# qiyueyao/Kubernetes-verification

Measured on AMD Instinct MI355X. Metric: pod-pairs/sec for reachability build + all-checks latency, 100k pods, 1/2/4/8 GPU, higher is better.
Workload: dtype u64

## Files before the change

kubernetes-verification_amd/csrc/kano_engine.hpp:

```cpp
#pragma once
#include <hip/hip_runtime.h>
#include <hip/hip_ext.h>

#include <algorithm>
#include <cmath>
#include <functional>
#include <cerrno>
#include <cstdint>
#include <cstdlib>
#include <cstring>
#include <string>
#include <vector>
#include <array>
#include <chrono>
#include <ctime>
#include <cstdio>
#include <dlfcn.h>
#include <link.h>
#include <thread>

#include "kano_hip.h"
#include "kano_internal.hpp"
#include "kano_prims.hpp"

using namespace kano;

namespace {
constexpr int MAX_CWW = 8192;
constexpr int MAX_CWW_KNOB = 16384;
constexpr int XCD_WRITE = 3;
constexpr long long XCD_MIN_BYTES = 1ll << 30;
constexpr int HT_ROWS = 128;
constexpr int ROWS_CH = 24;
constexpr int LD_ALIGN = 16;
constexpr int MFMA_KMIN = 8;

}

struct DBuf {
  void* p = nullptr;
  size_t bytes = 0;
};

struct ClassSet {
  std::vector<int32_t> keys;
  int KS = 0;
  int packed = 0;
  int tbits = 0;
  i64 U = 0;
  i64 m0 = 0, m1 = 0;
  DBuf keys_d, table, smin, slot_of, flag, cid, cls, rep, mcnt, mcur, moff, mem, cval;
};

struct RowsInputs {
  DBuf wioff, wicls, soffc, slist, aloff, alist, alcoff, alc, rmoff, rmem, cmoff, cmem, ccls,
      hflag, hlist, Mc;
};

struct SideMatch {
  i64 nterms = 0;
  int NM = 0;
  bool dense = false;
  DBuf toff, tslot, tval, pmask, moff, mslot;
  DBuf table, pslot, gcnt, goff, gcur, gmem, pstart, plen, bits, bcnt, boff;
  i64 T = 0;
};

enum {
  SZ_UR = 0, SZ_UA, SZ_NNZ_SEL, SZ_NNZ_ALC, SZ_NNZ_ALW, SZ_NFLAGS, SZ_WI, SZ_HEAVY, SZ_MAXSEL,
  SZ_LIGHT, SZ_HSEL, SZ_NL, SZ_PAIRS, SZ_IDX0, SZ_IDX1, SZ_IDX2, SZ_IDX3, SZ_ERR, SZ_SLOTS = 18,
  SZ_SIGNAL = SZ_SLOTS
};

constexpr size_t ROW_STAGE_BYTES = 256 * 1024;

struct kano_ctx {
  int device = 0;
  hipStream_t stream = nullptr;
  bool own_stream = false;
  std::string err;

  i64 n = 0, W = 0, ldM = 0, P = 0, PB = 0;
  int ncols = 0;
  std::vector<int32_t> colbits;
  i64 r0 = 0, r1 = -1;
  bool have_pods = false, have_pols = false, built = false;
  bool lists_mode = false;
  bool cols_valid = false;
  bool rows_dirty = false;
  bool rows_deferred = false;
  bool defer_alloc = false;
  bool rows_timed = false;
  bool alist_valid = false;
  bool cols_deferred = false;
  int32_t cross_G = 0;
  i64 groups_n = -1;
  int32_t groups_G = 0;
  int stage_timing = 0;
  int cls_packed = 1;
  int rows_wide = 1;
  DBuf rw_items, rw_segs, rw_ticket;
  DBuf slist_tmp;
  int sort_ww = 768;
  i64 rows_w_grid = 0;
  int rows_early_heavy = 2;
  int assign_ipt = 0;
  int async_rows = 1;
  int shadow_count_mode = 0;
  int path_dens = 8;
  int path_tm = 2;
  int path_tn = 2;
  int heavy_gemm = -1;
  double xo_mfma = 4500e12, xo_or = 8500e9;
  i64 heavy_gemm_min = 512;
  int time_or = 0;
  int heavy_expand_lds = 2;
  int dx_on = 1;
  DBuf dx_sc, dx_sa;
  DBuf mct;
  bool shg_prefilled = false;
  i64 dx_ldY = 0, dx_PBo = 0;
  bool dense_sel = false;
  int ac_lds = 1;
  int mlists_side_ok = 1;
  bool mlists_side = false;
  bool rin_marked = false;
  i64 sel_early_cap = -1;
  int path_lds = 1;
  int rows_ch = ROWS_CH;
  int rows_cww = MAX_CWW_KNOB;
  int shadow_r = 0;
  int shg_sub_lds = 1;
  int rows_cu_off = 20;
  int xcd_split = 1;
  i64 xcd_min_bytes = XCD_MIN_BYTES;
  int xcd_write = XCD_WRITE;
  int xcd_eng0 = -1;
  bool xcd_tried = false, eng_on_xcd = false, xcd_last_ok = false;
  int side_mode = 0;
  int xcd_side = -1;
  hipStream_t stream_x = nullptr, stream2_x = nullptr, stream3x = nullptr;
  hipStream_t stream2_u = nullptr;
  hipEvent_t ev_sw = nullptr, ev_sw2 = nullptr;
  i64 rows_cu_bytes = 8ll << 30;
  int num_cus = 0, rows_cus = 0;

  ClassSet rc, cc;
  SideMatch sm, am;
  i64 UAW = 0, ldC = 0;
  i64 nnz_sel = 0, nnz_alc = 0, nnz_alw = 0, heavy_count = 0, wi_total = 0, nflags = 0;
  i64 heavy_sel = 0;
  i64 light_cost = 0;
  bool rows_use_alist = false;
  int max_sel = 0;
  int heavy_path = 0;
  int heavy_kernel = 0;
  int rows_kernel = 0;

  DBuf pv;
  DBuf scnt, cost, soffc, scur, slist, ecls, wicls, maxs, wicnt, wioff, hflag, hoff, hlist, sq, pfoff;
  DBuf ACT, AC, nca, acnt, alcoff, alc, aloff, alist;
  DBuf M, Mc, color, colnand, col_and, col_or_c, col_nand_c;
  DBuf scan_tmp;
  i64 scan_cap = 0;
  int scan_parity = 0;
  DBuf scan_tmp2;
  i64 scan_cap2 = 0;
  int scan_parity2 = 0;
  hipEvent_t ev_pre = nullptr, ev_pre_done = nullptr, ev_pre_ac = nullptr;
  bool pre_forked = false, pre_side_pending = false, pre_ac_pending = false;
  bool tail_compacted = false;
  hipEvent_t ev_pairs = nullptr;
  DBuf gid, gids, cgroup, R, multi, A1, A2, own, cross, gmin, gmax, ckey, corder, kcnt, koff;
  DBuf flags, T, loff, L, tp, poff, out, tcnt, toff;
  DBuf scratch_words, ident;
  DBuf xw, xg;
  i64 xg_emul = -1;
  DBuf pT, pR[2], pD[2], pA, pB, pcnt;
  DBuf xv, asel, aalw, iterm, idead, irows;
  i64 inc_A = 0, inc_acap = 0, inc_xcols = 0;
  std::vector<uint8_t> dead;
  bool user_edited = false;
  i64 shadow_total = -1;
  DBuf conflict_out;
  i64 conflict_total = -1;
  bool vs_count_only = false;
  bool shg_ran = false;
  DBuf shg_h, shg_tkey, shg_trep, shg_slot, shg_isrep, shg_gidx, shg_gid, shg_reps, shg_sub,
      shg_err;
  DBuf sizes;
  DBuf icnt, ioff, sysrow, idxd;
  u64* ghost = nullptr;
  void* row_stage = nullptr;
  u64* gmirror = nullptr;
  u64* gmirror_dev = nullptr;
  DBuf sig_ctr;
  u64 sig_seq = 0;
  u64 sig_armed = 0;
  u64 sig_wait = 0;
  double ht[20] = {};
  double ht_wait_cur = 0.0;
  int ht_wait = 0;
  std::chrono::steady_clock::time_point ht_last{};

  hipEvent_t ev[10] = {};
  hipStream_t stream2 = nullptr;
  hipEvent_t ev_fork2 = nullptr, ev_join2 = nullptr;
  bool fork_pending = false;
  std::function<int(bool)> fork_hook;
  hipStream_t stream3 = nullptr;
  hipStream_t stream3m = nullptr;
  bool stream3m_tried = false;
  hipStream_t rows_last = nullptr;
  RowsInputs rin_alt;
  int rows_set = 0;
  bool rows_overlap = false;
  hipEvent_t rows_after = nullptr;
  hipEvent_t rows_in = nullptr;
  hipEvent_t ev_rin = nullptr;
  hipEvent_t ev_rin_e = nullptr;
  hipEvent_t ev_rows_end[2] = {};
  hipEvent_t rows_end_ev[2] = {};
  bool rows_end_rec[2] = {false, false};
  hipEvent_t ev_fork = nullptr;
  hipEvent_t ev_sizes = nullptr;
  bool async_pending = false;
  int pipeline = 0;
  bool primed = false;
  bool priming = false;
  bool consume_prime = false;
  bool prime_pre_marked = false;
  bool prime_alist_valid = false;
  u64 prime_sig = 0;
  u64* bell = nullptr;
  u64* bell_dev = nullptr;
  u64 bell_seq = 0;
  u64 gate_ticks = 0;
  u64 wall_khz = 100000;
  DBuf gate_wait;
  u64 gate_seq0 = 0;
  u64 gate_forced = 0;
  DBuf sizes_alt;
  hipEvent_t ev_tail = nullptr;
  hipEvent_t ev_rt[2][2] = {};
  bool rows_time_pending[2] = {false, false};
  hipEvent_t ev_m0 = nullptr, ev_m1 = nullptr;
  bool mfma_time_pending = false;
  double mfma_ops_last = 0.0, mfma_ops_sum = 0.0, mfma_ms_sum = 0.0;
  i64 mfma_n = 0;
  float rows_ms_last = 0.f;
  double rows_ms_sum = 0.0, rows_ms_min = 0.0, rows_ms_max = 0.0;
  i64 rows_ms_n = 0;
  bool vs_open = false, vs_shadow = false, vs_cross_want = false, vs_cross_on = false;
  bool vs_have_sys = false, vs_sys_on = false;
  bool vs_rows = false;
  i64 vs_nb = 0, vs_rl = 0;
};

#define KCHK(expr)                                                                 \
  do {                                                                             \
    hipError_t e_ = (expr);                                                        \
    if (e_ != hipSuccess) {                                                        \
      ctx->err = std::string(#expr) + " -> " + hipGetErrorString(e_);             \
      return -EIO;                                                                 \
    }                                                                              \
  } while (0)

#define KLAUNCH()                                                                  \
  do {                                                                             \
    hipError_t e_ = hipGetLastError();                                             \
    if (e_ != hipSuccess) {                                                        \
      ctx->err = std::string("kernel launch at line ") + std::to_string(__LINE__) + \
                 " -> " + hipGetErrorString(e_);                                   \
      return -EIO;                                                                 \
    }                                                                              \
  } while (0)

#define KTRY(expr)       \
  do {                   \
    int rc_ = (expr);    \
    if (rc_) return rc_; \
  } while (0)

namespace kano_eng {

int fail(kano_ctx* ctx, int code, const std::string& msg);
int settle(kano_ctx* ctx);
int dalloc(kano_ctx* ctx, DBuf& b, size_t bytes);
void dfree(DBuf& b);
int sync(kano_ctx* ctx);
int ensure_built(kano_ctx* ctx);
int ensure_matrix(kano_ctx* ctx);
i64 rows_local(const kano_ctx* ctx);

template <typename T>
T* P_(DBuf& b) {
  return reinterpret_cast<T*>(b.p);
}

inline unsigned nblk(i64 n, i64 per = TPB) { return (unsigned)((n + per - 1) / per); }

}
```

kubernetes-verification_amd/csrc/kano_hip.hip:

```cpp
#include "kano_engine.hpp"
#include "kano_kernels.hpp"

namespace kano_eng {

int fail(kano_ctx* ctx, int code, const std::string& msg) {
  ctx->err = msg;
  return code;
}

int settle(kano_ctx* ctx);

int dalloc(kano_ctx* ctx, DBuf& b, size_t bytes) {
  if (bytes == 0) bytes = 16;
  if (b.p && b.bytes >= bytes) return 0;
  if (b.p) {
    KTRY(settle(ctx));
    KCHK(hipFree(b.p));
    b.p = nullptr;
    b.bytes = 0;
  }
  const hipError_t e = hipMalloc(&b.p, bytes);
  if (e != hipSuccess) {
    b.p = nullptr;
    return fail(ctx, -ENOMEM, "hipMalloc(" + std::to_string(bytes) + " bytes) -> " +
                                  hipGetErrorString(e));
  }
  b.bytes = bytes;
  return 0;
}

void dfree(DBuf& b) {
  if (b.p) (void)hipFree(b.p);
  b.p = nullptr;
  b.bytes = 0;
}


template <typename... KArgs, typename... Args>
void launch_marked(void (*kernel)(KArgs...), dim3 grid, dim3 block, size_t lds, hipStream_t st,
                   hipEvent_t ev, Args... args) {
  hipExtLaunchKernelGGL(kernel, grid, block, (std::uint32_t)lds, st, nullptr, ev, 0, args...);
}

inline i64 scan_tiles(i64 n, int items = SCAN_ITEMS) {
  return (n + (i64)TPB * items - 1) / ((i64)TPB * items);
}

int scan_reserve(kano_ctx* ctx, i64 slots, bool side = false) {
  i64& cap = side ? ctx->scan_cap2 : ctx->scan_cap;
  if (slots <= cap) return 0;
  slots = std::max<i64>(slots, 2 * cap);
  const size_t bytes = sizeof(u64) * 2 * (size_t)slots;
  DBuf& tmp = side ? ctx->scan_tmp2 : ctx->scan_tmp;
  KTRY(dalloc(ctx, tmp, bytes));
  KCHK(hipMemsetAsync(tmp.p, 0, bytes, side ? ctx->stream2 : ctx->stream));
  cap = slots;
  (side ? ctx->scan_parity2 : ctx->scan_parity) = 0;
  return 0;
}

struct ScanBatch {
  ScanJobs jobs{};
  kano_ctx* ctx;
  bool side = false;
  explicit ScanBatch(kano_ctx* c, bool on_side = false) : ctx(c), side(on_side) {
    jobs.count = 0;
    jobs.npub = 0;
  }
  void publish(int slot) {
    if (!ctx->gmirror_dev || jobs.npub == MAX_PUBLISH) return;
    jobs.pub_src[jobs.npub] = P_<u64>(ctx->sizes) + slot;
    jobs.pub_dst[jobs.npub] = ctx->gmirror_dev + slot;
    ++jobs.npub;
  }
  template <typename Tin, typename Tout>
  int add(const Tin* in, i64 n, Tout* out, int total_slot = -1) {
    static_assert(sizeof(Tin) == 4 || sizeof(Tin) == 8, "int32 / int64 scans");
    static_assert(sizeof(Tout) == 4 || sizeof(Tout) == 8, "int32 / int64 scans");
    if (jobs.count == MAX_SCAN_JOBS) KTRY(run());
    ScanJob& j = jobs.j[jobs.count++];
    j.in = in;
    j.out = out;
    j.total = total_slot >= 0 ? P_<u64>(ctx->sizes) + total_slot : nullptr;
    j.total_host = total_slot >= 0 && ctx->gmirror_dev ? ctx->gmirror_dev + total_slot : nullptr;
    j.n = n;
    j.st = 0;
    j.in64 = sizeof(Tin) == 8;
    j.out64 = sizeof(Tout) == 8;
    j.gen = 0;
    j.gcnt = nullptr;
    return 0;
  }
  int add_rep_flags(ClassSet& cs, int pbits, i64 n, int total_slot) {
    KTRY(add(static_cast<const int32_t*>(nullptr), n, P_<int32_t>(cs.cid), total_slot));
    ScanJob& j = jobs.j[jobs.count - 1];
    j.gen = 1;
    j.gsmin = P_<int32_t>(cs.smin);
    j.gtab = P_<u64>(cs.table);
    j.gpb = pbits;
    j.gslot = P_<int32_t>(cs.slot_of);
    j.gm0 = cs.m0;
    return 0;
  }
  int add_class_lengths(const int32_t* cls, const i64* loff, i64 m0, i64 n, i64* out,
                        int total_slot) {
    KTRY(add(static_cast<const int32_t*>(nullptr), n, out, total_slot));
    ScanJob& j = jobs.j[jobs.count - 1];
    j.gen = 2;
    j.gslot = cls;
    j.gloff = loff;
    j.gm0 = m0;
    return 0;
  }
  int add_class_counts(const int32_t* cls, const i64* cnt, i64 m0, i64 n, i64* out,
                       int total_slot) {
    KTRY(add(static_cast<const int32_t*>(nullptr), n, out, total_slot));
    ScanJob& j = jobs.j[jobs.count - 1];
    j.gen = 3;
    j.gslot = cls;
    j.gcnt = cnt;
    j.gm0 = m0;
    return 0;
  }
  template <int NJ, int IT>
  void launch_n(dim3 g, u64* cur, u64* nxt, hipEvent_t mark) {
    ScanJobsN<NJ> a;
    for (int q = 0; q < NJ; ++q) a.j[q] = jobs.j[q];
    a.count = jobs.count;
    a.npub = jobs.npub;
    for (int q = 0; q < MAX_PUBLISH; ++q) {
      a.pub_src[q] = jobs.pub_src[q];
      a.pub_dst[q] = jobs.pub_dst[q];
    }
    a.sig_host = jobs.sig_host;
    a.sig_val = jobs.sig_val;
    a.sig_ctr = jobs.sig_ctr;
    a.sig_n = jobs.sig_n;
    launch_marked(k_scan_lb<NJ, IT>, g, dim3(TPB), 0, side ? ctx->stream2 : ctx->stream, mark, a,
                  cur, nxt, side ? ctx->scan_cap2 : ctx->scan_cap);
  }
  template <int IT>
  void launch_it(dim3 g, u64* cur, u64* nxt, hipEvent_t mark) {
    switch (jobs.count) {
      case 1: launch_n<1, IT>(g, cur, nxt, mark); break;
      case 2: launch_n<2, IT>(g, cur, nxt, mark); break;
      case 3: launch_n<3, IT>(g, cur, nxt, mark); break;
      case 4: launch_n<4, IT>(g, cur, nxt, mark); break;
      case 5: launch_n<5, IT>(g, cur, nxt, mark); break;
      case 6: launch_n<6, IT>(g, cur, nxt, mark); break;
      case 7: launch_n<7, IT>(g, cur, nxt, mark); break;
      default: launch_n<MAX_SCAN_JOBS, IT>(g, cur, nxt, mark); break;
    }
  }
  int run(hipEvent_t mark = nullptr) {
    if (jobs.count == 0) return 0;
    const int items = SCAN_ITEMS;
    i64 slots = 0, maxt = 1;
    for (int q = 0; q < jobs.count; ++q) {
      jobs.j[q].st = slots;
      slots += 1 + scan_tiles(jobs.j[q].n, items);
      maxt = std::max<i64>(maxt, scan_tiles(jobs.j[q].n, items));
    }
    KTRY(scan_reserve(ctx, slots, side));
    int writers = jobs.npub > 0 ? 1 : 0;
    for (int q = 0; q < jobs.count; ++q) writers += jobs.j[q].total_host ? 1 : 0;
    jobs.sig_host = nullptr;
    if (side) writers = 0;
    if (writers > 0 && ctx->sig_ctr.p) {
      jobs.sig_host = ctx->gmirror_dev + SZ_SIGNAL;
      jobs.sig_val = ++ctx->sig_seq;
      jobs.sig_ctr = reinterpret_cast<uint32_t*>(ctx->sig_ctr.p);
      jobs.sig_n = writers;
      ctx->sig_armed = jobs.sig_val;
    } else if (writers > 0) {
      ctx->sig_armed = 0;
    }
    u64* st = P_<u64>(side ? ctx->scan_tmp2 : ctx->scan_tmp);
    const i64 cap = side ? ctx->scan_cap2 : ctx->scan_cap;
    int& parity = side ? ctx->scan_parity2 : ctx->scan_parity;
    u64* cur = st + (parity ? cap : 0);
    u64* nxt = st + (parity ? 0 : cap);
    const dim3 g((unsigned)maxt, (unsigned)jobs.count);
    if (items == 32) launch_it<32>(g, cur, nxt, mark);
    else if (items == 16) launch_it<16>(g, cur, nxt, mark);
    else if (items == 4) launch_it<4>(g, cur, nxt, mark);
    else launch_it<SCAN_ITEMS>(g, cur, nxt, mark);
    KLAUNCH();
    parity ^= 1;
    jobs.count = 0;
    jobs.npub = 0;
    return 0;
  }
};

template <typename Tin, typename Tout>
int scan_excl(kano_ctx* ctx, const Tin* in, i64 n, Tout* out) {
  ScanBatch sb(ctx);
  KTRY(sb.add(in, n, out));
  return sb.run();
}

struct FillBatch {
  FillJobs jobs{};
  kano_ctx* ctx;
  hipStream_t st = nullptr;
  explicit FillBatch(kano_ctx* c, hipStream_t s = nullptr) : ctx(c), st(s) { jobs.count = 0; }
  int add(DBuf& b, size_t bytes, uint32_t value);
  int add_raw(void* p, size_t bytes, uint32_t value) {
    if (bytes == 0) return 0;
    if (jobs.count == MAX_FILLS) KTRY(run());
    jobs.j[jobs.count++] = FillJob{static_cast<uint32_t*>(p), (i64)(bytes / 4), value};
    return 0;
  }
  int run();
  FillJobs take() {
    FillJobs j = jobs;
    jobs.count = 0;
    return j;
  }
};

unsigned fill_ride_blocks(const FillJobs& fj) {
  if (fj.count == 0) return 0;
  i64 most = 0;
  for (int q = 0; q < fj.count; ++q) most = std::max(most, fj.j[q].words);
  return (unsigned)std::max<i64>(1, std::min<i64>(FILL_RIDE_BLOCKS, (most + TPB - 1) / TPB));
}

int FillBatch::add(DBuf& b, size_t bytes, uint32_t value) {
  if (bytes == 0) return 0;
  if (bytes % 4 != 0 || bytes > b.bytes) return fail(ctx, -EINVAL, "internal: bad fill job");
  if (jobs.count == MAX_FILLS) KTRY(run());
  jobs.j[jobs.count++] = FillJob{reinterpret_cast<uint32_t*>(b.p), (i64)(bytes / 4), value};
  return 0;
}

int FillBatch::run() {
  if (jobs.count == 0) return 0;
  i64 most = 0;
  for (int q = 0; q < jobs.count; ++q) most = std::max(most, jobs.j[q].words);
  const unsigned grid = (unsigned)std::max<i64>(1, std::min<i64>(2048, (most + TPB - 1) / TPB));
  hipLaunchKernelGGL(k_fill_many, dim3(grid), dim3(TPB), 0, st ? st : ctx->stream, jobs);
  KLAUNCH();
  jobs.count = 0;
  return 0;
}

void swap_rows_ptrs(kano_ctx* ctx) {
  RowsInputs& a = ctx->rin_alt;
  std::swap(ctx->wioff, a.wioff);
  std::swap(ctx->wicls, a.wicls);
  std::swap(ctx->soffc, a.soffc);
  std::swap(ctx->slist, a.slist);
  std::swap(ctx->aloff, a.aloff);
  std::swap(ctx->alist, a.alist);
  std::swap(ctx->alcoff, a.alcoff);
  std::swap(ctx->alc, a.alc);
  std::swap(ctx->rc.moff, a.rmoff);
  std::swap(ctx->rc.mem, a.rmem);
  std::swap(ctx->cc.moff, a.cmoff);
  std::swap(ctx->cc.mem, a.cmem);
  std::swap(ctx->cc.cls, a.ccls);
  std::swap(ctx->hflag, a.hflag);
  std::swap(ctx->hlist, a.hlist);
  std::swap(ctx->Mc, a.Mc);
  ctx->rows_set ^= 1;
}

void ring_bell(kano_ctx* ctx) {
  if (ctx->bell) __atomic_store_n(ctx->bell, ctx->bell_seq, __ATOMIC_SEQ_CST);
}

int unprime(kano_ctx* ctx) {
  if (!ctx->primed || ctx->priming) return 0;
  ctx->primed = false;
  ring_bell(ctx);
  ctx->gate_forced = ctx->bell_seq;
  KCHK(hipStreamSynchronize(ctx->stream));
  KCHK(hipStreamSynchronize(ctx->stream2));
  std::swap(ctx->sizes, ctx->sizes_alt);
  swap_rows_ptrs(ctx);
  ctx->alist_valid = ctx->prime_alist_valid;
  return 0;
}

int sync(kano_ctx* ctx) {
  KTRY(unprime(ctx));
  KCHK(hipStreamSynchronize(ctx->stream));
  return 0;
}

int settle(kano_ctx* ctx) {
  KTRY(unprime(ctx));
  if (!ctx->async_pending) return 0;
  ctx->async_pending = false;
  KCHK(hipSetDevice(ctx->device));
  KCHK(hipStreamSynchronize(ctx->stream3));
  if (ctx->stream3m) KCHK(hipStreamSynchronize(ctx->stream3m));
  if (ctx->stream3x) KCHK(hipStreamSynchronize(ctx->stream3x));
  return sync(ctx);
}

int resolve_rows_slot(kano_ctx* ctx, int k, bool block) {
  if (!ctx->rows_time_pending[k]) return 0;
  if (!block) {
    const hipError_t q = hipEventQuery(ctx->ev_rt[k][1]);
    if (q == hipErrorNotReady) return 0;
    KCHK(q);
  }
  ctx->rows_time_pending[k] = false;
  KCHK(hipEventSynchronize(ctx->ev_rt[k][1]));
  float ms = 0.f;
  KCHK(hipEventElapsedTime(&ms, ctx->ev_rt[k][0], ctx->ev_rt[k][1]));
  ctx->rows_ms_last = ms;
  if (ctx->rows_ms_n == 0 || ms < ctx->rows_ms_min) ctx->rows_ms_min = ms;
  if (ctx->rows_ms_n == 0 || ms > ctx->rows_ms_max) ctx->rows_ms_max = ms;
  ctx->rows_ms_sum += ms;
  ctx->rows_ms_n += 1;
  return 0;
}

int resolve_rows_time(kano_ctx* ctx, bool block = true) {
  for (int k = 0; k < 2; ++k) KTRY(resolve_rows_slot(ctx, k, block));
  return 0;
}

int swap_rows_inputs(kano_ctx* ctx) {
  swap_rows_ptrs(ctx);
  ctx->alist_valid = false;
  if (ctx->rows_end_rec[ctx->rows_set]) {
    const hipError_t q = hipEventQuery(ctx->rows_end_ev[ctx->rows_set]);
    if (q == hipErrorNotReady)
      KCHK(hipStreamWaitEvent(ctx->stream, ctx->rows_end_ev[ctx->rows_set], 0));
    else
      KCHK(q);
  }
  return 0;
}


int resolve_mfma_time(kano_ctx* ctx) {
  if (!ctx->mfma_time_pending) return 0;
  ctx->mfma_time_pending = false;
  KCHK(hipEventSynchronize(ctx->ev_m1));
  float ms = 0.f;
  KCHK(hipEventElapsedTime(&ms, ctx->ev_m0, ctx->ev_m1));
  ctx->mfma_ms_sum += ms;
  ctx->mfma_ops_sum += ctx->mfma_ops_last;
  ctx->mfma_n += 1;
  return 0;
}

int read_slots(kano_ctx* ctx, int first, int count, i64* out) {
  KCHK(hipMemcpyAsync(ctx->ghost, P_<u64>(ctx->sizes) + first, sizeof(u64) * count,
                      hipMemcpyDeviceToHost, ctx->stream));
  KTRY(sync(ctx));
  for (int k = 0; k < count; ++k) out[k] = (i64)ctx->ghost[k];
  return 0;
}

void* pinned_dev(void* host) {
  if (!host || (reinterpret_cast<uintptr_t>(host) & 15)) return nullptr;
  hipPointerAttribute_t at{};
  void* dptr = nullptr;
  if (hipPointerGetAttributes(&at, host) == hipSuccess && at.type == hipMemoryTypeHost &&
      at.devicePointer)
    dptr = at.devicePointer;
  (void)hipGetLastError();
  return dptr;
}

int copy_out(kano_ctx* ctx, void* host, const void* dev, size_t bytes, hipStream_t st) {
  if (bytes == 0) return 0;
  hipPointerAttribute_t at{};
  void* dptr = nullptr;
  if (hipPointerGetAttributes(&at, host) == hipSuccess && at.type == hipMemoryTypeHost &&
      at.devicePointer)
    dptr = at.devicePointer;
  (void)hipGetLastError();
  if (!dptr || (reinterpret_cast<uintptr_t>(dptr) & 15) || (reinterpret_cast<uintptr_t>(dev) & 15)) {
    KCHK(hipMemcpyAsync(host, dev, bytes, hipMemcpyDeviceToHost, st));
    return 0;
  }
  const i64 n16 = (i64)(bytes / 16);
  const int ntail = (int)((bytes % 16) / 4);
  const unsigned grid = (unsigned)std::max<i64>(1, std::min<i64>(1024, nblk(std::max<i64>(1, n16))));
  hipLaunchKernelGGL(k_copy_out, dim3(grid), dim3(TPB), 0, st, static_cast<const uint4*>(dev),
                     static_cast<uint4*>(dptr), n16,
                     reinterpret_cast<const uint32_t*>(static_cast<const char*>(dev) + n16 * 16),
                     reinterpret_cast<uint32_t*>(static_cast<char*>(dptr) + n16 * 16), ntail);
  KLAUNCH();
  return 0;
}

int mirror_begin(kano_ctx* ctx) {
  if (ctx->sig_armed) {
    ctx->sig_wait = ctx->sig_armed;
    ctx->sig_armed = 0;
    return 0;
  }
  ctx->sig_wait = 0;
  KCHK(hipEventRecord(ctx->ev_sizes, ctx->stream));
  return 0;
}

int wait_signal(kano_ctx* ctx, u64 val) {
  volatile u64* sig = ctx->gmirror + SZ_SIGNAL;
  using clk = std::chrono::steady_clock;
  const auto t0 = clk::now();
  for (uint32_t spin = 1; *sig < val; ++spin) {
    __builtin_ia32_pause();
    if ((spin & 0xfff) != 0) continue;
    if (clk::now() - t0 > std::chrono::seconds(1)) {
      KCHK(hipStreamSynchronize(ctx->stream));
      if (*sig < val)
        return fail(ctx, -EIO, "internal: host signal not raised (wait " +
                                   std::to_string(ctx->ht_wait) + ": want " + std::to_string(val) +
                                   ", have " + std::to_string((u64)*sig) + ")");
      break;
    }
  }
  return 0;
}

int mirror_wait(kano_ctx* ctx, int first, int count, i64* out) {
  const auto t0 = std::chrono::steady_clock::now();
  if (ctx->sig_wait) {
    const u64 v = ctx->sig_wait;
    ctx->sig_wait = 0;
    KTRY(wait_signal(ctx, v));
  } else {
    KCHK(hipEventSynchronize(ctx->ev_sizes));
  }
  const double w =
      std::chrono::duration<double, std::micro>(std::chrono::steady_clock::now() - t0).count();
  ctx->ht_wait_cur += w;
  const int k = 9 + std::min(ctx->ht_wait++, 2);
  ctx->ht[k] = std::max(ctx->ht[k], w);
  for (int q = 0; q < count; ++q) out[q] = (i64)((volatile u64*)ctx->gmirror)[first + q];
  return 0;
}

int stage_mark(kano_ctx* ctx, int k, hipStream_t st) {
  if (ctx->stage_timing) KCHK(hipEventRecord(ctx->ev[k], st));
  return 0;
}

i64 rows_local(const kano_ctx* ctx) { return ctx->r1 - ctx->r0; }

i64 table_size(i64 n) {
  i64 T = 64;
  while (T < 2 * n) T <<= 1;
  return T;
}

int cls_pod_bits(const kano_ctx* ctx, const ClassSet& cs) {
  if (!cs.packed) return 0;
  int pb = 1;
  while (pb < 31 && ((i64)1 << pb) < ctx->n) ++pb;
  return cs.tbits + pb <= 63 ? pb : 0;
}

int classify_alloc1(kano_ctx* ctx, ClassSet& cs, FillBatch& fb) {
  const i64 n = ctx->n, T = table_size(n);
  KTRY(dalloc(ctx, cs.table, sizeof(u64) * T));
  KTRY(dalloc(ctx, cs.smin, sizeof(int32_t) * T));
  KTRY(dalloc(ctx, cs.slot_of, sizeof(int32_t) * std::max<i64>(1, n)));
  KTRY(dalloc(ctx, cs.flag, sizeof(int32_t) * std::max<i64>(1, n)));
  KTRY(dalloc(ctx, cs.cid, sizeof(int32_t) * (n + 1)));
  KTRY(dalloc(ctx, cs.cls, sizeof(int32_t) * std::max<i64>(1, n)));
  KTRY(fb.add(cs.table, (cs.packed ? sizeof(u64) : sizeof(int32_t)) * T, 0xffffffffu));
  if (!cls_pod_bits(ctx, cs)) KTRY(fb.add(cs.smin, sizeof(int32_t) * T, 0x7fffffffu));
  const i64 m = std::max<i64>(1, cs.m1 - cs.m0);
  KTRY(dalloc(ctx, cs.rep, sizeof(int32_t) * m));
  KTRY(dalloc(ctx, cs.mcnt, sizeof(int32_t) * m));
  KTRY(dalloc(ctx, cs.mcur, sizeof(int32_t) * m));
  KTRY(dalloc(ctx, cs.moff, sizeof(int32_t) * (m + 1)));
  KTRY(dalloc(ctx, cs.mem, sizeof(int32_t) * m));
  return 0;
}

ClsSide cls_side(kano_ctx* ctx, ClassSet& cs) {
  ClsSide a{};
  a.keys = P_<int32_t>(cs.keys_d);
  a.KS = cs.KS;
  a.packed = cs.packed;
  a.pbits = cls_pod_bits(ctx, cs);
  a.tmask = (uint32_t)(table_size(ctx->n) - 1);
  a.table = P_<int32_t>(cs.table);
  a.slot_of = P_<int32_t>(cs.slot_of);
  a.smin = P_<int32_t>(cs.smin);
  a.flag = P_<int32_t>(cs.flag);
  a.cid = P_<int32_t>(cs.cid);
  a.cls = P_<int32_t>(cs.cls);
  a.rep = P_<int32_t>(cs.rep);
  a.mcnt = P_<int32_t>(cs.mcnt);
  a.mcur = P_<int32_t>(cs.mcur);
  a.moff = P_<int32_t>(cs.moff);
  a.mem = P_<int32_t>(cs.mem);
  a.cval = P_<int32_t>(cs.cval);
  a.m0 = cs.m0;
  a.m1 = cs.m1;
  a.U = cs.U;
  return a;
}

int classify_phase1(kano_ctx* ctx) {
  const i64 n = ctx->n;
  ClsPair pr{{cls_side(ctx, ctx->rc), cls_side(ctx, ctx->cc)}};
  const i64 nr = ctx->rc.m1 - ctx->rc.m0, na = ctx->cc.m1 - ctx->cc.m0;
  const i64 most = std::max(nr, na);
  if (most > 0) {
    hipLaunchKernelGGL(k_cls_insert, dim3(nblk(most), 2), dim3(TPB), 0, ctx->stream,
                       P_<int32_t>(ctx->pv), n, pr);
    KLAUNCH();
  }
  ScanBatch sb(ctx);
  KTRY(sb.add_rep_flags(ctx->rc, cls_pod_bits(ctx, ctx->rc), nr, SZ_UR));
  KTRY(sb.add_rep_flags(ctx->cc, cls_pod_bits(ctx, ctx->cc), na, SZ_UA));
  return sb.run();
}

int classify_alloc2(kano_ctx* ctx, ClassSet& cs) {
  return dalloc(ctx, cs.cval, sizeof(int32_t) * std::max<i64>(1, (i64)cs.KS * cs.U));
}

int classify_phase2a(kano_ctx* ctx) {
  ClsPair pr{{cls_side(ctx, ctx->rc), cls_side(ctx, ctx->cc)}};
  const i64 mr = ctx->rc.m1 - ctx->rc.m0, ma = ctx->cc.m1 - ctx->cc.m0;
  const i64 rl = std::max(mr, ma);
  hipStream_t side = ctx->mlists_side ? ctx->stream2 : nullptr;
  if (rl > 0) {
    const i64 prevU = std::max(ctx->rc.U, ctx->cc.U);
    const int ipt = ctx->assign_ipt > 0 ? ctx->assign_ipt
                                        : (prevU > 0 && prevU <= 1024 ? ASSIGN_IPT : 1);
    launch_marked(k_cls_assign_count, dim3(nblk(rl, (i64)TPB * ipt), 2), dim3(TPB), 0,
                  ctx->stream, side ? ctx->ev_pre : nullptr, pr, ipt);
    KLAUNCH();
  } else if (side) {
    KCHK(hipEventRecord(ctx->ev_pre, ctx->stream));
  }
  if (side) KCHK(hipStreamWaitEvent(side, ctx->ev_pre, 0));
  ScanBatch sb(ctx, side != nullptr);
  KTRY(sb.add(P_<int32_t>(ctx->rc.mcnt), mr, P_<int32_t>(ctx->rc.moff)));
  KTRY(sb.add(P_<int32_t>(ctx->cc.mcnt), ma, P_<int32_t>(ctx->cc.moff)));
  KTRY(sb.run());
  if (rl > 0) {
    hipLaunchKernelGGL(k_cls_mfill, dim3(nblk(rl), 2), dim3(TPB), 0, side ? side : ctx->stream, pr,
                       (const int32_t*)nullptr, 0, (int32_t*)nullptr, (int32_t*)nullptr,
                       reinterpret_cast<int32_t*>(P_<u64>(ctx->sizes) + SZ_ERR));
    KLAUNCH();
  }
  return 0;
}

int classify_phase2b(kano_ctx* ctx, FillJobs fj) {
  ClsPair pr{{cls_side(ctx, ctx->rc), cls_side(ctx, ctx->cc)}};
  const i64 U = std::max(ctx->rc.U, ctx->cc.U);
  if (U > 0) {
    const unsigned nbv = nblk(U), nbf = fill_ride_blocks(fj);
    hipLaunchKernelGGL(k_cls_vals, dim3(nbv + nbf, 2), dim3(TPB), 0, ctx->stream,
                       P_<int32_t>(ctx->pv), ctx->n, pr, fj, nbv);
    KLAUNCH();
  } else if (fj.count > 0) {
    hipLaunchKernelGGL(k_fill_many, dim3(fill_ride_blocks(fj)), dim3(TPB), 0, ctx->stream, fj);
    KLAUNCH();
  }
  return 0;
}

int match_alloc(kano_ctx* ctx, SideMatch& sx, ClassSet& cs, FillBatch& fb) {
  const i64 P = ctx->P, U = cs.U;
  KTRY(dalloc(ctx, sx.pstart, sizeof(i64) * std::max<i64>(1, P)));
  KTRY(dalloc(ctx, sx.plen, sizeof(int32_t) * std::max<i64>(1, P)));
  if (P == 0) return 0;
  if (U == 0) {
    KTRY(fb.add(sx.pstart, sizeof(i64) * P, 0u));
    KTRY(fb.add(sx.plen, sizeof(int32_t) * P, 0u));
    return 0;
  }
  if (sx.dense) return 0;
  const int NM = sx.NM;
  sx.T = table_size(U);
  const i64 NT = std::max<i64>(1, (i64)NM * sx.T);
  KTRY(dalloc(ctx, sx.table, sizeof(int32_t) * NT));
  KTRY(dalloc(ctx, sx.pslot, sizeof(int32_t) * std::max<i64>(1, (i64)NM * U)));
  KTRY(dalloc(ctx, sx.gcnt, sizeof(int32_t) * NT));
  KTRY(dalloc(ctx, sx.gcur, sizeof(int32_t) * std::max<i64>(1, (i64)NM * U)));
  KTRY(dalloc(ctx, sx.goff, sizeof(int32_t) * (NT + 1)));
  KTRY(dalloc(ctx, sx.gmem, sizeof(int32_t) * ((i64)NM * U + U)));
  if (NM > 0) {
    KTRY(fb.add(sx.table, sizeof(int32_t) * NT, 0xffffffffu));
    KTRY(fb.add(sx.gcnt, sizeof(int32_t) * NT, 0u));
  }
  return 0;
}

JoinSide join_side(kano_ctx* ctx, SideMatch& sx, ClassSet& cs) {
  JoinSide a{};
  a.cval = P_<int32_t>(cs.cval);
  a.U = cs.U;
  a.moff = P_<int32_t>(sx.moff);
  a.mslot = P_<int32_t>(sx.mslot);
  a.table = P_<int32_t>(sx.table);
  a.T = sx.T;
  a.pslot = P_<int32_t>(sx.pslot);
  a.gcnt = P_<int32_t>(sx.gcnt);
  a.goff = P_<int32_t>(sx.goff);
  a.gcur = P_<int32_t>(sx.gcur);
  a.gmem = P_<int32_t>(sx.gmem);
  a.toff = P_<i64>(sx.toff);
  a.tval = P_<int32_t>(sx.tval);
  a.pmask = P_<int32_t>(sx.pmask);
  a.pstart = P_<i64>(sx.pstart);
  a.plen = P_<int32_t>(sx.plen);
  a.NM = sx.NM;
  a.live = (ctx->P > 0 && cs.U > 0 && !sx.dense) ? 1 : 0;
  a.ctab = P_<u64>(cs.table);
  a.ctmask = (uint32_t)(table_size(ctx->n) - 1);
  a.csmin = P_<int32_t>(cs.smin);
  a.cpb = cls_pod_bits(ctx, cs);
  a.ccid = P_<int32_t>(cs.cid);
  a.cm0 = cs.m0;
  a.kbits = P_<int32_t>(cs.keys_d) + cs.KS;
  a.KS = cs.KS;
  return a;
}

int match_dense(kano_ctx* ctx, SideMatch& sx, ClassSet& cs);

int match_both(kano_ctx* ctx) {
  JoinPair pr{{join_side(ctx, ctx->am, ctx->cc), join_side(ctx, ctx->sm, ctx->rc)}};
  const JoinSide &a0 = pr.s[0], &a1 = pr.s[1];
  const i64 maxU = std::max(a0.live ? a0.U : 0, a1.live ? a1.U : 0);
  const unsigned rows_i = (a0.live ? a0.NM : 0) + (a1.live ? a1.NM : 0);
  const unsigned rows_f = (a0.live ? a0.NM + 1 : 0) + (a1.live ? a1.NM + 1 : 0);
  if (rows_i > 0) {
    hipLaunchKernelGGL(k_join_insert, dim3(nblk(maxU), rows_i), dim3(TPB), 0, ctx->stream, pr);
    KLAUNCH();
    ScanBatch sb(ctx);
    for (int q = 0; q < 2; ++q) {
      SideMatch& sx = q ? ctx->sm : ctx->am;
      if (pr.s[q].live && sx.NM > 0)
        KTRY(sb.add(P_<int32_t>(sx.gcnt), (i64)sx.NM * sx.T, P_<int32_t>(sx.goff)));
    }
    KTRY(sb.run());
  }
  if (rows_f > 0) {
    const unsigned nbf = nblk(maxU), nbm = nblk(ctx->P);
    hipLaunchKernelGGL(k_join_fill_match, dim3(std::max(nbf, nbm), rows_f + 2), dim3(TPB), 0,
                       ctx->stream, ctx->P, pr, (int)rows_f, nbf, nbm);
    KLAUNCH();
  }
  if (ctx->P > 0 && ctx->cc.U > 0 && ctx->am.dense) KTRY(match_dense(ctx, ctx->am, ctx->cc));
  if (ctx->P > 0 && ctx->rc.U > 0 && ctx->sm.dense) KTRY(match_dense(ctx, ctx->sm, ctx->rc));
  return 0;
}

int match_dense(kano_ctx* ctx, SideMatch& sx, ClassSet& cs) {
  const i64 P = ctx->P, U = cs.U;
  const i64 UW = (U + 63) / 64, ld = std::max<i64>(2, (UW + 1) & ~(i64)1);
  KTRY(dalloc(ctx, sx.bits, sizeof(u64) * P * ld));
  KTRY(dalloc(ctx, sx.boff, sizeof(i64) * (P + 1)));
  hipLaunchKernelGGL(k_class_eval, dim3(nblk(U), (unsigned)ctx->PB), dim3(TPB), 0, ctx->stream,
                     P_<int32_t>(cs.cval), U, P, P_<i64>(sx.toff), P_<int32_t>(sx.tslot),
                     P_<int32_t>(sx.tval), (u64*)nullptr, P_<u64>(sx.bits), ld);
  KLAUNCH();
  hipLaunchKernelGGL(k_popc_rows, dim3((unsigned)P), dim3(TPB), 0, ctx->stream, P_<u64>(sx.bits),
                     ld, UW, P_<int32_t>(sx.plen));
  KLAUNCH();
  KTRY((scan_excl<int32_t, i64>(ctx, P_<int32_t>(sx.plen), P, P_<i64>(sx.boff))));
  i64 nnz = 0;
  KCHK(hipMemcpyAsync(&nnz, P_<i64>(sx.boff) + P, 8, hipMemcpyDeviceToHost, ctx->stream));
  KTRY(sync(ctx));
  KTRY(dalloc(ctx, sx.gmem, sizeof(int32_t) * std::max<i64>(1, nnz)));
  hipLaunchKernelGGL(k_bits_to_lists, dim3((unsigned)P), dim3(TPB), 0, ctx->stream,
                     P_<u64>(sx.bits), ld, UW, P_<i64>(sx.boff), P_<int32_t>(sx.gmem));
  KLAUNCH();
  hipLaunchKernelGGL(k_offsets_to_start, dim3(nblk(P)), dim3(TPB), 0, ctx->stream,
                     P_<i64>(sx.boff), P, P_<i64>(sx.pstart));
  KLAUNCH();
  return 0;
}

int sel_spb(const kano_ctx* ctx) {
  return ctx->P >= 8 * std::max<i64>(1, ctx->rc.U) ? TPB : WPB;
}

int front_fills(kano_ctx* ctx, FillBatch& fb) {
  KTRY(dalloc(ctx, ctx->sizes, sizeof(u64) * SZ_SLOTS));
  KTRY(fb.add(ctx->sizes, sizeof(u64) * SZ_SLOTS, 0u));
  KTRY(classify_alloc1(ctx, ctx->rc, fb));
  KTRY(classify_alloc1(ctx, ctx->cc, fb));
  return 0;
}

int select_engine_streams(kano_ctx* ctx);

int front_a(kano_ctx* ctx) {
  KTRY(select_engine_streams(ctx));
  ctx->rc.m0 = ctx->r0;
  ctx->rc.m1 = ctx->r1;
  ctx->cc.m0 = 0;
  ctx->cc.m1 = ctx->n;
  {
    FillBatch fb(ctx);
    KTRY(front_fills(ctx, fb));
    KTRY(fb.run());
  }
  KTRY(classify_phase1(ctx));
  KTRY(mirror_begin(ctx));
  ctx->mlists_side = ctx->stream2 != nullptr && ctx->mlists_side_ok;
  if (!ctx->mlists_side && ctx->stream2) {
    KTRY(classify_phase2a(ctx));
    KCHK(hipEventRecord(ctx->ev_pre, ctx->stream));
    return 0;
  }
  return classify_phase2a(ctx);
}

int do_front(kano_ctx* ctx, int path, bool primed = false) {
  if (primed) {
    ctx->primed = false;
    ring_bell(ctx);
    ctx->rc.m0 = ctx->r0;
    ctx->rc.m1 = ctx->r1;
    ctx->cc.m0 = 0;
    ctx->cc.m1 = ctx->n;
    ctx->sig_wait = ctx->prime_sig;
  } else {
    KTRY(front_a(ctx));
  }
  ctx->pre_forked = ctx->stream2 != nullptr;
  i64 u[2] = {0, 0};
  KTRY(mirror_wait(ctx, SZ_UR, 2, u));
  KTRY(resolve_rows_time(ctx, false));
  ctx->rc.U = u[0];
  ctx->cc.U = u[1];
  KTRY(stage_mark(ctx, 1, ctx->stream));

  const i64 P = ctx->P, Ur = ctx->rc.U, Ua = ctx->cc.U;
  ctx->UAW = (Ua + 63) / 64;
  ctx->ldC = std::max<i64>(2, (ctx->UAW + 1) & ~(i64)1);
  FillJobs carried{};
  {
    FillBatch fb(ctx);
    KTRY(classify_alloc2(ctx, ctx->rc));
    KTRY(classify_alloc2(ctx, ctx->cc));
    KTRY(match_alloc(ctx, ctx->am, ctx->cc, fb));
    KTRY(match_alloc(ctx, ctx->sm, ctx->rc, fb));
    KTRY(dalloc(ctx, ctx->nca, sizeof(int32_t) * std::max<i64>(1, P)));
    KTRY(dalloc(ctx, ctx->acnt, sizeof(int32_t) * std::max<i64>(1, P)));
    KTRY(dalloc(ctx, ctx->alcoff, sizeof(i64) * (P + 1)));
    KTRY(dalloc(ctx, ctx->aloff, sizeof(i64) * (P + 1)));
    KTRY(dalloc(ctx, ctx->scnt, sizeof(int32_t) * std::max<i64>(1, Ur)));
    KTRY(dalloc(ctx, ctx->cost, sizeof(u64) * std::max<i64>(1, Ur)));
    KTRY(dalloc(ctx, ctx->wicnt, sizeof(int32_t) * std::max<i64>(1, Ur)));
    KTRY(dalloc(ctx, ctx->hflag, sizeof(int32_t) * std::max<i64>(1, Ur)));
    KTRY(dalloc(ctx, ctx->sq, sizeof(i64) * std::max<i64>(1, Ur)));
    KTRY(dalloc(ctx, ctx->soffc, sizeof(i64) * (Ur + 1)));
    KTRY(dalloc(ctx, ctx->wioff, sizeof(int32_t) * (Ur + 1)));
    KTRY(dalloc(ctx, ctx->hoff, sizeof(int32_t) * (Ur + 1)));
    KTRY(dalloc(ctx, ctx->pfoff, sizeof(i64) * (Ur + 1)));
    KTRY(dalloc(ctx, ctx->scur, sizeof(int32_t) * std::max<i64>(1, Ur)));
    KTRY(fb.add(ctx->scnt, sizeof(int32_t) * Ur, 0u));
    KTRY(fb.add(ctx->cost, sizeof(u64) * Ur, 0u));
    KTRY(fb.add(ctx->scur, sizeof(int32_t) * Ur, 0u));
    carried = fb.take();
  }
  KTRY(classify_phase2b(ctx, carried));
  KTRY(match_both(ctx));
  KTRY(stage_mark(ctx, 2, ctx->stream));
  ctx->dense_sel = ctx->dx_on && Ur > 0 && Ur <= DX_MAX &&
                   (ctx->dx_on == 2 || ctx->nnz_sel >= 32 * Ur);
  if (P > 0 && ctx->dense_sel) {
    const i64 ldU = (Ur + 63) / 64;
    ctx->dx_ldY = (Ur + 255) / 256 * 256;
    ctx->dx_PBo = (ctx->PB + GK_KC - 1) / GK_KC * GK_KC;
    KTRY(dalloc(ctx, ctx->dx_sc, sizeof(u64) * (size_t)(P * ldU)));
    KTRY(dalloc(ctx, ctx->dx_sa, sizeof(u64) * (size_t)(ctx->dx_PBo * ctx->dx_ldY)));
    hipLaunchKernelGGL(k_selrows_dx, dim3(nblk(P, WPB)), dim3(TPB), sizeof(u64) * WPB * ldU,
                       ctx->stream, P, P_<i64>(ctx->am.pstart), P_<int32_t>(ctx->am.plen),
                       P_<int32_t>(ctx->am.gmem), P_<int32_t>(ctx->cc.mcnt), P_<int32_t>(ctx->nca),
                       P_<int32_t>(ctx->acnt), P_<i64>(ctx->sm.pstart), P_<int32_t>(ctx->sm.plen),
                       P_<int32_t>(ctx->sm.gmem), ldU, P_<u64>(ctx->dx_sc));
    KLAUNCH();
    const i64 tiles = ctx->dx_PBo * (ctx->dx_ldY / 64);
    hipLaunchKernelGGL(k_ptrans, dim3(nblk(tiles, WPB)), dim3(TPB), 0, ctx->stream,
                       P_<u64>(ctx->dx_sc), ldU, P, P_<u64>(ctx->dx_sa), ctx->dx_ldY, ctx->dx_PBo,
                       (const int32_t*)nullptr);
    KLAUNCH();
    hipLaunchKernelGGL(k_cls_counts_dx, dim3((unsigned)Ur), dim3(TPB), 0, ctx->stream,
                       P_<u64>(ctx->dx_sa), ctx->dx_ldY, ctx->PB, Ur, P_<int32_t>(ctx->acnt),
                       P_<int32_t>(ctx->scnt), P_<unsigned long long>(ctx->cost));
    KLAUNCH();
  } else if (P > 0) {
    const bool sel = Ur > 0;
    hipLaunchKernelGGL(k_pol_counts, dim3(nblk(P, sel_spb(ctx))), dim3(TPB), 0, ctx->stream, P,
                       P_<i64>(ctx->am.pstart), P_<int32_t>(ctx->am.plen),
                       P_<int32_t>(ctx->am.gmem), P_<int32_t>(ctx->cc.mcnt), P_<int32_t>(ctx->nca),
                       P_<int32_t>(ctx->acnt), P_<i64>(ctx->sm.pstart), P_<int32_t>(ctx->sm.plen),
                       sel ? P_<int32_t>(ctx->sm.gmem) : (const int32_t*)nullptr,
                       P_<int32_t>(ctx->scnt), P_<unsigned long long>(ctx->cost), sel_spb(ctx));
    KLAUNCH();
  }
  if (Ur > 0) {
    ClassPlan a;
    a.U = Ur;
    a.scnt = P_<int32_t>(ctx->scnt);
    a.cost = P_<unsigned long long>(ctx->cost);
    a.mcnt = P_<int32_t>(ctx->rc.mcnt);
    a.W = ctx->W;
    a.ch = ctx->rows_ch;
    a.force = path == KANO_PATH_MFMA ? 2 : 0;
    a.wicnt = P_<int32_t>(ctx->wicnt);
    a.hflag = P_<int32_t>(ctx->hflag);
    a.sq = P_<i64>(ctx->sq);
    a.maxs = reinterpret_cast<int32_t*>(P_<u64>(ctx->sizes) + SZ_MAXSEL);
    a.light = P_<unsigned long long>(ctx->sizes) + SZ_LIGHT;
    a.hsel = P_<unsigned long long>(ctx->sizes) + SZ_HSEL;
    hipLaunchKernelGGL(k_class_plan, dim3(nblk(Ur)), dim3(TPB), 0, ctx->stream, a);
    KLAUNCH();
  }
  ScanBatch sb(ctx);
  KTRY(sb.add(P_<int32_t>(ctx->nca), P, P_<i64>(ctx->alcoff), SZ_NNZ_ALC));
  KTRY(sb.add(P_<int32_t>(ctx->acnt), P, P_<i64>(ctx->aloff), SZ_NNZ_ALW));
  KTRY(sb.add(P_<int32_t>(ctx->scnt), Ur, P_<i64>(ctx->soffc), SZ_NNZ_SEL));
  KTRY(sb.add(P_<int32_t>(ctx->wicnt), Ur, P_<int32_t>(ctx->wioff), SZ_WI));
  KTRY(sb.add(P_<int32_t>(ctx->hflag), Ur, P_<int32_t>(ctx->hoff), SZ_HEAVY));
  KTRY(sb.add(P_<i64>(ctx->sq), Ur, P_<i64>(ctx->pfoff), SZ_NFLAGS));
  sb.publish(SZ_MAXSEL);
  sb.publish(SZ_LIGHT);
  sb.publish(SZ_HSEL);
  KTRY(sb.run());
  return 0;
}

int read_sizes(kano_ctx* ctx) {
  i64 v[SZ_HSEL - SZ_NNZ_SEL + 1];
  KTRY(mirror_wait(ctx, SZ_NNZ_SEL, SZ_HSEL - SZ_NNZ_SEL + 1, v));
  ctx->nnz_sel = v[SZ_NNZ_SEL - SZ_NNZ_SEL];
  ctx->nnz_alc = v[SZ_NNZ_ALC - SZ_NNZ_SEL];
  ctx->nnz_alw = v[SZ_NNZ_ALW - SZ_NNZ_SEL];
  ctx->nflags = v[SZ_NFLAGS - SZ_NNZ_SEL];
  ctx->wi_total = v[SZ_WI - SZ_NNZ_SEL];
  ctx->heavy_count = v[SZ_HEAVY - SZ_NNZ_SEL];
  ctx->max_sel = (int)(v[SZ_MAXSEL - SZ_NNZ_SEL] & 0xffffffff);
  ctx->light_cost = v[SZ_LIGHT - SZ_NNZ_SEL];
  ctx->heavy_sel = v[SZ_HSEL - SZ_NNZ_SEL];
  return 0;
}

int mc_cols(kano_ctx* ctx) {
  const i64 U = ctx->rc.U;
  if (rows_local(ctx) > 0 && U > 0) {
    hipLaunchKernelGGL(k_mc_cols, dim3(nblk(ctx->UAW, 64), nblk(U, 128)), dim3(TPB), 0,
                       ctx->stream, P_<u64>(ctx->Mc), ctx->ldC, ctx->UAW, ctx->cc.U, U,
                       P_<int32_t>(ctx->rc.mcnt), P_<u64>(ctx->col_or_c), P_<u64>(ctx->col_nand_c));
    KLAUNCH();
  }
  return 0;
}

PolPodsArgs pol_pods_args(kano_ctx* ctx) {
  return PolPodsArgs{ctx->P, P_<i64>(ctx->alcoff), P_<int32_t>(ctx->alc),
                     P_<int32_t>(ctx->cc.moff), P_<int32_t>(ctx->cc.mem), P_<i64>(ctx->aloff),
                     P_<int32_t>(ctx->alist)};
}

int build_alist(kano_ctx* ctx, hipStream_t st = nullptr, bool launch = true) {
  const i64 P = ctx->P;
  KTRY(dalloc(ctx, ctx->alist, sizeof(int32_t) * std::max<i64>(1, ctx->nnz_alw)));
  if (launch && P > 0 && ctx->cc.U > 0) {
    hipLaunchKernelGGL(k_pol_pods, dim3(nblk(P, WPB)), dim3(TPB), 0, st ? st : ctx->stream,
                       pol_pods_args(ctx));
    KLAUNCH();
  }
  ctx->alist_valid = true;
  return 0;
}

bool ac_whole_rows(const kano_ctx* ctx) {
  return ctx->ac_lds && ctx->P > 0 && ctx->cc.U > 0 &&
         sizeof(u64) * (size_t)ctx->ldC * WPB <= 32 * 1024;
}

using PreLaunch = std::function<int(FillBatch&)>;
using PreRun = std::function<int(hipStream_t)>;
int do_back_pre(kano_ctx* ctx, const PreLaunch& pre_fill, const PreRun& pre_run) {
  const i64 U = ctx->rc.U, P = ctx->P, ldMc = ctx->ldC;
  const bool side = ctx->pre_forked;
  ctx->pre_forked = false;
  hipStream_t ss = side ? ctx->stream2 : nullptr;
  if (side) KCHK(hipStreamWaitEvent(ss, ctx->ev_pre, 0));
  KTRY(dalloc(ctx, ctx->AC, sizeof(u64) * std::max<i64>(1, P * ctx->ldC)));
  KTRY(dalloc(ctx, ctx->Mc, sizeof(u64) * std::max<i64>(1, U * ldMc)));
  KTRY(dalloc(ctx, ctx->col_or_c, sizeof(u64) * ldMc));
  KTRY(dalloc(ctx, ctx->col_nand_c, sizeof(u64) * ldMc));
  const bool ac_fill = !ac_whole_rows(ctx);
  if (side && ac_fill) {
    FillBatch fa(ctx, ss);
    KTRY(fa.add(ctx->AC, sizeof(u64) * P * ctx->ldC, 0u));
    KTRY(fa.run());
    KCHK(hipEventRecord(ctx->ev_pre_ac, ss));
    ctx->pre_ac_pending = true;
  }
  {
    FillBatch fb(ctx, ss);
    if (!side && ac_fill) KTRY(fb.add(ctx->AC, sizeof(u64) * P * ctx->ldC, 0u));
    KTRY(fb.add(ctx->Mc, sizeof(u64) * U * ldMc, 0u));
    KTRY(fb.add(ctx->col_or_c, sizeof(u64) * ldMc, 0u));
    KTRY(fb.add(ctx->col_nand_c, sizeof(u64) * ldMc, 0u));
    if (pre_fill) KTRY(pre_fill(fb));
    KTRY(fb.run());
  }
  if (pre_run) KTRY(pre_run(ss));
  if (side) {
    KCHK(hipEventRecord(ctx->ev_pre_done, ss));
    ctx->pre_side_pending = true;
  }
  return 0;
}

int join_event(kano_ctx* ctx, hipEvent_t e) {
  const hipError_t q = hipEventQuery(e);
  if (q == hipSuccess) return 0;
  if (q != hipErrorNotReady) KCHK(q);
// ... 783 lines not shown
  KLAUNCH();
  const i64 budget_rows = std::max<i64>(1, (2ll << 30) / (8 * ldM));
  const unsigned ycols = std::max<unsigned>(1, nblk(W, TPB * 4));
  for (int32_t g0 = 0; g0 < G; g0 += (int32_t)budget_rows) {
    const int32_t g1 = (int32_t)std::min<i64>(G, (i64)g0 + budget_rows);
    const i64 ng = g1 - g0;
    KTRY(dalloc(ctx, ctx->R, sizeof(u64) * ng * ldM));
    KCHK(hipMemsetAsync(ctx->R.p, 0, sizeof(u64) * ng * ldM, ctx->stream));
    hipLaunchKernelGGL(k_cross_accum, dim3((unsigned)nclass, ycols), dim3(TPB), 0, ctx->stream,
                       P_<int32_t>(ctx->cgroup), moff, mem, P_<u64>(ctx->M), ldM, ctx->r0, W, g0,
                       g1, P_<u64>(ctx->R), P_<u64>(ctx->multi));
    KLAUNCH();
    hipLaunchKernelGGL(k_cross_groups, dim3((unsigned)ng, ycols), dim3(TPB), 0, ctx->stream,
                       P_<u64>(ctx->R), ldM, W, P_<u64>(ctx->A1), P_<u64>(ctx->A2));
    KLAUNCH();
    hipLaunchKernelGGL(k_cross_own, dim3(nblk(n)), dim3(TPB), 0, ctx->stream,
                       gdev, n, P_<u64>(ctx->R), ldM, g0, g1, P_<u64>(ctx->own));
    KLAUNCH();
  }
  hipLaunchKernelGGL(k_cross_final, dim3(nblk(W)), dim3(TPB), 0, ctx->stream, P_<u64>(ctx->multi),
                     P_<u64>(ctx->A1), P_<u64>(ctx->A2), P_<u64>(ctx->own), W, n,
                     P_<u64>(ctx->cross));
  KLAUNCH();
  return 0;
}

}

using namespace kano_eng;

extern "C" {

int kano_create_lean(int device, kano_ctx** out) {
  g_create_lean = true;
  const int rc = kano_create(device, out);
  g_create_lean = false;
  return rc;
}

int kano_create(int device, kano_ctx** out) {
  if (!out) return -EINVAL;
  *out = nullptr;
  int ndev = 0;
  if (hipGetDeviceCount(&ndev) != hipSuccess || ndev == 0) return -ENODEV;
  if (device < 0 || device >= ndev) return -EINVAL;
  const bool trace = getenv("KANO_CREATE_TRACE") != nullptr;
  auto tc0 = std::chrono::steady_clock::now();
  auto mark = [&](const char* what) {
    if (!trace) return;
    const auto t = std::chrono::steady_clock::now();
    std::fprintf(stderr, "kano_create %s %.3f ms\n", what,
                 std::chrono::duration<double, std::milli>(t - tc0).count());
    tc0 = t;
  };
  if (hipSetDevice(device) != hipSuccess) return -EIO;
  mark("set_device");
  kano_ctx* ctx = new kano_ctx();
  ctx->device = device;
  (void)hipDeviceGetAttribute(&ctx->num_cus, hipDeviceAttributeMultiprocessorCount, device);
  if (const char* t = getenv("KANO_TUNE")) {
    std::string spec(t);
    size_t pos = 0;
    while (pos < spec.size()) {
      size_t end = spec.find(',', pos);
      if (end == std::string::npos) end = spec.size();
      const std::string kv = spec.substr(pos, end - pos);
      const size_t eq = kv.find('=');
      if (eq != std::string::npos) {
        const std::string k = kv.substr(0, eq);
        const int v = atoi(kv.c_str() + eq + 1);
        if (k == "timing") ctx->stage_timing = v;
        if (k == "packed") ctx->cls_packed = v;
        if (k == "rw" && v >= 0 && v <= 2) ctx->rows_wide = v;
        if (k == "rwg" && v >= 0) ctx->rows_w_grid = v;
        if (k == "rheavy" && v >= 0 && v <= 2) ctx->rows_early_heavy = v;
        if (k == "aipt" && v >= 0 && v <= ASSIGN_IPT) ctx->assign_ipt = v;
        if (k == "sww" && v >= 1 && v <= SORT_LDS_WW) ctx->sort_ww = v;
        if (k == "cww" && v >= 16 && v <= MAX_CWW_KNOB && v % 16 == 0) ctx->rows_cww = v;
        if (k == "rch" && v >= 1 && v <= 1024) ctx->rows_ch = v;
        if (k == "async") ctx->async_rows = v;
        if (k == "shcount" && v >= 0 && v <= 2) ctx->shadow_count_mode = v;
        if (k == "pathdens" && v >= 0 && v <= 101) ctx->path_dens = v;
        if (k == "pathtm" && (v == 1 || v == 2 || v == 4)) ctx->path_tm = v;
        if (k == "pathlds") ctx->path_lds = v;
        if (k == "pathtn" && (v == 2 || v == 4)) ctx->path_tn = v;
        if (k == "shgsub") ctx->shg_sub_lds = v;
        if (k == "shr" && (v == 1 || v == 2 || v == 4 || v == 8)) ctx->shadow_r = v;
        if (k == "rcu" && v >= 0 && v <= 28 && (v < 4 || v % 4 == 0)) ctx->rows_cu_off = v;
        if (k == "rcubytes" && v >= 0) ctx->rows_cu_bytes = (i64)v << 30;
        if (k == "xcd") ctx->xcd_split = v;
        if (k == "xcdmin" && v >= 0) ctx->xcd_min_bytes = (i64)v << 10;
        if (k == "xcdw" && v >= 1 && v <= 7) ctx->xcd_write = v;
        if (k == "xcde" && v >= 0 && v <= 7) ctx->xcd_eng0 = v;
        if (k == "xcdside" && v >= -1 && v <= 1) ctx->xcd_side = v;
        if (k == "hgemm" && (v == -1 || v == 0 || v == 22 || v == 42 || v == 44))
          ctx->heavy_gemm = v;
        if (k == "hgemmmin" && v > 0) ctx->heavy_gemm_min = v;
        if (k == "hortime") ctx->time_or = v;
        if (k == "hexplds" && v >= 2 && v <= 4) ctx->heavy_expand_lds = v;
        if (k == "dx") ctx->dx_on = v;
        if (k == "aclds") ctx->ac_lds = v;
        if (k == "mlside") ctx->mlists_side_ok = v;
        if (k == "xomfma" && v > 0) ctx->xo_mfma = (double)v * 1e12;
        if (k == "xoor" && v > 0) ctx->xo_or = (double)v * 1e9;
      }
      pos = end + 1;
    }
  }
  int prio_lo = 0, prio_hi = 0;
  (void)hipDeviceGetStreamPriorityRange(&prio_lo, &prio_hi);
  (void)prio_lo;

  const int prio_main = prio_hi;
  if (hipStreamCreateWithPriority(&ctx->stream, hipStreamNonBlocking, prio_main) != hipSuccess) {
    delete ctx;
    return -EIO;
  }
  ctx->own_stream = true;
  mark("stream");
  for (auto& e : ctx->ev) (void)hipEventCreate(&e);
  mark("stage_events");
  {
    const int lds44 = (int)(sizeof(u64) * 2 * GK_KC * (256 + 256));
    (void)hipFuncSetAttribute(reinterpret_cast<const void*>(&k_heavy_gemm_f4<4, 4, gemm_kc(4, 4)>),
                              hipFuncAttributeMaxDynamicSharedMemorySize, lds44);
    (void)hipFuncSetAttribute(reinterpret_cast<const void*>(&k_heavy_gemm_f4<4, 2, gemm_kc(4, 2)>),
                              hipFuncAttributeMaxDynamicSharedMemorySize, lds44);
    (void)hipFuncSetAttribute(reinterpret_cast<const void*>(&k_heavy_gemm_f4<2, 2, gemm_kc(2, 2)>),
                              hipFuncAttributeMaxDynamicSharedMemorySize, lds44);
    (void)hipFuncSetAttribute(reinterpret_cast<const void*>(&k_rows<1024>),
                              hipFuncAttributeMaxDynamicSharedMemorySize,
                              (int)sizeof(u64) * MAX_CWW_KNOB);
    (void)hipFuncSetAttribute(reinterpret_cast<const void*>(&k_rows_w<1024>),
                              hipFuncAttributeMaxDynamicSharedMemorySize,
                              (int)sizeof(u64) * MAX_CWW_KNOB);
  }
  mark("func_attributes");
  if (hipStreamCreateWithFlags(&ctx->stream3, hipStreamNonBlocking) != hipSuccess) {
    ctx->stream3 = nullptr;
    kano_destroy(ctx);
    return -EIO;
  }
  if (!g_create_lean) KTRY(ensure_masked_stream(ctx));
  mark("write_streams");
  if (hipStreamCreateWithPriority(&ctx->stream2, hipStreamNonBlocking, prio_main) != hipSuccess ||
      hipEventCreateWithFlags(&ctx->ev_fork, hipEventDisableTiming) != hipSuccess ||
      hipEventCreateWithFlags(&ctx->ev_sizes, hipEventDisableTiming) != hipSuccess ||
      hipEventCreateWithFlags(&ctx->ev_tail, hipEventDisableTiming) != hipSuccess ||
      hipEventCreateWithFlags(&ctx->ev_rin, hipEventDisableTiming) != hipSuccess ||
      hipEventCreateWithFlags(&ctx->ev_rin_e, hipEventDisableTiming) != hipSuccess ||
      hipEventCreateWithFlags(&ctx->ev_fork2, hipEventDisableTiming) != hipSuccess ||
      hipEventCreateWithFlags(&ctx->ev_join2, hipEventDisableTiming) != hipSuccess ||
      hipEventCreateWithFlags(&ctx->ev_pre, hipEventDisableTiming) != hipSuccess ||
      hipEventCreateWithFlags(&ctx->ev_pre_done, hipEventDisableTiming) != hipSuccess ||
      hipEventCreateWithFlags(&ctx->ev_pre_ac, hipEventDisableTiming) != hipSuccess ||
      hipEventCreateWithFlags(&ctx->ev_sw, hipEventDisableTiming) != hipSuccess ||
      hipEventCreateWithFlags(&ctx->ev_sw2, hipEventDisableTiming) != hipSuccess ||
      hipEventCreateWithFlags(&ctx->ev_pairs, hipEventDisableTiming) != hipSuccess ||
      hipEventCreate(&ctx->ev_m0) != hipSuccess || hipEventCreate(&ctx->ev_m1) != hipSuccess ||
      hipEventCreateWithFlags(&ctx->ev_rows_end[0], hipEventDisableTiming) != hipSuccess ||
      hipEventCreateWithFlags(&ctx->ev_rows_end[1], hipEventDisableTiming) != hipSuccess ||
      hipEventCreate(&ctx->ev_rt[0][0]) != hipSuccess || hipEventCreate(&ctx->ev_rt[0][1]) != hipSuccess ||
      hipEventCreate(&ctx->ev_rt[1][0]) != hipSuccess || hipEventCreate(&ctx->ev_rt[1][1]) != hipSuccess) {
    kano_destroy(ctx);
    return -EIO;
  }
  mark("stream2_events");
  if (hipHostMalloc(reinterpret_cast<void**>(&ctx->ghost), sizeof(u64) * SZ_SLOTS,
                    hipHostMallocDefault) != hipSuccess) {
    kano_destroy(ctx);
    return -ENOMEM;
  }
  if (hipHostMalloc(reinterpret_cast<void**>(&ctx->gmirror), sizeof(u64) * (SZ_SIGNAL + 1),
                    hipHostMallocCoherent | hipHostMallocMapped) != hipSuccess ||
      hipHostGetDevicePointer(reinterpret_cast<void**>(&ctx->gmirror_dev), ctx->gmirror, 0) !=
          hipSuccess) {
    kano_destroy(ctx);
    return -ENOMEM;
  }
  for (int k = 0; k <= SZ_SIGNAL; ++k) ctx->gmirror[k] = 0;
  if (hipHostMalloc(reinterpret_cast<void**>(&ctx->bell), 64,
                    hipHostMallocCoherent | hipHostMallocMapped) != hipSuccess ||
      hipHostGetDevicePointer(reinterpret_cast<void**>(&ctx->bell_dev), ctx->bell, 0) !=
          hipSuccess) {
    kano_destroy(ctx);
    return -ENOMEM;
  }
  ctx->bell[0] = 0;
  {
    int khz = 0;
    if (hipDeviceGetAttribute(&khz, hipDeviceAttributeWallClockRate, device) != hipSuccess ||
        khz <= 0)
      khz = 100000;
    ctx->gate_ticks = (u64)khz * 200;
    ctx->wall_khz = (u64)khz;
  }
  if (hipHostMalloc(&ctx->row_stage, ROW_STAGE_BYTES, hipHostMallocDefault) != hipSuccess)
    ctx->row_stage = nullptr;
  if (dalloc(ctx, ctx->sig_ctr, sizeof(uint32_t) * 4) != 0 ||
      hipMemset(ctx->sig_ctr.p, 0, sizeof(uint32_t) * 4) != hipSuccess) {
    kano_destroy(ctx);
    return -ENOMEM;
  }
  mark("pinned_and_device_buffers");
  *out = ctx;
  return 0;
}

void kano_destroy(kano_ctx* ctx) {
  if (!ctx) return;
  (void)hipSetDevice(ctx->device);
  ring_bell(ctx);
  if (ctx->stream) (void)hipStreamSynchronize(ctx->stream);
  if (ctx->stream2) (void)hipStreamSynchronize(ctx->stream2);
  if (ctx->stream3) (void)hipStreamSynchronize(ctx->stream3);
  if (ctx->stream3m) (void)hipStreamSynchronize(ctx->stream3m);
  for (hipStream_t t : {ctx->stream_x, ctx->stream2_x, ctx->stream3x, ctx->stream2_u})
    if (t) (void)hipStreamSynchronize(t);
  if (ctx->ghost) (void)hipHostFree(ctx->ghost);
  if (ctx->gmirror) (void)hipHostFree(ctx->gmirror);
  if (ctx->row_stage) (void)hipHostFree(ctx->row_stage);
  if (ctx->bell) (void)hipHostFree(ctx->bell);
  dfree(ctx->sizes_alt);
  dfree(ctx->gate_wait);
  for (ClassSet* cs : {&ctx->rc, &ctx->cc}) {
    DBuf* b[] = {&cs->keys_d, &cs->table, &cs->smin, &cs->slot_of, &cs->flag, &cs->cid, &cs->cls,
                 &cs->rep,    &cs->mcnt,  &cs->mcur, &cs->moff,    &cs->mem,  &cs->cval};
    for (DBuf* x : b) dfree(*x);
  }
  for (SideMatch* sx : {&ctx->sm, &ctx->am}) {
    DBuf* b[] = {&sx->toff,  &sx->tslot, &sx->tval, &sx->pmask,  &sx->moff, &sx->mslot,
                 &sx->table, &sx->pslot, &sx->gcnt, &sx->goff,   &sx->gcur, &sx->gmem,
                 &sx->pstart, &sx->plen, &sx->bits, &sx->bcnt,   &sx->boff};
    for (DBuf* x : b) dfree(*x);
  }
  DBuf* bufs[] = {&ctx->pv,     &ctx->scnt,    &ctx->cost,    &ctx->soffc,     &ctx->scur,
                  &ctx->slist,  &ctx->maxs,    &ctx->wicnt,   &ctx->wioff,     &ctx->hflag,
                  &ctx->hoff,   &ctx->hlist,   &ctx->sq,      &ctx->pfoff,     &ctx->ACT,
                  &ctx->AC,     &ctx->nca,     &ctx->acnt,    &ctx->alcoff,    &ctx->alc,
                  &ctx->aloff,  &ctx->alist,   &ctx->M,       &ctx->Mc,        &ctx->color,
                  &ctx->colnand, &ctx->col_and, &ctx->col_or_c, &ctx->col_nand_c, &ctx->scan_tmp, &ctx->scan_tmp2,
                  &ctx->shg_h,  &ctx->shg_tkey, &ctx->shg_trep, &ctx->shg_slot, &ctx->shg_isrep,
                  &ctx->shg_gidx, &ctx->shg_gid, &ctx->shg_reps, &ctx->shg_sub, &ctx->shg_err, &ctx->sig_ctr,
                  &ctx->gid,    &ctx->cgroup,  &ctx->R,       &ctx->multi,     &ctx->A1,
                  &ctx->A2,     &ctx->own,     &ctx->cross,   &ctx->gmin,      &ctx->gmax,
                  &ctx->flags,  &ctx->T,       &ctx->loff,    &ctx->L,         &ctx->tp,
                  &ctx->poff,   &ctx->out,     &ctx->conflict_out, &ctx->scratch_words, &ctx->ident, &ctx->ecls,
                  &ctx->tcnt,   &ctx->toff,    &ctx->sizes,   &ctx->icnt,      &ctx->ioff,
                  &ctx->sysrow, &ctx->wicls,   &ctx->idxd,
                  &ctx->ckey,   &ctx->corder,  &ctx->kcnt,    &ctx->koff,
                  &ctx->gids,
                  &ctx->pT,     &ctx->pR[0],   &ctx->pR[1],   &ctx->pD[0],     &ctx->pD[1],
                  &ctx->pA,     &ctx->pB,      &ctx->pcnt,
                  &ctx->xv,     &ctx->asel,    &ctx->aalw,    &ctx->iterm,     &ctx->idead,
                  &ctx->irows,  &ctx->xw,      &ctx->xg,
                  &ctx->rw_items, &ctx->rw_segs, &ctx->rw_ticket, &ctx->slist_tmp,
                  &ctx->dx_sc, &ctx->dx_sa, &ctx->mct};
  for (DBuf* b : bufs) dfree(*b);
  RowsInputs& ra = ctx->rin_alt;
  for (DBuf* b : {&ra.wioff, &ra.wicls, &ra.soffc, &ra.slist, &ra.aloff, &ra.alist, &ra.alcoff,
                  &ra.alc, &ra.rmoff, &ra.rmem, &ra.cmoff, &ra.cmem, &ra.ccls, &ra.hflag,
                  &ra.hlist, &ra.Mc})
    dfree(*b);
  for (auto& e : ctx->ev)
    if (e) (void)hipEventDestroy(e);
  if (ctx->own_stream && ctx->stream) (void)hipStreamDestroy(ctx->stream);
  if (ctx->stream2) (void)hipStreamDestroy(ctx->stream2);
  if (ctx->stream3) (void)hipStreamDestroy(ctx->stream3);
  if (ctx->stream3m) (void)hipStreamDestroy(ctx->stream3m);
  for (hipStream_t t : {ctx->stream_x, ctx->stream2_x, ctx->stream3x, ctx->stream2_u})
    if (t) (void)hipStreamDestroy(t);
  for (hipEvent_t e : {ctx->ev_sw, ctx->ev_sw2})
    if (e) (void)hipEventDestroy(e);
  for (hipEvent_t e : {ctx->ev_fork, ctx->ev_tail, ctx->ev_rin, ctx->ev_rin_e, ctx->ev_sizes,
                       ctx->ev_fork2, ctx->ev_join2, ctx->ev_pre, ctx->ev_pre_done, ctx->ev_pre_ac, ctx->ev_pairs, ctx->ev_m0, ctx->ev_m1, ctx->ev_rows_end[0],
                       ctx->ev_rows_end[1], ctx->ev_rt[0][0], ctx->ev_rt[0][1], ctx->ev_rt[1][0],
                       ctx->ev_rt[1][1]})
    if (e) (void)hipEventDestroy(e);
  delete ctx;
}

const char* kano_last_error(const kano_ctx* ctx) { return ctx ? ctx->err.c_str() : "null context"; }

int kano_set_stream(kano_ctx* ctx, void* s) {
  if (!ctx) return -EINVAL;
  KCHK(hipSetDevice(ctx->device));
  KTRY(settle(ctx));
  KTRY(leave_xcd_streams(ctx));
  KCHK(hipStreamSynchronize(ctx->stream2));
  KCHK(hipStreamSynchronize(ctx->stream3));
  if (ctx->stream3m) KCHK(hipStreamSynchronize(ctx->stream3m));
  if (ctx->stream3x) KCHK(hipStreamSynchronize(ctx->stream3x));
  if (ctx->own_stream && ctx->stream) {
    (void)hipStreamSynchronize(ctx->stream);
    (void)hipStreamDestroy(ctx->stream);
    ctx->stream = nullptr;
    ctx->own_stream = false;
  }
  if (s) {
    ctx->stream = (hipStream_t)s;
  } else {
    KCHK(hipStreamCreateWithFlags(&ctx->stream, hipStreamNonBlocking));
    ctx->own_stream = true;
  }
  return 0;
}

int kano_set_pods(kano_ctx* ctx, int64_t n, int32_t ncols, const int32_t* pod_val) {
  if (!ctx) return -EINVAL;
  if (n < 0 || ncols < 0 || n >= (int64_t)INT32_MAX / 2 || (n * ncols > 0 && !pod_val))
    return fail(ctx, -EINVAL, "kano_set_pods: bad arguments");
  KCHK(hipSetDevice(ctx->device));
  KTRY(settle(ctx));
  ctx->n = n;
  ctx->W = (n + 63) / 64;
  ctx->ldM = std::max<i64>(LD_ALIGN, (ctx->W + LD_ALIGN - 1) / LD_ALIGN * LD_ALIGN);
  ctx->ncols = ncols;
  ctx->colbits.assign(ncols, 1);
  for (int32_t c = 0; c < ncols; ++c) {
    int32_t mx = 0, mn = 0;
    const int32_t* col = pod_val + (i64)c * n;
    for (i64 i = 0; i < n; ++i) {
      mx = std::max(mx, col[i] + 3);
      mn = std::min(mn, col[i] + 3);
    }
    int b = 1;
    while (b < 31 && (1 << b) <= mx) ++b;
    ctx->colbits[c] = mn < 0 ? 64 : b;
  }
  KTRY(dalloc(ctx, ctx->pv, sizeof(int32_t) * std::max<i64>(1, n * ncols)));
  if (n * ncols > 0)
    KCHK(hipMemcpyAsync(ctx->pv.p, pod_val, sizeof(int32_t) * n * ncols, hipMemcpyHostToDevice,
                        ctx->stream));
  ctx->r0 = 0;
  ctx->r1 = n;
  ctx->have_pods = true;
  ctx->have_pols = false;
  ctx->built = false;
  return sync(ctx);
}

int kano_set_expressions(kano_ctx* ctx, int32_t E, const int32_t* col, const int32_t* op,
                         const int64_t* off, const int32_t* vals) {
  if (!ctx) return -EINVAL;
  if (!ctx->have_pods) return fail(ctx, -EINVAL, "kano_set_expressions before kano_set_pods");
  if (E < 0 || (E > 0 && (!col || !op || !off))) return fail(ctx, -EINVAL, "kano_set_expressions");
  if (E == 0) return 0;
  KCHK(hipSetDevice(ctx->device));
  KTRY(settle(ctx));
  const i64 n = ctx->n, nc = ctx->ncols;
  for (int32_t e = 0; e < E; ++e) {
    if (col[e] >= nc || op[e] < 0 || op[e] > 3 || off[e + 1] < off[e])
      return fail(ctx, -EINVAL, "kano_set_expressions: bad requirement");
    for (i64 k = off[e] + 1; k < off[e + 1]; ++k)
      if (vals[k - 1] >= vals[k]) return fail(ctx, -EINVAL, "kano_set_expressions: unsorted set");
  }
  DBuf grown;
  KTRY(dalloc(ctx, grown, sizeof(int32_t) * std::max<i64>(1, n * (nc + E))));
  if (n * nc > 0)
    KCHK(hipMemcpyAsync(grown.p, ctx->pv.p, sizeof(int32_t) * n * nc, hipMemcpyDeviceToDevice,
                        ctx->stream));
  const i64 nv = off[E];
  std::vector<uint8_t> h(sizeof(int32_t) * 2 * E + sizeof(i64) * (E + 1) +
                         sizeof(int32_t) * std::max<i64>(1, nv) + 16);
  std::memcpy(h.data(), off, sizeof(i64) * (E + 1));
  int32_t* hb = reinterpret_cast<int32_t*>(h.data() + sizeof(i64) * (E + 1));
  std::memcpy(hb, col, sizeof(int32_t) * E);
  std::memcpy(hb + E, op, sizeof(int32_t) * E);
  if (nv) std::memcpy(hb + 2 * E, vals, sizeof(int32_t) * nv);
  DBuf args;
  KTRY(dalloc(ctx, args, h.size()));
  KCHK(hipMemcpyAsync(args.p, h.data(), h.size(), hipMemcpyHostToDevice, ctx->stream));
  if (n > 0) {
    const i64* d_off = P_<i64>(args);
    const int32_t* d_b = reinterpret_cast<const int32_t*>(d_off + E + 1);
    hipLaunchKernelGGL(k_expr_cols, dim3(nblk(n), (unsigned)E), dim3(TPB), 0, ctx->stream,
                       P_<int32_t>(grown), n, d_b, d_b + E, d_off, d_b + 2 * E,
                       P_<int32_t>(grown) + n * nc);
    KLAUNCH();
  }
  KTRY(sync(ctx));
  dfree(args);
  dfree(ctx->pv);
  ctx->pv = grown;
  ctx->ncols = (int32_t)(nc + E);
  ctx->colbits.resize((size_t)ctx->ncols, 3);
  ctx->have_pols = false;
  ctx->built = false;
  return 0;
}

static constexpr int MAX_MASKS = 64;

static int prepare_side(kano_ctx* ctx, i64 P, const int64_t* off, const int32_t* col,
                        const int32_t* val, ClassSet& cs, SideMatch& sx) {
  const i64 nt = off[P];
  std::vector<int32_t> slot(ctx->ncols, -1);
  for (i64 t = 0; t < nt; ++t) {
    if (col[t] < 0 || col[t] >= ctx->ncols) return fail(ctx, -EINVAL, "term column out of range");
    slot[col[t]] = 0;
  }
  cs.keys.clear();
  for (int32_t c = 0; c < ctx->ncols; ++c)
    if (slot[c] == 0) {
      slot[c] = (int32_t)cs.keys.size();
      cs.keys.push_back(c);
    }
  cs.KS = (int)cs.keys.size();
  std::vector<int32_t> kd(cs.keys);
  int tb = 0;
  for (int32_t c : cs.keys) {
    kd.push_back(ctx->colbits[c]);
    tb += ctx->colbits[c];
  }
  cs.packed = (tb <= 63 && ctx->cls_packed) ? 1 : 0;
  cs.tbits = tb;
  KTRY(dalloc(ctx, cs.keys_d, sizeof(int32_t) * std::max<size_t>(1, kd.size())));
  if (cs.KS > 0)
    KCHK(hipMemcpy(cs.keys_d.p, kd.data(), sizeof(int32_t) * kd.size(), hipMemcpyHostToDevice));
  std::vector<i64> toff(P + 1, 0);
  std::vector<int32_t> tslot, tval, pmask(std::max<i64>(1, P), -1), moff(1, 0), mslot;
  std::vector<std::vector<int32_t>> masks;
  std::vector<std::pair<int32_t, int32_t>> terms;
  tslot.reserve(nt);
  tval.reserve(nt);
  for (i64 p = 0; p < P; ++p) {
    terms.clear();
    for (i64 t = off[p]; t < off[p + 1]; ++t) terms.emplace_back(slot[col[t]], val[t]);
// ... 832 lines not shown
    a.slist = P_<int32_t>(ctx->slist);
    a.mcnt = P_<int32_t>(ctx->rc.mcnt);
    a.pfoff = P_<i64>(ctx->pfoff);
    a.nca = P_<int32_t>(ctx->nca);
    a.alcoff = P_<i64>(ctx->alcoff);
    a.alc = P_<int32_t>(ctx->alc);
    a.AC = P_<u64>(ctx->AC);
    a.ldC = ctx->ldC;
    a.flags = count_only ? nullptr : P_<uint8_t>(ctx->flags);
    a.T = P_<i64>(ctx->T);
    const int R = ctx->shadow_r > 0 ? ctx->shadow_r : (sp.nf >= (i64)1 << 24 ? 8 : 1);
    const i64 grid = (sp.nf + (i64)TPB * R - 1) / ((i64)TPB * R);
    i64* tc = count_only ? (i64*)nullptr : P_<i64>(ctx->tcnt);
    const i64 UA = ctx->cc.U;
#define KANO_CFT(RR)                                                                       \
  hipLaunchKernelGGL((k_conflict_test<1024, RR>), dim3((unsigned)grid), dim3(TPB), 0,      \
                     ctx->stream, a, sp.nf, tc, UA)
    if (R == 8) KANO_CFT(8);
    else if (R == 4) KANO_CFT(4);
    else if (R == 2) KANO_CFT(2);
    else KANO_CFT(1);
#undef KANO_CFT
    KLAUNCH();
  }
  {
    ScanBatch sb(ctx);
    if (!count_only) KTRY(sb.add(P_<i64>(ctx->tcnt), sp.nt, P_<i64>(ctx->toff)));
    KTRY(sb.add(P_<i64>(ctx->T), sp.U, P_<i64>(ctx->loff), SZ_NL));
    KTRY(sb.run());
  }
  {
    ScanBatch sb(ctx);
    KTRY(shadow_stage_b(ctx, sp, sb));
    KTRY(sb.run());
  }
  i64 tot[2] = {0, 0};
  KTRY(read_slots(ctx, SZ_NL, 2, tot));
  *nl = tot[0];
  *total = tot[1];
  return 0;
}

int conflict_compact(kano_ctx* ctx, i64 nl) {
  const i64 U = ctx->rc.U, nf = ctx->nflags;
  const i64 nt = (nf + SH_TILE - 1) / SH_TILE;
  KTRY(dalloc(ctx, ctx->L, sizeof(int2) * std::max<i64>(1, nl)));
  if (nt > 0 && nl > 0) {
    hipLaunchKernelGGL(k_shadow_compact, dim3((unsigned)nt), dim3(TPB), 0, ctx->stream,
                       P_<i64>(ctx->soffc), U, P_<int32_t>(ctx->slist), P_<i64>(ctx->pfoff),
                       P_<uint8_t>(ctx->flags), nf, P_<i64>(ctx->toff), P_<int2>(ctx->L), nl);
    KLAUNCH();
  }
  return 0;
}
}

extern "C" {

int kano_conflict_pairs(kano_ctx* ctx, int mode, int64_t* count, int64_t* class_pairs) {
  KTRY(ensure_built(ctx));
  if (mode != 0 && mode != 1) return fail(ctx, -EINVAL, "kano_conflict_pairs: unknown mode");
  ctx->conflict_total = -1;
  i64 nl = 0, total = 0;
  KTRY(conflict_front(ctx, mode == 1, &nl, &total));
  if (mode == 0) {
    const i64 rl = rows_local(ctx);
    KTRY(dalloc(ctx, ctx->conflict_out, sizeof(int2) * std::max<i64>(1, total)));
    KTRY(conflict_compact(ctx, nl));
    if (rl > 0 && total > 0) {
      hipLaunchKernelGGL(k_shadow_emit, dim3(nblk(rl)), dim3(TPB), 0, ctx->stream,
                         P_<int32_t>(ctx->rc.cls), ctx->r0, ctx->r1, P_<i64>(ctx->loff),
                         P_<int2>(ctx->L), P_<i64>(ctx->poff), P_<int2>(ctx->conflict_out), total,
                         (const i64*)nullptr, nl);
      KLAUNCH();
    }
    ctx->conflict_total = total;
  }
  if (count) *count = total;
  if (class_pairs) *class_pairs = nl;
  return 0;
}

int kano_conflict_fetch(kano_ctx* ctx, int32_t* pairs) {
  KTRY(ensure_built(ctx));
  if (ctx->conflict_total < 0)
    return fail(ctx, -EINVAL, "kano_conflict_fetch before kano_conflict_pairs (mode 0)");
  if (ctx->conflict_total > 0) {
    if (!pairs) return fail(ctx, -EINVAL, "kano_conflict_fetch: NULL buffer");
    KCHK(hipMemcpyAsync(pairs, ctx->conflict_out.p, sizeof(int2) * ctx->conflict_total,
                        hipMemcpyDeviceToHost, ctx->stream));
  }
  return sync(ctx);
}

int kano_conflict_lists(kano_ctx* ctx, int64_t n_lists, int64_t nbits, int64_t P,
                        const int64_t* soff, const int32_t* slist, const uint64_t* allow_rows,
                        int mode, int64_t* count) {
  if (ctx && mode != 0 && mode != 1)
    return fail(ctx, -EINVAL, "kano_conflict_lists: unknown mode");
  KTRY(lists_setup(ctx, "kano_conflict_lists", n_lists, nbits, P, soff, slist, allow_rows));
  return kano_conflict_pairs(ctx, mode, count, nullptr);
}

int kano_conflict_classes(kano_ctx* ctx, int64_t* off, int32_t* pairs, int32_t* members) {
  KTRY(ensure_built(ctx));
  i64 nl = 0, total = 0;
  KTRY(conflict_front(ctx, false, &nl, &total));
  KTRY(conflict_compact(ctx, nl));
  const i64 U = ctx->rc.U;
  if (off)
    KCHK(hipMemcpyAsync(off, ctx->loff.p, sizeof(i64) * (U + 1), hipMemcpyDeviceToHost,
                        ctx->stream));
  if (pairs && nl > 0)
    KCHK(hipMemcpyAsync(pairs, ctx->L.p, sizeof(int2) * nl, hipMemcpyDeviceToHost, ctx->stream));
  if (members && U > 0)
    KCHK(hipMemcpyAsync(members, ctx->rc.mcnt.p, sizeof(int32_t) * U, hipMemcpyDeviceToHost,
                        ctx->stream));
  return sync(ctx);
}

}

namespace {
typedef int (*RcclAllGather)(const void*, void*, size_t, int, void*, hipStream_t);
constexpr int RCCL_UINT64 = 5;
int rccl_find_loaded(struct dl_phdr_info* info, size_t, void* out) {
  const char* name = info->dlpi_name;
  if (name && std::strstr(name, "librccl")) {
    *static_cast<std::string*>(out) = name;
    return 1;
  }
  return 0;
}
RcclAllGather rccl_all_gather() {
  static RcclAllGather fn = [] {
    std::string path;
    dl_iterate_phdr(rccl_find_loaded, &path);
    void* f = nullptr;
    if (!path.empty()) {
      if (void* h = dlopen(path.c_str(), RTLD_NOW | RTLD_NOLOAD)) f = dlsym(h, "ncclAllGather");
    }
    if (!f) f = dlsym(RTLD_DEFAULT, "ncclAllGather");
    if (!f) {
      void* h = dlopen("librccl.so", RTLD_NOW | RTLD_GLOBAL);
      if (!h) h = dlopen("librccl.so.1", RTLD_NOW | RTLD_GLOBAL);
      if (h) f = dlsym(h, "ncclAllGather");
    }
    return reinterpret_cast<RcclAllGather>(f);
  }();
  return fn;
}

int verify_front(kano_ctx* ctx, int path, const int32_t* gid, int32_t ngroups, int64_t sys_row,
                 bool want_shadow, u64* words_dev, bool count_only = false) {
  ctx->vs_count_only = want_shadow && count_only;
  ctx->consume_prime = ctx->primed;
  if (ctx->async_pending && !ctx->primed) KTRY(swap_rows_inputs(ctx));
  const bool stored = !gid && ngroups == KANO_STORED_GROUPS;
  const bool want_cross = gid || stored;
  CrossPlan cp;
  ShadowPlan sp;
  auto pre_fill = [&](FillBatch& fb) -> int {
    return want_cross ? cross_prepare(ctx, gid, ngroups, cp, fb) : 0;
  };
  auto pre_run = [&](hipStream_t st) -> int {
    if (!want_cross || !cp.on) return 0;
    ScanBatch sb(ctx, st != nullptr);
    KTRY(cross_stage_a(ctx, cp, sb, st));
    KTRY(sb.run());
    return cross_stage_b1(ctx, cp, st);
  };
  auto extra = [&](FillBatch& fb) -> int {
    return want_shadow ? shadow_prepare(ctx, sp, fb) : 0;
  };
  ctx->vs_open = false;
  ctx->fork_pending = false;
  ctx->tail_compacted = false;
  bool fork_marked = false;
  const bool side_sh = want_shadow && !count_only;
  if (want_shadow) {
    ctx->fork_hook = [&](bool marked) -> int {
      if (!marked) KCHK(hipEventRecord(ctx->ev_fork2, ctx->stream));
      KCHK(hipStreamWaitEvent(ctx->stream2, ctx->ev_fork2, 0));
      KTRY(shadow_test_launch(ctx, sp, ctx->stream2));
      fork_marked = true;
      return 0;
    };
  }
  const int brc = build_impl(ctx, path, false, want_cross, extra, pre_fill, pre_run);
  ctx->fork_hook = nullptr;
  KTRY(brc);
  const i64 n = ctx->n, W = ctx->W;
  const bool have_sys = sys_row >= ctx->r0 && sys_row < ctx->r1;
  const bool cross_on = want_cross && cp.on;
  if (cross_on) KTRY(cross_stage_b2(ctx, cp));
  const bool side_run = fork_marked && side_sh;
  if (!side_run && fork_marked) {
    KCHK(hipEventRecord(ctx->ev_join2, ctx->stream2));
    ctx->fork_pending = true;
  }
  if (want_shadow && !side_run) {
    ScanBatch sb(ctx);
    if (ctx->fork_pending) {
      KCHK(hipStreamWaitEvent(ctx->stream, ctx->ev_join2, 0));
      ctx->fork_pending = false;
      KTRY(shadow_stage_a_scans(ctx, sp, sb));
    } else {
      KTRY(shadow_stage_a(ctx, sp, sb));
    }
    KTRY(sb.run());
  }
  if (ctx->cols_deferred) {
    ctx->cols_deferred = false;
    KTRY(mc_cols(ctx));
  }
  const i64 nb = std::max<i64>(1, nblk(W * 64));
  KTRY(dalloc(ctx, ctx->col_and, sizeof(u64) * std::max<i64>(1, W)));
  KTRY(dalloc(ctx, ctx->sysrow, sizeof(u64) * std::max<i64>(1, W)));
  KTRY(dalloc(ctx, ctx->icnt, sizeof(i64) * 4 * nb));
  KTRY(dalloc(ctx, ctx->ioff, sizeof(i64) * 4 * (nb + 1)));
  KTRY(dalloc(ctx, ctx->idxd, sizeof(int32_t) * std::max<i64>(1, 4 * n) + 16));
  const bool sys_on = have_sys && W > 0;
  if (n > 0 && W > 0) {
    FinishArgs fa{};
    fa.cla = P_<int32_t>(ctx->cc.cls);
    fa.n = n;
    fa.W = W;
    fa.nb = nb;
    fa.col_or_c = P_<u64>(ctx->col_or_c);
    fa.col_nand_c = P_<u64>(ctx->col_nand_c);
    fa.color = P_<u64>(ctx->color);
    fa.colnand = P_<u64>(ctx->colnand);
    fa.col_and = P_<u64>(ctx->col_and);
    fa.ldC = ctx->ldC;
    if (cross_on) {
      fa.gid = cp.gdev;
      fa.G = cp.G;
      fa.R = P_<u64>(ctx->R);
      fa.multi = P_<u64>(ctx->multi);
      fa.A1 = P_<u64>(ctx->A1);
      fa.A2 = P_<u64>(ctx->A2);
      fa.cross = P_<u64>(ctx->cross);
      fa.err = reinterpret_cast<int32_t*>(P_<u64>(ctx->sizes) + SZ_ERR);
    }
    if (sys_on) {
      fa.Mc = P_<u64>(ctx->Mc);
      fa.clr = P_<int32_t>(ctx->rc.cls);
      fa.sys_row = sys_row;
      fa.sysrow = P_<u64>(ctx->sysrow);
    }
    fa.icnt = P_<i64>(ctx->icnt);
    fa.words = words_dev;
    if (want_shadow && sp.rl > 0 && !side_run) {
      fa.rcls = P_<int32_t>(ctx->rc.cls);
      fa.loff = P_<i64>(ctx->loff);
      fa.tp = P_<i64>(ctx->tp);
      fa.r0 = ctx->r0;
      fa.r1 = ctx->r1;
    }
    hipLaunchKernelGGL(k_verify_cols, dim3((unsigned)nb), dim3(TPB), 0, ctx->stream, fa);
    KLAUNCH();
  } else {
    KCHK(hipMemsetAsync(ctx->icnt.p, 0, sizeof(i64) * 4 * nb, ctx->stream));
  }
  if (side_run) {
    hipStream_t s2 = ctx->stream2;
    {
      ScanBatch sbs(ctx, true);
      KTRY(shadow_stage_a_scans(ctx, sp, sbs));
      KTRY(sbs.add_class_counts(P_<int32_t>(ctx->rc.cls), P_<i64>(ctx->T), ctx->r0, sp.rl,
                                P_<i64>(ctx->poff), SZ_PAIRS));
      KTRY(sbs.run(sp.nt > 0 ? nullptr : ctx->ev_pairs));
    }
    KTRY(dalloc(ctx, ctx->L, sizeof(int2) * std::max<i64>(1, sp.nf)));
    if (sp.nt > 0) {
      launch_marked(k_shadow_compact, dim3((unsigned)sp.nt), dim3(TPB), 0, s2, ctx->ev_pairs,
                    P_<i64>(ctx->soffc), ctx->rc.U, P_<int32_t>(ctx->slist),
                    P_<i64>(ctx->pfoff), P_<uint8_t>(ctx->flags), sp.nf, P_<i64>(ctx->toff),
                    P_<int2>(ctx->L), sp.nf);
      KLAUNCH();
    }
    ctx->tail_compacted = true;
  }
  ctx->vs_open = true;
  ctx->vs_shadow = want_shadow;
  ctx->vs_cross_want = want_cross;
  ctx->vs_cross_on = cross_on;
  ctx->vs_have_sys = have_sys;
  ctx->vs_sys_on = sys_on;
  ctx->vs_rows = true;
  ctx->vs_nb = nb;
  ctx->vs_rl = sp.rl;
  return 0;
}

int spin_event(kano_ctx* ctx, hipEvent_t e) {
  using clk = std::chrono::steady_clock;
  const auto t0 = clk::now();
  for (uint32_t spin = 1;; ++spin) {
    const hipError_t q = hipEventQuery(e);
    if (q == hipSuccess) return 0;
    if (q != hipErrorNotReady) KCHK(q);
    __builtin_ia32_pause();
    if ((spin & 0xff) == 0 && clk::now() - t0 > std::chrono::seconds(1)) {
      KCHK(hipEventSynchronize(e));
      return 0;
    }
  }
}

int prime_next(kano_ctx* ctx) {
  if (ctx->primed || !ctx->bell || ctx->stage_timing) return 0;
  KTRY(dalloc(ctx, ctx->sizes_alt, sizeof(u64) * SZ_SLOTS));
  ctx->prime_alist_valid = ctx->alist_valid;
  KTRY(swap_rows_inputs(ctx));
  std::swap(ctx->sizes, ctx->sizes_alt);
  ctx->primed = true;
  ctx->priming = true;
  const u64 armed = ctx->sig_armed, waiting = ctx->sig_wait;
  if (!ctx->gate_wait.p) {
    KTRY(dalloc(ctx, ctx->gate_wait, sizeof(u64) * GATE_RING));
    KCHK(hipMemsetAsync(ctx->gate_wait.p, 0, sizeof(u64) * GATE_RING, ctx->stream));
  }
  hipLaunchKernelGGL(k_gate, dim3(1), dim3(64), 0, ctx->stream, (const u64*)ctx->bell_dev,
                     ++ctx->bell_seq, ctx->gate_ticks, P_<u64>(ctx->gate_wait));
  int rc = hipGetLastError() == hipSuccess ? 0 : fail(ctx, -EIO, "k_gate launch failed");
  if (!rc) {
    ctx->sig_armed = 0;
    rc = front_a(ctx);
  }
  ctx->priming = false;
  if (rc) {
    (void)unprime(ctx);
    return rc;
  }
  ctx->prime_sig = ctx->sig_wait;
  ctx->sig_armed = armed;
  ctx->sig_wait = waiting;
  return 0;
}

int verify_back_direct(kano_ctx* ctx, int32_t* idx, void* idx_h, int64_t* counts,
                       int32_t* shadow_pairs, void* pairs_h, int64_t shadow_cap,
                       int64_t* shadow_count, bool async, bool compacted = false) {
  using clk = std::chrono::steady_clock;
  auto tmark = clk::now();
  auto part = [&](int k) {
    const auto t = clk::now();
    ctx->ht[k] = std::max(ctx->ht[k], std::chrono::duration<double, std::micro>(t - tmark).count());
    tmark = t;
  };
  const i64 n = ctx->n, rl = ctx->vs_rl;
  const bool want_shadow = ctx->vs_shadow;
  const bool pairs_mode = want_shadow && shadow_cap >= 0;
  hipStream_t st = ctx->stream;
  const i64 nf = ctx->nflags, nt = (nf + SH_TILE - 1) / SH_TILE;
  i64 out_cap = 0;
  const bool pairs_job = pairs_mode && pairs_h && rl > 0;
  const u64* tots = P_<u64>(ctx->sizes) + SZ_IDX0;
  if (pairs_mode) {
    KTRY(dalloc(ctx, ctx->L, sizeof(int2) * std::max<i64>(1, nf)));
    KTRY(dalloc(ctx, ctx->out, sizeof(int2) * 1024));
    out_cap = (i64)(ctx->out.bytes / sizeof(int2));
    if (compacted) KCHK(hipStreamWaitEvent(st, ctx->ev_pairs, 0));
    if (nt > 0 && !compacted) {
      hipLaunchKernelGGL(k_shadow_compact, dim3((unsigned)nt), dim3(TPB), 0, st,
                         P_<i64>(ctx->soffc), ctx->rc.U, P_<int32_t>(ctx->slist),
                         P_<i64>(ctx->pfoff), P_<uint8_t>(ctx->flags), nf, P_<i64>(ctx->toff),
                         P_<int2>(ctx->L), nf);
      KLAUNCH();
    }
    if (rl > 0) {
      hipLaunchKernelGGL(k_shadow_emit, dim3(nblk(rl)), dim3(TPB), 0, st,
                         P_<int32_t>(ctx->rc.cls), ctx->r0, ctx->r1, P_<i64>(ctx->loff),
                         P_<int2>(ctx->L), P_<i64>(ctx->poff), P_<int2>(ctx->out), out_cap,
                         nt > 0 ? P_<i64>(ctx->toff) + nt : (const i64*)nullptr, nf);
      KLAUNCH();
    }
  }
  CopySegs cj{};
  int njobs = 0;
  cj.j[njobs++] = CopySeg{static_cast<const char*>(ctx->idxd.p), static_cast<char*>(idx_h),
                          tots, 4, nullptr, 0, 4, 4 * n};
  if (pairs_job) {
    cj.j[njobs++] = CopySeg{static_cast<const char*>(ctx->out.p), static_cast<char*>(pairs_h),
                            reinterpret_cast<const u64*>(P_<i64>(ctx->poff) + rl), 1, nullptr, 0,
                            8, std::min<i64>(shadow_cap, out_cap)};
  }
  if (njobs > 0) {
    hipExtLaunchKernelGGL(k_copy_segs, dim3(256, njobs), dim3(TPB), 0, st, nullptr, ctx->ev_tail,
                          0, cj);
    KLAUNCH();
  }
  if (ctx->vs_rows) {
    ctx->rows_overlap = async;
    ctx->rows_in = ctx->rin_marked ? ctx->ev_rin_e : ctx->ev_tail;
    ctx->rin_marked = false;
    const int rc = launch_rows(ctx);
    ctx->rows_overlap = false;
    ctx->rows_in = nullptr;
    KTRY(rc);
  }
  if (async && ctx->pipeline) KTRY(prime_next(ctx));
  part(12);
  const auto tw0 = clk::now();
  KTRY(spin_event(ctx, ctx->ev_tail));
  ctx->ht[18] += std::chrono::duration<double, std::micro>(clk::now() - tw0).count();
  part(14);
  ctx->sig_wait = 0;
  constexpr int NS = SZ_ERR - SZ_NL + 1;
  i64 v[NS];
  for (int q = 0; q < NS; ++q) v[q] = (i64)((volatile u64*)ctx->gmirror)[SZ_NL + q];
  if (ctx->vs_cross_on && (v[SZ_ERR - SZ_NL] & 0xffffffff)) {
    (void)settle(ctx);
    (void)sync(ctx);
    return fail(ctx, -EINVAL, "kano_verify: a group id lies outside [0, ngroups)");
  }
  for (int r = 0; r < 4; ++r) counts[r] = v[SZ_IDX0 - SZ_NL + r];
  if (!ctx->vs_have_sys) counts[3] = -1;
  if (want_shadow) {
    const i64 total = v[SZ_PAIRS - SZ_NL];
    *shadow_count = total;
    ctx->shadow_total = pairs_mode ? total : -1;
    if (pairs_mode && total > out_cap) {
      KTRY(unprime(ctx));
      KTRY(dalloc(ctx, ctx->out, sizeof(int2) * (total + total / 4)));
      if (rl > 0) {
        hipLaunchKernelGGL(k_shadow_emit, dim3(nblk(rl)), dim3(TPB), 0, st,
                           P_<int32_t>(ctx->rc.cls), ctx->r0, ctx->r1, P_<i64>(ctx->loff),
                           P_<int2>(ctx->L), P_<i64>(ctx->poff), P_<int2>(ctx->out), total,
                           (const i64*)nullptr, nf);
        KLAUNCH();
      }
      if (shadow_pairs && total <= shadow_cap)
        KTRY(copy_out(ctx, shadow_pairs, ctx->out.p, sizeof(int2) * total, st));
      KCHK(hipEventRecord(ctx->ev_tail, st));
      KCHK(hipEventSynchronize(ctx->ev_tail));
    }
  }
  part(15);
  if (async) {
    ctx->async_pending = true;
    return 0;
  }
  KTRY(sync(ctx));
  return 0;
}

int verify_back(kano_ctx* ctx, const u64* gathered, int32_t nranks, int32_t* idx, int64_t* counts,
                int32_t* shadow_pairs, int64_t shadow_cap, int64_t* shadow_count,
                bool may_async = false) {
  if (!ctx->vs_open) return fail(ctx, -EINVAL, "kano_verify_combine without kano_verify_shard");
  ctx->vs_open = false;
  const i64 n = ctx->n, W = ctx->W, nb = ctx->vs_nb;
  const bool want_shadow = ctx->vs_shadow;
  const bool cross_row = gathered ? ctx->vs_cross_want : ctx->vs_cross_on;
  const bool pairs_mode = want_shadow && shadow_cap >= 0;
  if (want_shadow && ctx->vs_count_only && shadow_cap >= 0) {
    (void)sync(ctx);
    return fail(ctx, -EINVAL, "kano_verify_combine: the shard ran policy_shadow count-only "
                              "(with_shadow = 2); pass shadow_cap < 0");
  }
  void* idx_h = n > 0 ? pinned_dev(idx) : nullptr;
  void* pairs_h = pairs_mode && shadow_pairs ? pinned_dev(shadow_pairs) : nullptr;
  const bool direct = n > 0 && W > 0 && idx_h && (!pairs_mode || !shadow_pairs || pairs_h);
  const bool side_sh = want_shadow && ctx->tail_compacted;
  const bool compacted = side_sh && direct && pairs_mode;
  if (side_sh && !compacted) KCHK(hipStreamWaitEvent(ctx->stream, ctx->ev_pairs, 0));
  ctx->tail_compacted = false;
  ScanBatch sb(ctx);
  if (want_shadow && !side_sh)
    KTRY(sb.add(P_<i64>(ctx->tp), ctx->vs_rl, P_<i64>(ctx->poff), SZ_PAIRS));
  if (gathered && n > 0 && W > 0) {
    if (cross_row) KTRY(dalloc(ctx, ctx->cross, sizeof(u64) * ctx->ldM));
    hipLaunchKernelGGL(k_combine_cols, dim3((unsigned)nb), dim3(TPB), 0, ctx->stream, gathered,
                       nranks, n, W, nb, P_<u64>(ctx->color), P_<u64>(ctx->colnand),
                       P_<u64>(ctx->col_and), cross_row ? P_<u64>(ctx->cross) : nullptr,
                       P_<i64>(ctx->icnt));
    KLAUNCH();
  }
  for (int r = 0; r < 4; ++r)
    KTRY(sb.add(P_<i64>(ctx->icnt) + r * nb, nb, P_<i64>(ctx->ioff) + r * (nb + 1),
                SZ_IDX0 + r));
  sb.publish(SZ_ERR);
  if (want_shadow && !compacted) sb.publish(SZ_NL);
  if (sb.jobs.count == 0) ctx->sig_armed = 0;
  KTRY(sb.run());
  IdxRows ir{};
  ir.W = W;
  ir.n = n;
  ir.nb = nb;
  ir.row[0] = P_<u64>(ctx->col_and);
  ir.row[1] = P_<u64>(ctx->color);
  ir.inv[1] = 1;
  ir.row[2] = cross_row ? P_<u64>(ctx->cross) : nullptr;
  ir.row[3] = ctx->vs_sys_on ? P_<u64>(ctx->sysrow) : nullptr;
  ir.inv[3] = 1;
  int32_t* idx_dev = P_<int32_t>(ctx->idxd);
  if (n > 0 && W > 0) {
    hipLaunchKernelGGL(k_idx_write, dim3((unsigned)nb, 4), dim3(TPB), 0, ctx->stream, ir,
                       P_<i64>(ctx->ioff), nb + 1, P_<u64>(ctx->sizes) + SZ_IDX0, idx_dev);
    KLAUNCH();
  }
  if (direct)
    return verify_back_direct(ctx, idx, idx_h, counts, shadow_pairs, pairs_h, shadow_cap,
                              shadow_count, may_async && ctx->async_rows, compacted);
  constexpr int NS = SZ_ERR - SZ_NL + 1;
  using clk = std::chrono::steady_clock;
  auto tmark = clk::now();
  auto part = [&](int k) {
    const auto t = clk::now();
    ctx->ht[k] = std::max(ctx->ht[k], std::chrono::duration<double, std::micro>(t - tmark).count());
    tmark = t;
  };
  const bool signalled = ctx->sig_armed != 0;
  KTRY(mirror_begin(ctx));
  hipEvent_t tail_ev = signalled ? nullptr : ctx->ev_sizes;
  const bool async = may_async && ctx->async_rows;
  if (!tail_ev) {
    KCHK(hipEventRecord(ctx->ev_sizes, ctx->stream));
    tail_ev = ctx->ev_sizes;
  }
  part(12);
  i64 v[NS];
  KTRY(mirror_wait(ctx, SZ_NL, NS, v));
  tmark = clk::now();
  if (ctx->vs_cross_on && (v[SZ_ERR - SZ_NL] & 0xffffffff)) {
    (void)sync(ctx);
    return fail(ctx, -EINVAL, "kano_verify: a group id lies outside [0, ngroups)");
  }
  i64 nidx = 0;
  for (int r = 0; r < 4; ++r) {
    counts[r] = v[SZ_IDX0 - SZ_NL + r];
    nidx += counts[r];
  }
  if (!ctx->vs_have_sys) counts[3] = -1;
  hipStream_t cs = ctx->stream2;
  KCHK(hipStreamWaitEvent(cs, tail_ev, 0));
  i64 total = 0;
  if (want_shadow) {
    total = v[SZ_PAIRS - SZ_NL];
    if (shadow_cap >= 0) {
      KTRY(shadow_back(ctx, v[0], total, cs));
      part(13);
      ctx->shadow_total = total;
    } else {
      ctx->shadow_total = -1;
    }
    *shadow_count = total;
  }
  tmark = clk::now();
  if (nidx > 0) {
    KTRY(copy_out(ctx, idx, idx_dev, sizeof(int32_t) * nidx, cs));
  }
  part(15);
  if (want_shadow && shadow_pairs && total > 0 && total <= shadow_cap)
    KTRY(copy_out(ctx, shadow_pairs, ctx->out.p, sizeof(int2) * total, cs));
  part(16);
  KCHK(hipEventRecord(ctx->ev_tail, cs));
  if (ctx->vs_rows) {
    ctx->rows_overlap = async;
    ctx->rows_after = ctx->ev_tail;
    const int rc = launch_rows(ctx);
    ctx->rows_overlap = false;
    ctx->rows_after = nullptr;
    KTRY(rc);
  }
  KCHK(hipEventRecord(ctx->ev_fork, cs));
  KCHK(hipStreamWaitEvent(ctx->stream, ctx->ev_fork, 0));
  part(17);
  if (async) {
    KCHK(hipEventSynchronize(ctx->ev_tail));
    part(14);
    ctx->async_pending = true;
    return 0;
  }
  KTRY(sync(ctx));
  part(14);
  return 0;
}
void host_time_record(kano_ctx* ctx, std::chrono::steady_clock::time_point t0,
                      std::chrono::steady_clock::time_point t1,
                      std::chrono::steady_clock::time_point t2) {
  auto us = [](std::chrono::steady_clock::duration d) {
    return std::chrono::duration<double, std::micro>(d).count();
  };
  double* h = ctx->ht;
  if (h[0] > 0) h[4] += us(t0 - ctx->ht_last);
  h[0] += 1;
  h[1] += us(t1 - t0);
  h[2] += us(t2 - t1);
  h[3] += ctx->ht_wait_cur;
  h[5] = std::max(h[5], us(t1 - t0));
  h[6] = std::max(h[6], us(t2 - t1));
  h[7] = std::max(h[7], ctx->ht_wait_cur);
  h[8] = std::max(h[8], us(t2 - t0));
  ctx->ht_last = t2;
}
}

extern "C" {

int kano_verify(kano_ctx* ctx, int path, const int32_t* gid, int32_t ngroups, int64_t sys_row,
                int32_t* idx, int64_t* counts, int32_t* shadow_pairs, int64_t shadow_cap,
                int64_t* shadow_count) {
  if (!ctx) return -EINVAL;
  if (!counts || (!idx && ctx->n > 0))
    return fail(ctx, -EINVAL, "kano_verify: idx / counts must not be NULL");
  ring_bell(ctx);
  using clk = std::chrono::steady_clock;
  const auto t0 = clk::now();
  ctx->ht_wait = 0;
  ctx->ht_wait_cur = 0.0;
  KTRY(verify_front(ctx, path, gid, ngroups, sys_row, shadow_count != nullptr, nullptr,
                    shadow_cap < 0));
  const auto t1 = clk::now();
  const int rc =
      verify_back(ctx, nullptr, 0, idx, counts, shadow_pairs, shadow_cap, shadow_count, true);
  host_time_record(ctx, t0, t1, clk::now());
  return rc;
}

int kano_set_pipeline(kano_ctx* ctx, int on) {
  if (!ctx) return -EINVAL;
  if (!on) KTRY(unprime(ctx));
  ctx->pipeline = on ? 1 : 0;
  return 0;
}

int kano_settle(kano_ctx* ctx) {
  if (!ctx) return -EINVAL;
  KCHK(hipSetDevice(ctx->device));
  return settle(ctx);
}

int kano_gate_timing(kano_ctx* ctx, int reset, int64_t* gates, double* mean_us,
                     double* max_us) {
  if (!ctx) return -EINVAL;
  KCHK(hipSetDevice(ctx->device));
  KTRY(settle(ctx));
  const u64 last = ctx->bell_seq - (ctx->gate_forced == ctx->bell_seq ? 1 : 0);
  const u64 n = last > ctx->gate_seq0 ? std::min<u64>(last - ctx->gate_seq0, GATE_RING) : 0;
  double sum = 0.0, mx = 0.0;
  if (n > 0 && ctx->gate_wait.p) {
    u64 ring[GATE_RING];
    KCHK(hipMemcpy(ring, ctx->gate_wait.p, sizeof(ring), hipMemcpyDeviceToHost));
    for (u64 q = 0; q < n; ++q) {
      const double us = (double)ring[(last - q) % GATE_RING] * 1e3 / (double)ctx->wall_khz;
      sum += us;
      mx = std::max(mx, us);
    }
  }
  if (gates) *gates = (int64_t)n;
  if (mean_us) *mean_us = n ? sum / (double)n : 0.0;
  if (max_us) *max_us = mx;
  if (reset) ctx->gate_seq0 = ctx->bell_seq;
  return 0;
}

int kano_host_times(kano_ctx* ctx, double* out, int reset) {
  if (!ctx || !out) return -EINVAL;
  for (int k = 0; k < 20; ++k) out[k] = ctx->ht[k];
  if (reset)
    for (double& v : ctx->ht) v = 0.0;
  return 0;
}

int kano_verify_shard(kano_ctx* ctx, int path, const int32_t* gid, int32_t ngroups,
                      int64_t sys_row, int with_shadow, uint64_t* words_dev) {
  if (!ctx) return -EINVAL;
  if (!words_dev) return fail(ctx, -EINVAL, "kano_verify_shard: words_dev is NULL");
  return verify_front(ctx, path, gid, ngroups, sys_row, with_shadow != 0,
                      reinterpret_cast<u64*>(words_dev), with_shadow == 2);
}

int kano_verify_combine(kano_ctx* ctx, const uint64_t* gathered_dev, int32_t nranks,
                        int32_t* idx, int64_t* counts, int32_t* shadow_pairs, int64_t shadow_cap,
                        int64_t* shadow_count) {
  if (!ctx) return -EINVAL;
  if (!counts || (!idx && ctx->n > 0) || !gathered_dev || nranks < 1)
    return fail(ctx, -EINVAL, "kano_verify_combine: bad arguments");
  if (ctx->vs_open && ctx->vs_shadow && !shadow_count)
    return fail(ctx, -EINVAL, "kano_verify_combine: shadow_count is NULL but the shard ran policy_shadow");
  return verify_back(ctx, reinterpret_cast<const u64*>(gathered_dev), nranks, idx, counts,
                     shadow_pairs, shadow_cap, shadow_count, true);
}

int kano_verify_gather(kano_ctx* ctx, int path, const int32_t* gid, int32_t ngroups,
                       int64_t sys_row, int with_shadow, void* comm, int32_t nranks,
                       int32_t* idx, int64_t* counts, int32_t* shadow_pairs, int64_t shadow_cap,
                       int64_t* shadow_count) {
  if (!ctx) return -EINVAL;
  if (nranks < 1) return fail(ctx, -EINVAL, "kano_verify_gather: bad communicator");
  if (!counts || (!idx && ctx->n > 0))
    return fail(ctx, -EINVAL, "kano_verify_gather: idx / counts must not be NULL");
  if (with_shadow && !shadow_count)
    return fail(ctx, -EINVAL, "kano_verify_gather: shadow_count is NULL but with_shadow is set");
  ring_bell(ctx);
  const RcclAllGather ag = comm ? rccl_all_gather() : nullptr;
  if (comm && !ag)
    return fail(ctx, -ENOSYS, "kano_verify_gather: no RCCL in the process (ncclAllGather)");
  const i64 nw = 3 * ctx->W;
  KTRY(dalloc(ctx, ctx->xw, sizeof(u64) * std::max<i64>(1, nw)));
  const void* xg_before = ctx->xg.p;
  KTRY(dalloc(ctx, ctx->xg, sizeof(u64) * std::max<i64>(1, nw * nranks)));
  if (!comm && (ctx->xg.p != xg_before || ctx->xg_emul != nw * nranks)) {
    KCHK(hipMemsetAsync(ctx->xg.p, 0, sizeof(u64) * std::max<i64>(1, nw * nranks), ctx->stream));
    ctx->xg_emul = nw * nranks;
  }
  using clk = std::chrono::steady_clock;
  const auto t0 = clk::now();
  ctx->ht_wait = 0;
  ctx->ht_wait_cur = 0.0;
  KTRY(verify_front(ctx, path, gid, ngroups, sys_row, with_shadow != 0, P_<u64>(ctx->xw),
                    with_shadow == 2));
  if (comm) ctx->xg_emul = -1;
  if (nw > 0 && comm) {
    const int rc = ag(ctx->xw.p, ctx->xg.p, (size_t)nw, RCCL_UINT64, comm, ctx->stream);
    if (rc != 0) {
      (void)sync(ctx);
      return fail(ctx, -EIO, "kano_verify_gather: ncclAllGather returned " + std::to_string(rc));
    }
  } else if (nw > 0) {
    KCHK(hipMemcpyAsync(ctx->xg.p, ctx->xw.p, sizeof(u64) * nw, hipMemcpyDeviceToDevice,
                        ctx->stream));
  }
  const auto t1 = clk::now();
  const int rc = verify_back(ctx, P_<u64>(ctx->xg), nranks, idx, counts, shadow_pairs,
                             shadow_cap, shadow_count, true);
  host_time_record(ctx, t0, t1, clk::now());
  return rc;
}

int kano_checks_shard(kano_ctx* ctx, const int32_t* gid, int32_t ngroups, int64_t sys_row,
                      uint64_t* words_dev) {
  KTRY(ensure_matrix(ctx));
  if (!words_dev) return fail(ctx, -EINVAL, "kano_checks_shard: words_dev is NULL");
  const i64 n = ctx->n, W = ctx->W;
  const bool stored = !gid && ngroups == KANO_STORED_GROUPS;
  const bool want_cross = gid || stored;
  if (!ctx->cols_valid) KTRY(recompute_cols(ctx));
  bool cross_on = false;
  if (want_cross) {
    KTRY(crosscheck_impl(ctx, stored ? nullptr : gid, stored ? 0 : ngroups));
    cross_on = n > 0 && rows_local(ctx) > 0 && W > 0;
  }
  const i64 nb = std::max<i64>(1, nblk(W * 64));
  KTRY(dalloc(ctx, ctx->col_and, sizeof(u64) * std::max<i64>(1, W)));
  KTRY(dalloc(ctx, ctx->sysrow, sizeof(u64) * std::max<i64>(1, W)));
  KTRY(dalloc(ctx, ctx->icnt, sizeof(i64) * 4 * nb));
  KTRY(dalloc(ctx, ctx->ioff, sizeof(i64) * 4 * (nb + 1)));
  KTRY(dalloc(ctx, ctx->idxd, sizeof(int32_t) * std::max<i64>(1, 4 * n) + 16));
  KTRY(dalloc(ctx, ctx->sizes, sizeof(u64) * SZ_SLOTS));
  if (W > 0) {
    KCHK(hipMemcpyAsync(words_dev, ctx->color.p, sizeof(u64) * W, hipMemcpyDeviceToDevice,
                        ctx->stream));
    if (cross_on)
      KCHK(hipMemcpyAsync(words_dev + W, ctx->cross.p, sizeof(u64) * W, hipMemcpyDeviceToDevice,
                          ctx->stream));
    else
      KCHK(hipMemsetAsync(words_dev + W, 0, sizeof(u64) * W, ctx->stream));
    KCHK(hipMemcpyAsync(words_dev + 2 * W, ctx->colnand.p, sizeof(u64) * W,
                        hipMemcpyDeviceToDevice, ctx->stream));
  }
  const bool have_sys = sys_row >= ctx->r0 && sys_row < ctx->r1;
  const bool sys_on = have_sys && W > 0;
  if (sys_on)
    KCHK(hipMemcpyAsync(ctx->sysrow.p, P_<u64>(ctx->M) + (sys_row - ctx->r0) * ctx->ldM,
                        sizeof(u64) * W, hipMemcpyDeviceToDevice, ctx->stream));
  hipLaunchKernelGGL(k_row_zero_counts, dim3((unsigned)nb), dim3(TPB), 0, ctx->stream,
                     sys_on ? P_<u64>(ctx->sysrow) : (const u64*)nullptr, n, W,
// ... 140 lines not shown
```

kubernetes-verification_amd/csrc/kano_kernels.hpp:

```cpp
#pragma once
#include "kano_prims.hpp"

namespace kano {

struct ClsSide {
  const int32_t* keys;
  int KS;
  int packed;
  int pbits;
  uint32_t tmask;
  int32_t* table;
  int32_t* slot_of;
  int32_t* smin;
  int32_t* flag;
  const int32_t* cid;
  int32_t* cls;
  int32_t* rep;
  int32_t* mcnt;
  int32_t* mcur;
  const int32_t* moff;
  int32_t* mem;
  int32_t* cval;
  i64 m0, m1, U;
};
struct ClsPair {
  ClsSide s[2];
};

constexpr int KEY_LDS_MAX = 8192;
constexpr int KEY_ITEMS = 8;
struct KeySort {
  i64 U;
  i64 nb;
  const int32_t* mcnt;
  const int32_t* gmin;
  const int32_t* gmax;
  int32_t G;
  int32_t* ckey;
  int32_t* hist;
  const int32_t* hoff;
  int32_t* order;
};

__device__ __forceinline__ void key_hist_block(const KeySort& k, i64 b) {
  extern __shared__ int32_t h[];
  const int nk = k.G + 1;
  for (int q = threadIdx.x; q < nk; q += TPB) h[q] = 0;
  __syncthreads();
  const i64 c0 = b * TPB * KEY_ITEMS;
  for (int q = 0; q < KEY_ITEMS; ++q) {
    const i64 c = c0 + (i64)q * TPB + threadIdx.x;
    if (c >= k.U) break;
    int32_t key = -1;
    if (k.mcnt[c] > 0 && k.gmin[c] <= k.gmax[c]) key = k.gmin[c] == k.gmax[c] ? k.gmin[c] : k.G;
    k.ckey[c] = key;
    if (key >= 0) atomicAdd(&h[key], 1);
  }
  __syncthreads();
  for (int q = threadIdx.x; q < nk; q += TPB) k.hist[(i64)q * k.nb + b] = h[q];
}

__device__ __forceinline__ void key_place_block(const KeySort& k, i64 b) {
  extern __shared__ int32_t h[];
  const int nk = k.G + 1;
  for (int q = threadIdx.x; q < nk; q += TPB) h[q] = k.hoff[(i64)q * k.nb + b];
  __syncthreads();
  const i64 c0 = b * TPB * KEY_ITEMS;
  for (int q = 0; q < KEY_ITEMS; ++q) {
    const i64 c = c0 + (i64)q * TPB + threadIdx.x;
    if (c >= k.U) break;
    const int32_t key = k.ckey[c];
    if (key >= 0) k.order[atomicAdd(&h[key], 1)] = (int32_t)c;
  }
}

constexpr int CLS_LDS = 512;

__device__ __forceinline__ int lds_class_slot(int32_t* lkey, int32_t c, bool insert) {
  uint32_t h = hfin(hmix(0x2545f491u, (uint32_t)c)) & (CLS_LDS - 1);
  for (int probe = 0; probe < CLS_LDS; ++probe) {
    int32_t cur = lkey[h];
    if (cur == -1 && insert) {
      cur = atomicCAS(&lkey[h], -1, c);
      if (cur == -1) return (int)h;
    }
    if (cur == c) return (int)h;
    if (cur == -1) return -1;
    h = (h + 1) & (CLS_LDS - 1);
  }
  return -1;
}


__device__ __forceinline__ uint32_t cls_packed_slot(const u64* tab, uint32_t tmask, u64 key) {
  uint32_t s = hfin(hmix(hmix(0x9747b28cu, (uint32_t)key), (uint32_t)(key >> 32))) & tmask;
  u64* t = const_cast<u64*>(tab);
  for (;;) {
    u64 cur = t[s];
    if (cur == ~0ull) {
      const u64 prev = atomicCAS(reinterpret_cast<unsigned long long*>(&t[s]), ~0ull,
                                 (unsigned long long)key);
      if (prev == ~0ull) break;
      cur = prev;
    }
    if (cur == key) break;
    s = (s + 1) & tmask;
  }
  return s;
}

__global__ __launch_bounds__(TPB) void k_cls_insert(const int32_t* __restrict__ pv, i64 n,
                                                    ClsPair pr) {
  const ClsSide a = blockIdx.y ? pr.s[1] : pr.s[0];
  const i64 i = a.m0 + (i64)blockIdx.x * TPB + threadIdx.x;
  const bool act = i < a.m1;
  if (act) a.mcnt[i - a.m0] = 0;
  if (a.packed) {
    __shared__ u64 lkey[CLS_LDS];
    __shared__ int32_t lmin[CLS_LDS], lslot[CLS_LDS];
    for (int t = threadIdx.x; t < CLS_LDS; t += TPB) {
      lkey[t] = ~0ull;
      lmin[t] = INT32_MAX;
    }
    __syncthreads();
    u64 key = 0;
    int t = -1;
    bool lead = false;
    if (act) {
      for (int k = 0; k < a.KS; ++k)
        key = (key << a.keys[a.KS + k]) | (u64)(uint32_t)(pv[(i64)a.keys[k] * n + i] + 3);
      uint32_t h = hfin(hmix(hmix(0x2545f491u, (uint32_t)key), (uint32_t)(key >> 32))) &
                   (CLS_LDS - 1);
      for (;;) {
        const u64 prev = atomicCAS(reinterpret_cast<unsigned long long*>(&lkey[h]), ~0ull,
                                   (unsigned long long)key);
        if (prev == ~0ull) { lead = true; break; }
        if (prev == key) break;
        h = (h + 1) & (CLS_LDS - 1);
      }
      t = (int)h;
      atomicMin(&lmin[t], (int32_t)i);
    }
    __syncthreads();
    if (lead && a.pbits) {
      unsigned long long* tb = reinterpret_cast<unsigned long long*>(a.table);
      const u64 mine = (key << a.pbits) | (u64)(uint32_t)lmin[t];
      uint32_t s = hfin(hmix(hmix(0x9747b28cu, (uint32_t)key), (uint32_t)(key >> 32))) & a.tmask;
      for (;;) {
        const u64 prev = atomicCAS(&tb[s], ~0ull, (unsigned long long)mine);
        if (prev == ~0ull) break;
        if ((prev >> a.pbits) == key) {
          if (prev > mine) atomicMin(&tb[s], (unsigned long long)mine);
          break;
        }
        s = (s + 1) & a.tmask;
      }
      lslot[t] = (int32_t)s;
    } else if (lead) {
      const uint32_t s = cls_packed_slot(reinterpret_cast<const u64*>(a.table), a.tmask, key);
      lslot[t] = (int32_t)s;
      if (lmin[t] < a.smin[s]) atomicMin(&a.smin[s], lmin[t]);
    }
    __syncthreads();
    if (act) a.slot_of[i] = lslot[t];
    return;
  }
  if (!act) return;
  uint32_t s;
  uint32_t h = 0x9747b28cu;
  for (int k = 0; k < a.KS; ++k) h = hmix(h, (uint32_t)pv[(i64)a.keys[k] * n + i]);
  s = hfin(h) & a.tmask;
  for (;;) {
    int32_t cur = a.table[s];
    if (cur < 0) {
      const int32_t prev = atomicCAS(&a.table[s], -1, (int32_t)i);
      if (prev < 0) break;
      cur = prev;
    }
    bool eq = true;
    for (int k = 0; k < a.KS; ++k) {
      const int32_t* col = pv + (i64)a.keys[k] * n;
      if (col[cur] != col[i]) { eq = false; break; }
    }
    if (eq) break;
    s = (s + 1) & a.tmask;
  }
  a.slot_of[i] = (int32_t)s;
  const int lane = threadIdx.x & 63;
  const u64 below = (1ull << lane) - 1ull;
  bool first = true;
  u64 pend = __ballot(true);
  for (int round = 0; round < 4 && pend; ++round) {
    const int leader = __ffsll((long long)pend) - 1;
    const uint32_t sl = __shfl(s, leader, 64);
    const u64 same = __ballot(s == sl);
    if (s == sl && (same & below)) first = false;
    pend &= ~same;
  }
  if (first && (int32_t)i < a.smin[s]) atomicMin(&a.smin[s], (int32_t)i);
}



constexpr int ASSIGN_IPT = 8;
__global__ __launch_bounds__(TPB) void k_cls_assign_count(ClsPair pr, int ipt) {
  const ClsSide a = blockIdx.y ? pr.s[1] : pr.s[0];
  __shared__ int32_t lkey[CLS_LDS], lcnt[CLS_LDS], lbase[CLS_LDS];
  for (int t = threadIdx.x; t < CLS_LDS; t += TPB) {
    lkey[t] = -1;
    lcnt[t] = 0;
  }
  __syncthreads();
  int32_t cs[ASSIGN_IPT], ts[ASSIGN_IPT], rs[ASSIGN_IPT];
  bool lead[ASSIGN_IPT];
  const i64 i0 = a.m0 + (i64)blockIdx.x * TPB * ipt + threadIdx.x;
#pragma unroll
  for (int k = 0; k < ASSIGN_IPT; ++k) {
    ts[k] = -2;
    lead[k] = false;
    const i64 i = i0 + (i64)k * TPB;
    if (k >= ipt || i >= a.m1) continue;
    const int32_t sl = a.slot_of[i];
    const int32_t rp = a.pbits ? (int32_t)(reinterpret_cast<const u64*>(a.table)[sl] &
                                           ((1ull << a.pbits) - 1ull))
                               : a.smin[sl];
    const int32_t c = a.cid[rp - a.m0];
    cs[k] = c;
    a.cls[i] = c;
    if (rp == (int32_t)i) a.rep[c] = (int32_t)i;
    uint32_t h = hfin(hmix(0x2545f491u, (uint32_t)c)) & (CLS_LDS - 1);
    int t = -1;
    for (int probe = 0; probe < CLS_LDS; ++probe) {
      const int32_t prev = atomicCAS(&lkey[h], -1, c);
      if (prev == -1) { lead[k] = true; t = (int)h; break; }
      if (prev == c) { t = (int)h; break; }
      h = (h + 1) & (CLS_LDS - 1);
    }
    ts[k] = t;
    if (t >= 0) rs[k] = atomicAdd(&lcnt[t], 1);
    else a.mcur[i - a.m0] = atomicAdd(&a.mcnt[c], 1);
  }
  __syncthreads();
#pragma unroll
  for (int k = 0; k < ASSIGN_IPT; ++k)
    if (lead[k]) lbase[ts[k]] = atomicAdd(&a.mcnt[cs[k]], lcnt[ts[k]]);
  __syncthreads();
#pragma unroll
  for (int k = 0; k < ASSIGN_IPT; ++k)
    if (ts[k] >= 0) a.mcur[i0 + (i64)k * TPB - a.m0] = lbase[ts[k]] + rs[k];
}


__global__ __launch_bounds__(TPB) void k_cls_mfill(ClsPair pr, const int32_t* __restrict__ gid,
                                                   int32_t G, int32_t* gmin, int32_t* gmax,
                                                   int32_t* err) {
  const ClsSide a = blockIdx.y ? pr.s[1] : pr.s[0];
  const i64 i = a.m0 + (i64)blockIdx.x * TPB + threadIdx.x;
  const bool act = i < a.m1;
  const int32_t c = act ? a.cls[i] : 0;
  if (act) a.mem[a.moff[c] + a.mcur[i - a.m0]] = (int32_t)i;
  if (blockIdx.y == 0 && gid) {
    __shared__ int32_t lk[CLS_LDS], lmn[CLS_LDS], lmx[CLS_LDS];
    for (int t = threadIdx.x; t < CLS_LDS; t += TPB) {
      lk[t] = -1;
      lmn[t] = INT32_MAX;
      lmx[t] = INT32_MIN;
    }
    __syncthreads();
    const int32_t g = act ? gid[i] : 0;
    if (act && (g < 0 || g >= G)) {
      atomicOr(err, 1);
    } else if (act) {
      const int t = lds_class_slot(lk, c, true);
      atomicMin(&lmn[t], g);
      atomicMax(&lmx[t], g);
    }
    __syncthreads();
    for (int t = threadIdx.x; t < CLS_LDS; t += TPB) {
      const int32_t k = lk[t];
      if (k < 0) continue;
      if (lmn[t] < gmin[k]) atomicMin(&gmin[k], lmn[t]);
      if (lmx[t] > gmax[k]) atomicMax(&gmax[k], lmx[t]);
    }
  }
}

__global__ __launch_bounds__(TPB) void k_cls_vals(const int32_t* __restrict__ pv, i64 n,
                                                  ClsPair pr, FillJobs fj, unsigned nbv) {
  if (blockIdx.x >= nbv) {
    if (blockIdx.y == 0) fill_item(fj, blockIdx.x - nbv, gridDim.x - nbv);
    return;
  }
  const ClsSide a = blockIdx.y ? pr.s[1] : pr.s[0];
  const i64 c = (i64)blockIdx.x * TPB + threadIdx.x;
  if (c < a.U) {
    const int32_t r = a.rep[c];
    for (int k = 0; k < a.KS; ++k) a.cval[(i64)k * a.U + c] = pv[(i64)a.keys[k] * n + r];
  }
}

__global__ __launch_bounds__(TPB) void k_expr_cols(const int32_t* __restrict__ pv, i64 n,
                                                   const int32_t* __restrict__ ecol,
                                                   const int32_t* __restrict__ eop,
                                                   const i64* __restrict__ eoff,
                                                   const int32_t* __restrict__ eval,
                                                   int32_t* __restrict__ out) {
  const i64 i = (i64)blockIdx.x * TPB + threadIdx.x;
  const i64 e = blockIdx.y;
  if (i >= n) return;
  const int32_t c = ecol[e];
  const int32_t v = c >= 0 ? pv[(i64)c * n + i] : -1;
  bool listed = false;
  if (v >= 0) {
    i64 lo = eoff[e], hi = eoff[e + 1];
    while (lo < hi) {
      const i64 mid = (lo + hi) >> 1;
      if (eval[mid] < v) lo = mid + 1; else hi = mid;
    }
    listed = lo < eoff[e + 1] && eval[lo] == v;
  }
  const int op = eop[e];
  const bool present = v != -1;
  const bool m = op == 0 ? listed : op == 1 ? !listed : op == 2 ? present : !present;
  out[e * n + i] = m ? 1 : 0;
}

__global__ __launch_bounds__(TPB) void k_class_eval(const int32_t* __restrict__ cval, i64 U, i64 P,
                                                    const i64* __restrict__ off,
                                                    const int32_t* __restrict__ slot,
                                                    const int32_t* __restrict__ val,
                                                    u64* __restrict__ outT,
                                                    u64* __restrict__ outP, i64 ldP) {
  const i64 c = (i64)blockIdx.x * TPB + threadIdx.x;
  const i64 pb = blockIdx.y;
  const i64 p0 = pb * 64;
  const int qn = (int)min((i64)64, P - p0);
  const bool live = c < U;
  const bool lane0 = (threadIdx.x & 63) == 0;
  const i64 cw = c >> 6;
  u64 word = 0;
  for (int q = 0; q < qn; ++q) {
    const i64 p = p0 + q;
    const i64 t0 = off[p], t1 = off[p + 1];
    bool ok = live;
    for (i64 t = t0; t < t1 && ok; ++t) ok = cval[(i64)slot[t] * U + c] == val[t];
    word |= (u64)ok << q;
    if (outP) {
      const u64 b = __ballot(ok);
      if (lane0 && cw * 64 < U) outP[p * ldP + cw] = b;
    }
  }
  if (live && outT) outT[pb * U + c] = word;
}

__global__ __launch_bounds__(TPB) void k_pol_count(const u64* __restrict__ AC, i64 ldC, i64 UW,
                                                   const int32_t* __restrict__ cmoff,
                                                   int32_t* __restrict__ nca,
                                                   int32_t* __restrict__ acnt) {
  __shared__ i64 sm[4];
  const i64 p = blockIdx.x;
  i64 nc = 0, np = 0;
  for (i64 w = threadIdx.x; w < UW; w += TPB) {
    u64 v = AC[p * ldC + w];
    nc += __popcll(v);
    if (cmoff) {
      while (v) {
        const i64 ca = w * 64 + __builtin_ctzll(v);
        np += cmoff[ca + 1] - cmoff[ca];
        v &= v - 1;
      }
    }
  }
  nc = block_sum(nc, sm);
  np = block_sum(np, sm);
  if (threadIdx.x == 0) {
    nca[p] = (int32_t)nc;
    acnt[p] = (int32_t)(cmoff ? np : nc);
  }
}

__global__ __launch_bounds__(TPB) void k_pol_classes(const u64* __restrict__ AC, i64 ldC, i64 UW,
                                                     const i64* __restrict__ alcoff,
                                                     int32_t* __restrict__ alc) {
  __shared__ int sm[4];
  const i64 p = blockIdx.x;
  i64 base = alcoff[p];
  for (i64 w0 = 0; w0 < UW; w0 += TPB) {
    const i64 w = w0 + threadIdx.x;
    u64 v = (w < UW) ? AC[p * ldC + w] : 0ull;
    int tot;
    i64 pos = base + block_excl_scan((int)__popcll(v), sm, tot);
    while (v) {
      alc[pos++] = (int32_t)(w * 64 + __builtin_ctzll(v));
      v &= v - 1;
    }
    base += tot;
  }
}

constexpr int WPB = TPB / 64;
__device__ __forceinline__ i64 wave_policy() {
  return (i64)blockIdx.x * WPB + (threadIdx.x >> 6);
}

struct PolPodsArgs {
  i64 P;
  const i64* alcoff;
  const int32_t* alc;
  const int32_t* cmoff;
  const int32_t* cmem;
  const i64* aloff;
  int32_t* alist;
};
__device__ __forceinline__ void pol_pods_item(const PolPodsArgs& a, i64 vb) {
  const i64 P = a.P;
  const i64* __restrict__ alcoff = a.alcoff;
  const int32_t* __restrict__ alc = a.alc;
  const int32_t* __restrict__ cmoff = a.cmoff;
  const int32_t* __restrict__ cmem = a.cmem;
  const i64* __restrict__ aloff = a.aloff;
  int32_t* __restrict__ alist = a.alist;
  __shared__ int32_t seg_m0[WPB][64];
  __shared__ int32_t seg_pre[WPB][65];
  const int wid = threadIdx.x >> 6, lane = threadIdx.x & 63;
  const i64 p = vb * WPB + wid;
  if (p >= P) return;
  i64 out = aloff[p];
  const i64 e1 = alcoff[p + 1];
  for (i64 e0 = alcoff[p]; e0 < e1; e0 += 64) {
    const int ns = (int)min((i64)64, e1 - e0);
    int32_t m0 = 0, len = 0;
    if (lane < ns) {
      const int32_t ca = alc[e0 + lane];
      m0 = cmoff[ca];
      len = cmoff[ca + 1] - m0;
    }
    int32_t tot;
    const int32_t pre = wave_excl_scan(len, tot);
    seg_m0[wid][lane] = m0;
    seg_pre[wid][lane] = pre;
    if (lane == 0) seg_pre[wid][ns] = tot;
    __builtin_amdgcn_wave_barrier();
    for (int32_t id = lane; id < tot; id += 64) {
      int lo = 0, hi = ns - 1;
      while (lo < hi) {
        const int mid = (lo + hi + 1) >> 1;
        if (seg_pre[wid][mid] <= id) lo = mid; else hi = mid - 1;
      }
      alist[out + id] = cmem[seg_m0[wid][lo] + (id - seg_pre[wid][lo])];
    }
    out += tot;
    __builtin_amdgcn_wave_barrier();
  }
}

__global__ __launch_bounds__(TPB) void k_pol_pods(PolPodsArgs a) { pol_pods_item(a, blockIdx.x); }

__device__ __forceinline__ uint32_t proj_hash(const int32_t* __restrict__ cval, i64 U, i64 c,
                                              const int32_t* __restrict__ slots, int ns) {
  uint32_t h = 0x2545f491u;
  for (int k = 0; k < ns; ++k) h = hmix(h, (uint32_t)cval[(i64)slots[k] * U + c]);
  return hfin(h);
}

struct JoinSide {
  const int32_t* cval;
  i64 U;
  const int32_t* moff;
  const int32_t* mslot;
  int32_t* table;
  i64 T;
  int32_t* pslot;
  int32_t* gcnt;
  const int32_t* goff;
  int32_t* gcur;
  int32_t* gmem;
  const i64* toff;
  const int32_t* tval;
  const int32_t* pmask;
  i64* pstart;
  int32_t* plen;
  int NM;
  int live;
  const u64* ctab;
  uint32_t ctmask;
  const int32_t* csmin;
  int cpb;
  const int32_t* ccid;
  i64 cm0;
  const int32_t* kbits;
  int KS;
};
struct JoinPair {
  JoinSide s[2];
};

__device__ __forceinline__ int join_row(const JoinPair& pr, int y, int extra, int* m) {
  const int r0 = pr.s[0].live ? pr.s[0].NM + extra : 0;
  if (y < r0) { *m = y; return 0; }
  *m = y - r0;
  return 1;
}

__global__ __launch_bounds__(TPB) void k_join_insert(JoinPair pr) {
  int m;
  const JoinSide a = join_row(pr, blockIdx.y, 0, &m) ? pr.s[1] : pr.s[0];
  const i64 c = (i64)blockIdx.x * TPB + threadIdx.x;
  const bool act = c < a.U;
  uint32_t s = 0;
  if (act) {
    const int32_t* sl = a.mslot + a.moff[m];
    const int ns = a.moff[m + 1] - a.moff[m];
    int32_t* tab = a.table + (i64)m * a.T;
    const uint32_t tm = (uint32_t)(a.T - 1);
    s = proj_hash(a.cval, a.U, c, sl, ns) & tm;
    for (;;) {
      int32_t cur = tab[s];
      if (cur < 0) {
        const int32_t prev = atomicCAS(&tab[s], -1, (int32_t)c);
        if (prev < 0) break;
        cur = prev;
      }
      bool eq = true;
      for (int k = 0; k < ns; ++k) {
        const int32_t* col = a.cval + (i64)sl[k] * a.U;
        if (col[cur] != col[c]) { eq = false; break; }
      }
      if (eq) break;
      s = (s + 1) & tm;
    }
    a.pslot[(i64)m * a.U + c] = (int32_t)s;
  }
  const int32_t r = wave_agg_inc(a.gcnt, act ? (i64)m * a.T + s : 0, act);
  if (act) a.gcur[(i64)m * a.U + c] = r;
}


__device__ __forceinline__ void join_fill_item(const JoinPair& pr, int y, i64 bx) {
  int m;
  const JoinSide a = join_row(pr, y, 1, &m) ? pr.s[1] : pr.s[0];
  const i64 c = bx * TPB + threadIdx.x;
  if (m == a.NM) {
    if (c < a.U) a.gmem[(i64)a.NM * a.U + c] = (int32_t)c;
    return;
  }
  if (c >= a.U) return;
  const i64 g = (i64)m * a.T + a.pslot[(i64)m * a.U + c];
  a.gmem[a.goff[g] + a.gcur[(i64)m * a.U + c]] = (int32_t)c;
}

__device__ __forceinline__ void join_match_item(i64 P, const JoinPair& pr, int side, i64 bx) {
  const JoinSide a = side ? pr.s[1] : pr.s[0];
  const i64 p = bx * TPB + threadIdx.x;
  if (!a.live || p >= P) return;
  const int m = a.pmask[p];
  i64 st = 0;
  int32_t len = 0;
  if (m == -3) {
    const i64 t0 = a.toff[p];
    bool possible = true;
    u64 key = 0;
    for (int k = 0; k < a.KS; ++k) {
      const int32_t v = a.tval[t0 + k];
      possible = possible && v >= 0;
      key = (key << a.kbits[k]) | (u64)(uint32_t)(v + 3);
    }
    if (possible && a.U > 0) {
      uint32_t s = hfin(hmix(hmix(0x9747b28cu, (uint32_t)key), (uint32_t)(key >> 32))) & a.ctmask;
      for (;;) {
        const u64 cur = a.ctab[s];
        if (cur == ~0ull) break;
        if ((a.cpb ? cur >> a.cpb : cur) == key) {
          const int32_t r = a.cpb ? (int32_t)(cur & ((1ull << a.cpb) - 1ull)) : a.csmin[s];
          st = (i64)a.NM * a.U + a.ccid[r - a.cm0];
          len = 1;
          break;
        }
        s = (s + 1) & a.ctmask;
      }
    }
  } else if (m == -2) {
    st = (i64)a.NM * a.U;
    len = (int32_t)a.U;
  } else if (m >= 0) {
    const i64 t0 = a.toff[p];
    const int32_t* sl = a.mslot + a.moff[m];
    const int ns = a.moff[m + 1] - a.moff[m];
    bool possible = true;
    uint32_t h = 0x2545f491u;
    for (int k = 0; k < ns; ++k) {
      const int32_t v = a.tval[t0 + k];
      possible = possible && v >= 0;
      h = hmix(h, (uint32_t)v);
    }
    if (possible && a.U > 0) {
      const int32_t* tab = a.table + (i64)m * a.T;
      const uint32_t tm = (uint32_t)(a.T - 1);
      uint32_t s = hfin(h) & tm;
      for (;;) {
        const int32_t cur = tab[s];
        if (cur < 0) break;
        bool eq = true;
        for (int k = 0; k < ns; ++k)
          if (a.cval[(i64)sl[k] * a.U + cur] != a.tval[t0 + k]) { eq = false; break; }
        if (eq) {
          const i64 g = (i64)m * a.T + s;
          st = a.goff[g];
          len = a.goff[g + 1] - a.goff[g];
          break;
        }
        s = (s + 1) & tm;
      }
    }
  }
  a.pstart[p] = st;
  a.plen[p] = len;
}

__global__ __launch_bounds__(TPB) void k_join_fill_match(i64 P, JoinPair pr, int rows_f,
                                                         unsigned nbf, unsigned nbm) {
  const int y = blockIdx.y;
  if (y < rows_f) {
    if (blockIdx.x < nbf) join_fill_item(pr, y, blockIdx.x);
  } else if (blockIdx.x < nbm) {
    join_match_item(P, pr, y - rows_f, blockIdx.x);
  }
}

__global__ __launch_bounds__(TPB) void k_bits_to_lists(const u64* __restrict__ bits, i64 ld,
                                                       i64 UW, const i64* __restrict__ off,
                                                       int32_t* __restrict__ lst) {
  __shared__ int sm[4];
  const i64 p = blockIdx.x;
  i64 base = off[p];
  for (i64 w0 = 0; w0 < UW; w0 += TPB) {
    const i64 w = w0 + threadIdx.x;
    u64 v = (w < UW) ? bits[p * ld + w] : 0ull;
    int tot;
    i64 pos = base + block_excl_scan((int)__popcll(v), sm, tot);
    while (v) {
      lst[pos++] = (int32_t)(w * 64 + __builtin_ctzll(v));
      v &= v - 1;
    }
    base += tot;
  }
}

__global__ __launch_bounds__(TPB) void k_popc_rows(const u64* __restrict__ bits, i64 ld, i64 UW,
                                                   int32_t* __restrict__ cnt) {
  __shared__ int sm[4];
  const i64 p = blockIdx.x;
  int s = 0;
  for (i64 w = threadIdx.x; w < UW; w += TPB) s += __popcll(bits[p * ld + w]);
  s = block_sum(s, sm);
  if (threadIdx.x == 0) cnt[p] = s;
}

__global__ __launch_bounds__(TPB) void k_offsets_to_start(const i64* __restrict__ off, i64 P,
                                                          i64* __restrict__ pstart) {
  const i64 p = (i64)blockIdx.x * TPB + threadIdx.x;
  if (p < P) pstart[p] = off[p];
}


__global__ __launch_bounds__(TPB) void k_sel_place(i64 P, const i64* __restrict__ pstart,
                                                   const int32_t* __restrict__ plen,
                                                   const int32_t* __restrict__ pcls,
                                                   const i64* __restrict__ soffc, int32_t* scur,
                                                   int32_t* __restrict__ slist,
                                                   int32_t* __restrict__ ecls, int spb,
                                                   FillJobs fj, unsigned nbs, i64 cap) {
  if (blockIdx.x >= nbs) {
    fill_item(fj, blockIdx.x - nbs, gridDim.x - nbs);
    return;
  }
  __shared__ int32_t lkey[CLS_LDS], lcnt[CLS_LDS], lbase[CLS_LDS];
  const bool comb = spb > WPB;
  if (comb) {
    for (int t = threadIdx.x; t < CLS_LDS; t += TPB) {
      lkey[t] = -1;
      lcnt[t] = 0;
    }
    __syncthreads();
  }
  const int lane = threadIdx.x & 63, wv = threadIdx.x >> 6;
  const bool lp = spb == TPB;
  const int q0 = lp ? threadIdx.x : wv, qs = lp ? TPB : TPB / 64;
  const int k0 = lp ? 0 : lane, ks = lp ? 1 : 64;
  for (int q = q0; q < spb; q += qs) {
    const i64 p = (i64)blockIdx.x * spb + q;
    if (p >= P) break;
    const int32_t* L = pcls + pstart[p];
    const int32_t len = plen[p];
    for (int32_t k = k0; k < len; k += ks) {
      const int32_t c = L[k];
      const int t = comb ? lds_class_slot(lkey, c, true) : -1;
      if (t >= 0) {
        atomicAdd(&lcnt[t], 1);
      } else {
        const i64 e = soffc[c] + atomicAdd(&scur[c], 1);
        if (e < cap) {
          slist[e] = (int32_t)p;
          ecls[e] = c;
        }
      }
    }
  }
  if (!comb) return;
  __syncthreads();
  for (int t = threadIdx.x; t < CLS_LDS; t += TPB) {
    const int32_t c = lkey[t];
    if (c >= 0) {
      lbase[t] = atomicAdd(&scur[c], lcnt[t]);
      lcnt[t] = 0;
    }
  }
  __syncthreads();
  for (int q = q0; q < spb; q += qs) {
    const i64 p = (i64)blockIdx.x * spb + q;
    if (p >= P) break;
    const int32_t* L = pcls + pstart[p];
    const int32_t len = plen[p];
    for (int32_t k = k0; k < len; k += ks) {
      const int32_t c = L[k];
      const int t = lds_class_slot(lkey, c, false);
      if (t < 0) continue;
      const i64 e = soffc[c] + lbase[t] + atomicAdd(&lcnt[t], 1);
      if (e < cap) {
        slist[e] = (int32_t)p;
        ecls[e] = c;
      }
    }
  }
}

constexpr int SORT_WAVE_MAX = 64;
constexpr int SORT_LDS_WW = 768;

struct ClassListsArgs {
  const i64* soffc;
  i64 U, P;
  int32_t* slist;
  int sort;
  const int32_t* hflag;
  const int32_t* hoff;
  int32_t* hlist;
  const int32_t* wioff;
  int32_t* wicls;
  i64 sort_ww;
  int32_t* stmp;
};
__device__ __forceinline__ void class_lists_item(const ClassListsArgs& a, i64 vb) {
  const i64* __restrict__ soffc = a.soffc;
  const i64 U = a.U, P = a.P;
  int32_t* __restrict__ slist = a.slist;
  const int sort = a.sort;
  const int32_t* __restrict__ hflag = a.hflag;
// ... 2260 lines not shown
```

kubernetes-verification_amd/csrc/kano_prims.hpp:

```cpp
#pragma once
#include <hip/hip_runtime.h>

#include <cstdint>

typedef unsigned long long u64;
typedef long long i64;
typedef unsigned long long u64x2 __attribute__((ext_vector_type(2)));

namespace kano {

constexpr int TPB = 256;
constexpr int SCAN_ITEMS = 8;
constexpr int SCAN_TILE = TPB * SCAN_ITEMS;

template <typename T>
__device__ __forceinline__ T wave_incl_scan(T x) {
  const int lane = threadIdx.x & 63;
#pragma unroll
  for (int d = 1; d < 64; d <<= 1) {
    T y = __shfl_up(x, d, 64);
    if (lane >= d) x += y;
  }
  return x;
}

template <int NW, typename T>
__device__ __forceinline__ T block_excl_scan_nw(T v, T* smem, T& total) {
  const int lane = threadIdx.x & 63, wid = threadIdx.x >> 6;
  T inc = wave_incl_scan(v);
  if (lane == 63) smem[wid] = inc;
  __syncthreads();
  T pre = 0;
  total = 0;
#pragma unroll
  for (int w = 0; w < NW; ++w) {
    if (w < wid) pre += smem[w];
    total += smem[w];
  }
  __syncthreads();
  return pre + inc - v;
}

template <typename T>
__device__ __forceinline__ T block_excl_scan(T v, T* smem, T& total) {
  const int lane = threadIdx.x & 63, wid = threadIdx.x >> 6;
  T inc = wave_incl_scan(v);
  if (lane == 63) smem[wid] = inc;
  __syncthreads();
  T pre = 0;
  for (int w = 0; w < wid; ++w) pre += smem[w];
  total = smem[0] + smem[1] + smem[2] + smem[3];
  __syncthreads();
  return pre + inc - v;
}

template <typename T>
__device__ __forceinline__ T wave_sum(T x) {
#pragma unroll
  for (int d = 32; d >= 1; d >>= 1) x += __shfl_xor(x, d, 64);
  return x;
}

template <typename T>
__device__ __forceinline__ T wave_excl_scan(T v, T& total) {
  const T inc = wave_incl_scan(v);
  total = __shfl(inc, 63, 64);
  return inc - v;
}

template <typename T>
__device__ __forceinline__ T block_sum(T v, T* smem) {
  T tot;
  (void)block_excl_scan(v, smem, tot);
  return tot;
}

template <typename Tin, typename Tout>
__global__ __launch_bounds__(TPB) void k_scan_sums(const Tin* __restrict__ in, i64 n,
                                                   Tout* __restrict__ sums) {
  __shared__ Tout sm[4];
  const i64 base = (i64)blockIdx.x * SCAN_TILE + (i64)threadIdx.x * SCAN_ITEMS;
  Tout s = 0;
#pragma unroll
  for (int k = 0; k < SCAN_ITEMS; ++k)
    if (base + k < n) s += (Tout)in[base + k];
  Tout tot = block_sum(s, sm);
  if (threadIdx.x == 0) sums[blockIdx.x] = tot;
}

template <typename Tin, typename Tout>
__global__ __launch_bounds__(TPB) void k_scan_tiles(const Tin* __restrict__ in, i64 n,
                                                    const Tout* __restrict__ tile_off,
                                                    Tout* __restrict__ out) {
  __shared__ Tout sm[4];
  const i64 base = (i64)blockIdx.x * SCAN_TILE + (i64)threadIdx.x * SCAN_ITEMS;
  Tout v[SCAN_ITEMS];
  Tout s = 0;
#pragma unroll
  for (int k = 0; k < SCAN_ITEMS; ++k) {
    v[k] = (base + k < n) ? (Tout)in[base + k] : (Tout)0;
    s += v[k];
  }
  Tout tot;
  Tout pre = block_excl_scan(s, sm, tot) + (tile_off ? tile_off[blockIdx.x] : (Tout)0);
#pragma unroll
  for (int k = 0; k < SCAN_ITEMS; ++k) {
    if (base + k < n) out[base + k] = pre;
    pre += v[k];
  }
  if (blockIdx.x == gridDim.x - 1 && threadIdx.x == TPB - 1) out[n] = pre;
}

constexpr u64 LB_AGG = 1ull << 62, LB_INC = 2ull << 62, LB_VAL = (1ull << 62) - 1;

__device__ __forceinline__ u64 lb_load(const u64* p) {
  return __hip_atomic_load(p, __ATOMIC_RELAXED, __HIP_MEMORY_SCOPE_AGENT);
}
__device__ __forceinline__ void lb_store(u64* p, u64 v) {
  __hip_atomic_store(p, v, __ATOMIC_RELAXED, __HIP_MEMORY_SCOPE_AGENT);
}

struct ScanJob {
  const void* in;
  void* out;
  u64* total;
  u64* total_host;
  i64 n;
  i64 st;
  int in64, out64;
  int gen;
  int gpb;
  const int32_t* gsmin;
  const u64* gtab;
  const int32_t* gslot;
  const i64* gloff;
  i64 gm0;
  const i64* gcnt;
};
constexpr int MAX_SCAN_JOBS = 8;
constexpr int MAX_PUBLISH = 4;
template <int NJ>
struct ScanJobsN {
  ScanJob j[NJ];
  int count;
  int npub;
  const u64* pub_src[MAX_PUBLISH];
  u64* pub_dst[MAX_PUBLISH];
  u64* sig_host;
  u64 sig_val;
  uint32_t* sig_ctr;
  int sig_n;
};
using ScanJobs = ScanJobsN<MAX_SCAN_JOBS>;

__device__ __forceinline__ void mirror_store(u64* p, u64 v) {
  __hip_atomic_store(p, v, __ATOMIC_RELAXED, __HIP_MEMORY_SCOPE_SYSTEM);
}

template <class J>
__device__ __forceinline__ void scan_sig_arrive(const J& jobs) {
  if (!jobs.sig_host) return;
  __builtin_amdgcn_s_waitcnt(0);
  const uint32_t old =
      __hip_atomic_fetch_add(jobs.sig_ctr, 1u, __ATOMIC_RELAXED, __HIP_MEMORY_SCOPE_AGENT);
  if (old + 1 == (uint32_t)jobs.sig_n) {
    __hip_atomic_store(jobs.sig_ctr, 0u, __ATOMIC_RELAXED, __HIP_MEMORY_SCOPE_AGENT);
    mirror_store(jobs.sig_host, jobs.sig_val);
  }
}

template <int NJ, int IT = SCAN_ITEMS>
__global__ __launch_bounds__(TPB) void k_scan_lb(ScanJobsN<NJ> jobs, u64* status,
                                                 u64* __restrict__ clear, i64 nclear) {
  constexpr i64 TILE = (i64)TPB * IT;
  __shared__ i64 sm[4];
  __shared__ i64 s_tile;
  __shared__ i64 s_prefix;
  const i64 lin = (i64)blockIdx.y * gridDim.x + blockIdx.x;
  const i64 nthr = (i64)gridDim.x * gridDim.y * TPB;
  for (i64 i = lin * TPB + threadIdx.x; i < nclear; i += nthr) clear[i] = 0;
  if (lin == 0 && threadIdx.x == 0 && jobs.npub > 0) {
    for (int q = 0; q < jobs.npub; ++q) mirror_store(jobs.pub_dst[q], *jobs.pub_src[q]);
    scan_sig_arrive(jobs);
  }
  ScanJob jb = jobs.j[0];
#pragma unroll
  for (int q = 1; q < NJ; ++q)
    if ((int)blockIdx.y == q) jb = jobs.j[q];
  const i64 tiles = (jb.n + TILE - 1) / TILE;
  if (jb.n == 0) {
    if (blockIdx.x == 0 && threadIdx.x == 0) {
      if (jb.out64) static_cast<i64*>(jb.out)[0] = 0;
      else static_cast<int32_t*>(jb.out)[0] = 0;
      if (jb.total) *jb.total = 0;
      if (jb.total_host) {
        mirror_store(jb.total_host, 0);
        scan_sig_arrive(jobs);
      }
    }
    return;
  }
  u64* st = status + jb.st;
  if (threadIdx.x == 0)
    s_tile = (i64)__hip_atomic_fetch_add(st, 1ull, __ATOMIC_RELAXED, __HIP_MEMORY_SCOPE_AGENT);
  __syncthreads();
  const i64 tile = s_tile;
  if (tile >= tiles) return;
  const i64 base = tile * TILE + (i64)threadIdx.x * IT;
  i64 v[IT];
  i64 s = 0;
#pragma unroll
  for (int k = 0; k < IT; ++k) {
    const i64 x = base + k;
    if (x >= jb.n) v[k] = 0;
    else if (jb.gen == 1) {
      const int32_t sl = jb.gslot[jb.gm0 + x];
      const int32_t r = jb.gpb ? (int32_t)(jb.gtab[sl] & ((1ull << jb.gpb) - 1ull)) : jb.gsmin[sl];
      v[k] = r == (int32_t)(jb.gm0 + x) ? 1 : 0;
    }
    else if (jb.gen == 2) {
      const int32_t c = jb.gslot[jb.gm0 + x];
      v[k] = jb.gloff[c + 1] - jb.gloff[c];
    }
    else if (jb.gen == 3) v[k] = jb.gcnt[jb.gslot[jb.gm0 + x]];
    else v[k] = jb.in64 ? static_cast<const i64*>(jb.in)[x]
                        : (i64) static_cast<const int32_t*>(jb.in)[x];
    s += v[k];
  }
  i64 tot;
  i64 pre = block_excl_scan(s, sm, tot);
  if (threadIdx.x < 64) {
    const int lane = threadIdx.x;
    u64* ts = st + 1;
    i64 excl = 0;
    if (tile == 0) {
      if (lane == 0) lb_store(&ts[0], LB_INC | ((u64)tot & LB_VAL));
    } else {
      if (lane == 0) lb_store(&ts[tile], LB_AGG | ((u64)tot & LB_VAL));
      for (i64 q0 = tile - 1;; q0 -= 64) {
        const i64 q = q0 - lane;
        u64 w = LB_INC;
        if (q >= 0) {
          do { w = lb_load(&ts[q]); } while (w == 0);
        }
        const u64 inc = __ballot((w & ~LB_VAL) == LB_INC);
        const int f = inc ? __ffsll((long long)inc) - 1 : 63;
        const i64 part = wave_sum(lane <= f ? (i64)(w & LB_VAL) : (i64)0);
        excl += part;
        if (inc) break;
      }
      if (lane == 0) lb_store(&ts[tile], LB_INC | ((u64)(excl + tot) & LB_VAL));
    }
    if (lane == 0) s_prefix = excl;
  }
  __syncthreads();
  pre += s_prefix;
  if (jb.out64) {
    i64* o = static_cast<i64*>(jb.out);
#pragma unroll
    for (int k = 0; k < IT; ++k) {
      if (base + k < jb.n) o[base + k] = pre;
      pre += v[k];
    }
    if (tile == tiles - 1 && threadIdx.x == TPB - 1) {
      o[jb.n] = pre;
      if (jb.total) *jb.total = (u64)pre;
      if (jb.total_host) {
        mirror_store(jb.total_host, (u64)pre);
        scan_sig_arrive(jobs);
      }
    }
  } else {
    int32_t* o = static_cast<int32_t*>(jb.out);
#pragma unroll
    for (int k = 0; k < IT; ++k) {
      if (base + k < jb.n) o[base + k] = (int32_t)pre;
      pre += v[k];
    }
    if (tile == tiles - 1 && threadIdx.x == TPB - 1) {
      o[jb.n] = (int32_t)pre;
      if (jb.total) *jb.total = (u64)pre;
      if (jb.total_host) {
        mirror_store(jb.total_host, (u64)pre);
        scan_sig_arrive(jobs);
      }
    }
  }
}

template <int NJ>
__device__ __forceinline__ void lookback_jobs(u64* st, i64 tiles, i64 tile, const i64* tot,
                                              i64* excl) {
  const int wid = threadIdx.x >> 6, lane = threadIdx.x & 63;
  for (int jq = wid; jq < NJ; jq += TPB / 64) {
    u64* ts = st + (i64)jq * tiles;
    const i64 t = tot[jq];
    i64 ex = 0;
    if (tile == 0) {
      if (lane == 0) lb_store(&ts[0], LB_INC | ((u64)t & LB_VAL));
    } else {
      if (lane == 0) lb_store(&ts[tile], LB_AGG | ((u64)t & LB_VAL));
      for (i64 q0 = tile - 1;; q0 -= 64) {
        const i64 q = q0 - lane;
        u64 w = LB_INC;
        if (q >= 0) {
          do { w = lb_load(&ts[q]); } while (w == 0);
        }
        const u64 inc = __ballot((w & ~LB_VAL) == LB_INC);
        const int f = inc ? __ffsll((long long)inc) - 1 : 63;
        ex += wave_sum(lane <= f ? (i64)(w & LB_VAL) : (i64)0);
        if (inc) break;
      }
      if (lane == 0) lb_store(&ts[tile], LB_INC | ((u64)(ex + t) & LB_VAL));
    }
    if (lane == 0) excl[jq] = ex;
  }
  __syncthreads();
}

__device__ __forceinline__ bool last_block_done(u64* done_ctr, i64 nblocks) {
  __shared__ int s_last;
  __builtin_amdgcn_s_waitcnt(0);
  __syncthreads();
  if (threadIdx.x == 0) {
    const u64 old =
        __hip_atomic_fetch_add(done_ctr, 1ull, __ATOMIC_RELAXED, __HIP_MEMORY_SCOPE_AGENT);
    s_last = old + 1 == (u64)nblocks;
  }
  __syncthreads();
  return s_last != 0;
}

__device__ __forceinline__ i64 lookback_total(u64* st, i64 tiles, int q) {
  u64 w;
  do { w = lb_load(&st[(i64)q * tiles + tiles - 1]); } while ((w & ~LB_VAL) != LB_INC);
  return (i64)(w & LB_VAL);
}

struct FillJob {
  uint32_t* ptr;
  i64 words;
  uint32_t value;
};
constexpr int MAX_FILLS = 24;
struct FillJobs {
  FillJob j[MAX_FILLS];
  int count;
};
__device__ __forceinline__ void fill_item(const FillJobs& jobs, i64 vb, i64 nvb) {
  const i64 stride = nvb * TPB;
  for (int q = 0; q < jobs.count; ++q) {
    uint32_t* p = jobs.j[q].ptr;
    const uint32_t v = jobs.j[q].value;
    const i64 nw = jobs.j[q].words;
    for (i64 i = vb * TPB + threadIdx.x; i < nw; i += stride) p[i] = v;
  }
}
static __global__ __attribute__((unused)) __launch_bounds__(TPB) void k_fill_many(FillJobs jobs) {
  fill_item(jobs, blockIdx.x, gridDim.x);
}
constexpr int FILL_RIDE_BLOCKS = 512;

constexpr int GATE_RING = 64;
static __global__ __attribute__((unused)) __launch_bounds__(64) void k_gate(const u64* bell,
                                                                            u64 want, u64 ticks,
                                                                            u64* waited) {
  if (threadIdx.x != 0) return;
  const u64 t0 = wall_clock64();
  while (__hip_atomic_load(bell, __ATOMIC_RELAXED, __HIP_MEMORY_SCOPE_SYSTEM) < want) {
    if (wall_clock64() - t0 > ticks) break;
    __builtin_amdgcn_s_sleep(1);
  }
  if (waited) waited[want % GATE_RING] = wall_clock64() - t0;
}

constexpr int AGG_ROUNDS = 4;
__device__ __forceinline__ int32_t wave_agg_inc(int32_t* ctr, i64 key, bool active) {
  const int lane = threadIdx.x & 63;
  const u64 below = (1ull << lane) - 1ull;
  u64 rem = __ballot(active);
  bool done = !active;
  int32_t res = 0;
  for (int round = 0; round < AGG_ROUNDS && rem; ++round) {
    const int leader = __ffsll((long long)rem) - 1;
    const i64 k0 = __shfl(key, leader, 64);
    const bool same = !done && key == k0;
    const u64 smask = __ballot(same);
    int32_t base = 0;
    if (lane == leader) base = atomicAdd(&ctr[k0], (int32_t)__popcll(smask));
    base = __shfl(base, leader, 64);
    if (same) {
      res = base + (int32_t)__popcll(smask & below);
      done = true;
    }
    rem &= ~smask;
  }
  if (!done) res = atomicAdd(&ctr[key], 1);
  return res;
}

__device__ __forceinline__ void wave_agg_minmax(int32_t* lo, int32_t* hi, i64 key, int32_t v,
                                                bool active) {
  const int lane = threadIdx.x & 63;
  u64 rem = __ballot(active);
  bool done = !active;
  for (int round = 0; round < AGG_ROUNDS && rem; ++round) {
    const int leader = __ffsll((long long)rem) - 1;
    const i64 k0 = __shfl(key, leader, 64);
    const bool same = !done && key == k0;
    const u64 smask = __ballot(same);
    int32_t mn = same ? v : INT32_MAX, mx = same ? v : INT32_MIN;
#pragma unroll
    for (int d = 32; d >= 1; d >>= 1) {
      mn = min(mn, __shfl_xor(mn, d, 64));
      mx = max(mx, __shfl_xor(mx, d, 64));
    }
    if (lane == leader) {
      atomicMin(&lo[k0], mn);
      atomicMax(&hi[k0], mx);
    }
    if (same) done = true;
    rem &= ~smask;
  }
  if (!done) {
    atomicMin(&lo[key], v);
    atomicMax(&hi[key], v);
  }
}

__device__ __forceinline__ void wave_seg_minmax(int32_t* lo, int32_t* hi, i64 key, int32_t v,
                                                bool active) {
  const int lane = threadIdx.x & 63;
  int32_t mn = active ? v : INT32_MAX, mx = active ? v : INT32_MIN;
#pragma unroll
  for (int d = 1; d < 64; d <<= 1) {
    const i64 ko = __shfl_up(key, d, 64);
    const int32_t a = __shfl_up(mn, d, 64), b = __shfl_up(mx, d, 64);
    if (lane >= d && ko == key) {
      mn = min(mn, a);
      mx = max(mx, b);
    }
  }
  const i64 kn = __shfl_down(key, 1, 64);
  const bool last = lane == 63 || kn != key;
  if (last && mn <= mx) {
    atomicMin(&lo[key], mn);
    atomicMax(&hi[key], mx);
  }
}

__device__ __forceinline__ i64 upper_bound_i32(const int32_t* a, i64 n, i64 key) {
  i64 lo = 0, hi = n;
  while (lo < hi) {
    const i64 mid = (lo + hi) >> 1;
    if ((i64)a[mid] <= key) lo = mid + 1; else hi = mid;
  }
  return lo;
}

__device__ __forceinline__ void or_if_new(u64* p, u64 v) {
  if (v & ~*p) atomicOr(p, v);
}

__device__ __forceinline__ u64 valid_mask(i64 w, i64 n) {
  const i64 lo = w * 64;
  if (lo + 64 <= n) return ~0ull;
  if (lo >= n) return 0ull;
  return (1ull << (n - lo)) - 1ull;
}

__device__ __forceinline__ uint32_t hmix(uint32_t h, uint32_t v) {
  v *= 0xcc9e2d51u;
  v = (v << 15) | (v >> 17);
  v *= 0x1b873593u;
  h ^= v;
  h = (h << 13) | (h >> 19);
  return h * 5u + 0xe6546b64u;
}
__device__ __forceinline__ uint32_t hfin(uint32_t h) {
  h ^= h >> 16; h *= 0x85ebca6bu; h ^= h >> 13; h *= 0xc2b2ae35u; h ^= h >> 16;
  return h;
}

static __global__ __attribute__((unused)) __launch_bounds__(TPB) void k_copy_out(const uint4* __restrict__ src, uint4* dst,
                                                 i64 n16, const uint32_t* __restrict__ src_tail,
                                                 uint32_t* dst_tail, int ntail) {
  const i64 stride = (i64)gridDim.x * TPB;
  for (i64 k = (i64)blockIdx.x * TPB + threadIdx.x; k < n16; k += stride) dst[k] = src[k];
  if (blockIdx.x == 0 && (int)threadIdx.x < ntail) dst_tail[threadIdx.x] = src_tail[threadIdx.x];
}

struct CopyJob {
  const char* src;
  char* dst;
  const u64* cnt;
  int ncnt;
  int esize;
  i64 cap;
};
struct CopyJobs {
  CopyJob j[2];
};
static __global__ __attribute__((unused)) __launch_bounds__(TPB) void k_copy_out_dev(CopyJobs jobs) {
  const CopyJob a = jobs.j[blockIdx.y];
  i64 cnt = 0;
  for (int q = 0; q < a.ncnt; ++q) cnt += (i64)a.cnt[q];
  if (cnt > a.cap) return;
  const i64 bytes = cnt * a.esize, n16 = bytes >> 4;
  const uint4* __restrict__ src = reinterpret_cast<const uint4*>(a.src);
  uint4* dst = reinterpret_cast<uint4*>(a.dst);
  const i64 stride = (i64)gridDim.x * TPB;
  for (i64 k = (i64)blockIdx.x * TPB + threadIdx.x; k < n16; k += stride) dst[k] = src[k];
  const int ntail = (int)((bytes & 15) >> 2);
  if (blockIdx.x == 0 && (int)threadIdx.x < ntail)
    reinterpret_cast<uint32_t*>(a.dst + n16 * 16)[threadIdx.x] =
// ... 5 lines not shown
```

Before: 31050 billion.

## Overlap classify count/vals with host sync and emit shadow pairs on side stream

Moves class value extraction (k_cls_vals) ahead of the host-side mirror sync by sizing cval by member capacity instead of the unknown U, and writes representatives inside the scan instead of in the assign kernel. Adds device-sized fills whose sizes are read on the GPU from class counts, so host fill jobs for those buffers can be skipped. The count kernel now runs on the side stream and is joined later, and the shadow emit kernel moves to the side stream during verify_front. Pinned host pointers are resolved once up front. The cost is larger cval allocations, more cross-stream events, and fills that are silently skipped when they exceed capacity.

Measured after the change: 31390 billion, median of 2. Within noise of the previous version (+1.1%).

```diff
diff --git a/kubernetes-verification_amd/csrc/kano_engine.hpp b/kubernetes-verification_amd/csrc/kano_engine.hpp
--- a/kubernetes-verification_amd/csrc/kano_engine.hpp
+++ b/kubernetes-verification_amd/csrc/kano_engine.hpp
@@ -167,10 +167,21 @@
   DBuf scan_tmp2;
   i64 scan_cap2 = 0;
   int scan_parity2 = 0;
-  hipEvent_t ev_pre = nullptr, ev_pre_done = nullptr, ev_pre_ac = nullptr;
+  hipEvent_t ev_pre = nullptr, ev_pre_done = nullptr, ev_pre_ac = nullptr, ev_cnt = nullptr;
   bool pre_forked = false, pre_side_pending = false, pre_ac_pending = false;
-  bool tail_compacted = false;
+  bool cnt_side_pending = false;
+  struct Prefill {
+    const DBuf* buf;
+    void* ptr;
+    i64 cap;
+    uint32_t value;
+  };
+  Prefill pre[8];
+  int npre = 0;
+  bool tail_compacted = false, tail_emitted = false;
   hipEvent_t ev_pairs = nullptr;
+  bool vs_pins = false;
+  void *vs_idx_h = nullptr, *vs_pairs_h = nullptr;
   DBuf gid, gids, cgroup, R, multi, A1, A2, own, cross, gmin, gmax, ckey, corder, kcnt, koff;
   DBuf flags, T, loff, L, tp, poff, out, tcnt, toff;
   DBuf scratch_words, ident;
diff --git a/kubernetes-verification_amd/csrc/kano_hip.hip b/kubernetes-verification_amd/csrc/kano_hip.hip
--- a/kubernetes-verification_amd/csrc/kano_hip.hip
+++ b/kubernetes-verification_amd/csrc/kano_hip.hip
@@ -89,6 +89,7 @@
     j.out64 = sizeof(Tout) == 8;
     j.gen = 0;
     j.gcnt = nullptr;
+    j.gout = nullptr;
     return 0;
   }
   int add_rep_flags(ClassSet& cs, int pbits, i64 n, int total_slot) {
@@ -100,6 +101,7 @@
     j.gpb = pbits;
     j.gslot = P_<int32_t>(cs.slot_of);
     j.gm0 = cs.m0;
+    j.gout = P_<int32_t>(cs.rep);
     return 0;
   }
   int add_class_lengths(const int32_t* cls, const i64* loff, i64 m0, i64 n, i64* out,
@@ -204,6 +206,7 @@
   FillJobs jobs{};
   kano_ctx* ctx;
   hipStream_t st = nullptr;
+  bool skip_prefilled = false;
   explicit FillBatch(kano_ctx* c, hipStream_t s = nullptr) : ctx(c), st(s) { jobs.count = 0; }
   int add(DBuf& b, size_t bytes, uint32_t value);
   int add_raw(void* p, size_t bytes, uint32_t value) {
@@ -230,6 +233,11 @@
 int FillBatch::add(DBuf& b, size_t bytes, uint32_t value) {
   if (bytes == 0) return 0;
   if (bytes % 4 != 0 || bytes > b.bytes) return fail(ctx, -EINVAL, "internal: bad fill job");
+  if (skip_prefilled)
+    for (int q = 0; q < ctx->npre; ++q)
+      if (ctx->pre[q].buf == &b && ctx->pre[q].ptr == b.p && (i64)(bytes / 4) <= ctx->pre[q].cap &&
+          ctx->pre[q].value == value)
+        return 0;
   if (jobs.count == MAX_FILLS) KTRY(run());
   jobs.j[jobs.count++] = FillJob{reinterpret_cast<uint32_t*>(b.p), (i64)(bytes / 4), value};
   return 0;
@@ -477,6 +485,7 @@
   KTRY(dalloc(ctx, cs.mcur, sizeof(int32_t) * m));
   KTRY(dalloc(ctx, cs.moff, sizeof(int32_t) * (m + 1)));
   KTRY(dalloc(ctx, cs.mem, sizeof(int32_t) * m));
+  KTRY(dalloc(ctx, cs.cval, sizeof(int32_t) * std::max<i64>(1, (i64)cs.KS * m)));
   return 0;
 }
 
@@ -499,13 +508,14 @@
   a.moff = P_<int32_t>(cs.moff);
   a.mem = P_<int32_t>(cs.mem);
   a.cval = P_<int32_t>(cs.cval);
+  a.cvs = std::max<i64>(1, cs.m1 - cs.m0);
   a.m0 = cs.m0;
   a.m1 = cs.m1;
   a.U = cs.U;
   return a;
 }
 
-int classify_phase1(kano_ctx* ctx) {
+int classify_phase1(kano_ctx* ctx, hipEvent_t mark) {
   const i64 n = ctx->n;
   ClsPair pr{{cls_side(ctx, ctx->rc), cls_side(ctx, ctx->cc)}};
   const i64 nr = ctx->rc.m1 - ctx->rc.m0, na = ctx->cc.m1 - ctx->cc.m0;
@@ -518,11 +528,7 @@
   ScanBatch sb(ctx);
   KTRY(sb.add_rep_flags(ctx->rc, cls_pod_bits(ctx, ctx->rc), nr, SZ_UR));
   KTRY(sb.add_rep_flags(ctx->cc, cls_pod_bits(ctx, ctx->cc), na, SZ_UA));
-  return sb.run();
-}
-
-int classify_alloc2(kano_ctx* ctx, ClassSet& cs) {
-  return dalloc(ctx, cs.cval, sizeof(int32_t) * std::max<i64>(1, (i64)cs.KS * cs.U));
+  return sb.run(mark);
 }
 
 int classify_phase2a(kano_ctx* ctx) {
@@ -530,23 +536,25 @@
   const i64 mr = ctx->rc.m1 - ctx->rc.m0, ma = ctx->cc.m1 - ctx->cc.m0;
   const i64 rl = std::max(mr, ma);
   hipStream_t side = ctx->mlists_side ? ctx->stream2 : nullptr;
+  hipStream_t cs = side ? side : ctx->stream;
+  if (side) KCHK(hipStreamWaitEvent(side, ctx->ev_pre, 0));
   if (rl > 0) {
     const i64 prevU = std::max(ctx->rc.U, ctx->cc.U);
     const int ipt = ctx->assign_ipt > 0 ? ctx->assign_ipt
                                         : (prevU > 0 && prevU <= 1024 ? ASSIGN_IPT : 1);
-    launch_marked(k_cls_assign_count, dim3(nblk(rl, (i64)TPB * ipt), 2), dim3(TPB), 0,
-                  ctx->stream, side ? ctx->ev_pre : nullptr, pr, ipt);
+    launch_marked(k_cls_assign_count, dim3(nblk(rl, (i64)TPB * ipt), 2), dim3(TPB), 0, cs,
+                  side ? ctx->ev_cnt : nullptr, pr, ipt);
     KLAUNCH();
   } else if (side) {
-    KCHK(hipEventRecord(ctx->ev_pre, ctx->stream));
-  }
-  if (side) KCHK(hipStreamWaitEvent(side, ctx->ev_pre, 0));
+    KCHK(hipEventRecord(ctx->ev_cnt, side));
+  }
+  ctx->cnt_side_pending = side != nullptr;
   ScanBatch sb(ctx, side != nullptr);
   KTRY(sb.add(P_<int32_t>(ctx->rc.mcnt), mr, P_<int32_t>(ctx->rc.moff)));
   KTRY(sb.add(P_<int32_t>(ctx->cc.mcnt), ma, P_<int32_t>(ctx->cc.moff)));
   KTRY(sb.run());
   if (rl > 0) {
-    hipLaunchKernelGGL(k_cls_mfill, dim3(nblk(rl), 2), dim3(TPB), 0, side ? side : ctx->stream, pr,
+    hipLaunchKernelGGL(k_cls_mfill, dim3(nblk(rl), 2), dim3(TPB), 0, cs, pr,
                        (const int32_t*)nullptr, 0, (int32_t*)nullptr, (int32_t*)nullptr,
                        reinterpret_cast<int32_t*>(P_<u64>(ctx->sizes) + SZ_ERR));
     KLAUNCH();
@@ -554,17 +562,40 @@
   return 0;
 }
 
-int classify_phase2b(kano_ctx* ctx, FillJobs fj) {
+int classify_phase2b(kano_ctx* ctx) {
   ClsPair pr{{cls_side(ctx, ctx->rc), cls_side(ctx, ctx->cc)}};
-  const i64 U = std::max(ctx->rc.U, ctx->cc.U);
-  if (U > 0) {
-    const unsigned nbv = nblk(U), nbf = fill_ride_blocks(fj);
+  const i64 mr = ctx->rc.m1 - ctx->rc.m0, ma = ctx->cc.m1 - ctx->cc.m0;
+  const i64 m = std::max(mr, ma);
+  DevFills df{};
+  ctx->npre = 0;
+  auto pre = [&](DBuf& b, const int32_t* cnt, i64 mul, uint32_t value, int table) {
+    if (!b.p || mul <= 0 || df.count == MAX_DEV_FILLS) return;
+    const i64 cap = (i64)(b.bytes / 4);
+    df.j[df.count++] = DevFill{static_cast<uint32_t*>(b.p), cnt, mul, cap, value, table};
+    ctx->pre[ctx->npre++] = kano_ctx::Prefill{&b, b.p, cap, value};
+  };
+  const int32_t* ur = P_<int32_t>(ctx->rc.cid) + mr;
+  const int32_t* ua = P_<int32_t>(ctx->cc.cid) + ma;
+  if (ctx->P > 0) {
+    if (!ctx->am.dense && ctx->am.NM > 0) {
+      pre(ctx->am.table, ua, ctx->am.NM, 0xffffffffu, 1);
+      pre(ctx->am.gcnt, ua, ctx->am.NM, 0u, 1);
+    }
+    if (!ctx->sm.dense && ctx->sm.NM > 0) {
+      pre(ctx->sm.table, ur, ctx->sm.NM, 0xffffffffu, 1);
+      pre(ctx->sm.gcnt, ur, ctx->sm.NM, 0u, 1);
+    }
+  }
+  pre(ctx->scnt, ur, 1, 0u, 0);
+  pre(ctx->cost, ur, 2, 0u, 0);
+  pre(ctx->scur, ur, 1, 0u, 0);
+  if (m > 0) {
+    const unsigned nbv = nblk(m), nbf = df.count > 0 ? FILL_RIDE_BLOCKS : 0;
     hipLaunchKernelGGL(k_cls_vals, dim3(nbv + nbf, 2), dim3(TPB), 0, ctx->stream,
-                       P_<int32_t>(ctx->pv), ctx->n, pr, fj, nbv);
-    KLAUNCH();
-  } else if (fj.count > 0) {
-    hipLaunchKernelGGL(k_fill_many, dim3(fill_ride_blocks(fj)), dim3(TPB), 0, ctx->stream, fj);
-    KLAUNCH();
+                       P_<int32_t>(ctx->pv), ctx->n, pr, df, nbv);
+    KLAUNCH();
+  } else {
+    ctx->npre = 0;
   }
   return 0;
 }
@@ -599,6 +630,7 @@
 JoinSide join_side(kano_ctx* ctx, SideMatch& sx, ClassSet& cs) {
   JoinSide a{};
   a.cval = P_<int32_t>(cs.cval);
+  a.cvs = std::max<i64>(1, cs.m1 - cs.m0);
   a.U = cs.U;
   a.moff = P_<int32_t>(sx.moff);
   a.mslot = P_<int32_t>(sx.mslot);
@@ -663,7 +695,8 @@
   KTRY(dalloc(ctx, sx.bits, sizeof(u64) * P * ld));
   KTRY(dalloc(ctx, sx.boff, sizeof(i64) * (P + 1)));
   hipLaunchKernelGGL(k_class_eval, dim3(nblk(U), (unsigned)ctx->PB), dim3(TPB), 0, ctx->stream,
-                     P_<int32_t>(cs.cval), U, P, P_<i64>(sx.toff), P_<int32_t>(sx.tslot),
+                     P_<int32_t>(cs.cval), std::max<i64>(1, cs.m1 - cs.m0), U, P,
+                     P_<i64>(sx.toff), P_<int32_t>(sx.tslot),
                      P_<int32_t>(sx.tval), (u64*)nullptr, P_<u64>(sx.bits), ld);
   KLAUNCH();
   hipLaunchKernelGGL(k_popc_rows, dim3((unsigned)P), dim3(TPB), 0, ctx->stream, P_<u64>(sx.bits),
@@ -696,6 +729,7 @@
 }
 
 int select_engine_streams(kano_ctx* ctx);
+int join_event(kano_ctx* ctx, hipEvent_t e);
 
 int front_a(kano_ctx* ctx) {
   KTRY(select_engine_streams(ctx));
@@ -708,9 +742,10 @@
     KTRY(front_fills(ctx, fb));
     KTRY(fb.run());
   }
-  KTRY(classify_phase1(ctx));
+  ctx->mlists_side = ctx->stream2 != nullptr && ctx->mlists_side_ok;
+  KTRY(classify_phase1(ctx, ctx->mlists_side ? ctx->ev_pre : nullptr));
   KTRY(mirror_begin(ctx));
-  ctx->mlists_side = ctx->stream2 != nullptr && ctx->mlists_side_ok;
+  KTRY(classify_phase2b(ctx));
   if (!ctx->mlists_side && ctx->stream2) {
     KTRY(classify_phase2a(ctx));
     KCHK(hipEventRecord(ctx->ev_pre, ctx->stream));
@@ -742,11 +777,9 @@
   const i64 P = ctx->P, Ur = ctx->rc.U, Ua = ctx->cc.U;
   ctx->UAW = (Ua + 63) / 64;
   ctx->ldC = std::max<i64>(2, (ctx->UAW + 1) & ~(i64)1);
-  FillJobs carried{};
   {
     FillBatch fb(ctx);
-    KTRY(classify_alloc2(ctx, ctx->rc));
-    KTRY(classify_alloc2(ctx, ctx->cc));
+    fb.skip_prefilled = true;
     KTRY(match_alloc(ctx, ctx->am, ctx->cc, fb));
     KTRY(match_alloc(ctx, ctx->sm, ctx->rc, fb));
     KTRY(dalloc(ctx, ctx->nca, sizeof(int32_t) * std::max<i64>(1, P)));
@@ -766,13 +799,17 @@
     KTRY(fb.add(ctx->scnt, sizeof(int32_t) * Ur, 0u));
     KTRY(fb.add(ctx->cost, sizeof(u64) * Ur, 0u));
     KTRY(fb.add(ctx->scur, sizeof(int32_t) * Ur, 0u));
-    carried = fb.take();
-  }
-  KTRY(classify_phase2b(ctx, carried));
+    KTRY(fb.run());
+    ctx->npre = 0;
+  }
   KTRY(match_both(ctx));
   KTRY(stage_mark(ctx, 2, ctx->stream));
   ctx->dense_sel = ctx->dx_on && Ur > 0 && Ur <= DX_MAX &&
                    (ctx->dx_on == 2 || ctx->nnz_sel >= 32 * Ur);
+  if (ctx->cnt_side_pending) {
+    ctx->cnt_side_pending = false;
+    KTRY(join_event(ctx, ctx->ev_cnt));
+  }
   if (P > 0 && ctx->dense_sel) {
     const i64 ldU = (Ur + 63) / 64;
     ctx->dx_ldY = (Ur + 255) / 256 * 256;
@@ -1862,6 +1899,7 @@
       hipEventCreateWithFlags(&ctx->ev_fork2, hipEventDisableTiming) != hipSuccess ||
       hipEventCreateWithFlags(&ctx->ev_join2, hipEventDisableTiming) != hipSuccess ||
       hipEventCreateWithFlags(&ctx->ev_pre, hipEventDisableTiming) != hipSuccess ||
+      hipEventCreateWithFlags(&ctx->ev_cnt, hipEventDisableTiming) != hipSuccess ||
       hipEventCreateWithFlags(&ctx->ev_pre_done, hipEventDisableTiming) != hipSuccess ||
       hipEventCreateWithFlags(&ctx->ev_pre_ac, hipEventDisableTiming) != hipSuccess ||
       hipEventCreateWithFlags(&ctx->ev_sw, hipEventDisableTiming) != hipSuccess ||
@@ -1983,7 +2021,7 @@
   for (hipEvent_t e : {ctx->ev_sw, ctx->ev_sw2})
     if (e) (void)hipEventDestroy(e);
   for (hipEvent_t e : {ctx->ev_fork, ctx->ev_tail, ctx->ev_rin, ctx->ev_rin_e, ctx->ev_sizes,
-                       ctx->ev_fork2, ctx->ev_join2, ctx->ev_pre, ctx->ev_pre_done, ctx->ev_pre_ac, ctx->ev_pairs, ctx->ev_m0, ctx->ev_m1, ctx->ev_rows_end[0],
+                       ctx->ev_fork2, ctx->ev_join2, ctx->ev_pre, ctx->ev_cnt, ctx->ev_pre_done, ctx->ev_pre_ac, ctx->ev_pairs, ctx->ev_m0, ctx->ev_m1, ctx->ev_rows_end[0],
                        ctx->ev_rows_end[1], ctx->ev_rt[0][0], ctx->ev_rt[0][1], ctx->ev_rt[1][0],
                        ctx->ev_rt[1][1]})
     if (e) (void)hipEventDestroy(e);
@@ -3122,7 +3160,8 @@
 }
 
 int verify_front(kano_ctx* ctx, int path, const int32_t* gid, int32_t ngroups, int64_t sys_row,
-                 bool want_shadow, u64* words_dev, bool count_only = false) {
+                 bool want_shadow, u64* words_dev, bool count_only = false,
+                 bool emit_side = false) {
   ctx->vs_count_only = want_shadow && count_only;
   ctx->consume_prime = ctx->primed;
   if (ctx->async_pending && !ctx->primed) KTRY(swap_rows_inputs(ctx));
@@ -3146,6 +3185,7 @@
   ctx->vs_open = false;
   ctx->fork_pending = false;
   ctx->tail_compacted = false;
+  ctx->tail_emitted = false;
   bool fork_marked = false;
   const bool side_sh = want_shadow && !count_only;
   if (want_shadow) {
@@ -3235,22 +3275,33 @@
   }
   if (side_run) {
     hipStream_t s2 = ctx->stream2;
+    const bool emit = emit_side && sp.rl > 0;
     {
       ScanBatch sbs(ctx, true);
       KTRY(shadow_stage_a_scans(ctx, sp, sbs));
       KTRY(sbs.add_class_counts(P_<int32_t>(ctx->rc.cls), P_<i64>(ctx->T), ctx->r0, sp.rl,
                                 P_<i64>(ctx->poff), SZ_PAIRS));
-      KTRY(sbs.run(sp.nt > 0 ? nullptr : ctx->ev_pairs));
+      KTRY(sbs.run(sp.nt > 0 || emit ? nullptr : ctx->ev_pairs));
     }
     KTRY(dalloc(ctx, ctx->L, sizeof(int2) * std::max<i64>(1, sp.nf)));
+    if (emit) KTRY(dalloc(ctx, ctx->out, sizeof(int2) * 1024));
     if (sp.nt > 0) {
-      launch_marked(k_shadow_compact, dim3((unsigned)sp.nt), dim3(TPB), 0, s2, ctx->ev_pairs,
-                    P_<i64>(ctx->soffc), ctx->rc.U, P_<int32_t>(ctx->slist),
-                    P_<i64>(ctx->pfoff), P_<uint8_t>(ctx->flags), sp.nf, P_<i64>(ctx->toff),
-                    P_<int2>(ctx->L), sp.nf);
+      launch_marked(k_shadow_compact, dim3((unsigned)sp.nt), dim3(TPB), 0, s2,
+                    emit ? nullptr : ctx->ev_pairs, P_<i64>(ctx->soffc), ctx->rc.U,
+                    P_<int32_t>(ctx->slist), P_<i64>(ctx->pfoff), P_<uint8_t>(ctx->flags), sp.nf,
+                    P_<i64>(ctx->toff), P_<int2>(ctx->L), sp.nf);
       KLAUNCH();
     }
+    if (emit) {
+      launch_marked(k_shadow_emit, dim3(nblk(sp.rl)), dim3(TPB), 0, s2, ctx->ev_pairs,
+                    P_<int32_t>(ctx->rc.cls), ctx->r0, ctx->r1, P_<i64>(ctx->loff),
+                    P_<int2>(ctx->L), P_<i64>(ctx->poff), P_<int2>(ctx->out),
+                    (i64)(ctx->out.bytes / sizeof(int2)),
+                    sp.nt > 0 ? P_<i64>(ctx->toff) + sp.nt : (const i64*)nullptr, sp.nf);
+      KLAUNCH();
+    }
     ctx->tail_compacted = true;
+    ctx->tail_emitted = emit;
   }
   ctx->vs_open = true;
   ctx->vs_shadow = want_shadow;
@@ -3312,7 +3363,8 @@
 
 int verify_back_direct(kano_ctx* ctx, int32_t* idx, void* idx_h, int64_t* counts,
                        int32_t* shadow_pairs, void* pairs_h, int64_t shadow_cap,
-                       int64_t* shadow_count, bool async, bool compacted = false) {
+                       int64_t* shadow_count, bool async, bool compacted = false,
+                       bool emitted = false) {
   using clk = std::chrono::steady_clock;
   auto tmark = clk::now();
   auto part = [&](int k) {
@@ -3340,7 +3392,7 @@
                          P_<int2>(ctx->L), nf);
       KLAUNCH();
     }
-    if (rl > 0) {
+    if (rl > 0 && !emitted) {
       hipLaunchKernelGGL(k_shadow_emit, dim3(nblk(rl)), dim3(TPB), 0, st,
                          P_<int32_t>(ctx->rc.cls), ctx->r0, ctx->r1, P_<i64>(ctx->loff),
                          P_<int2>(ctx->L), P_<i64>(ctx->poff), P_<int2>(ctx->out), out_cap,
@@ -3431,13 +3483,17 @@
     return fail(ctx, -EINVAL, "kano_verify_combine: the shard ran policy_shadow count-only "
                               "(with_shadow = 2); pass shadow_cap < 0");
   }
-  void* idx_h = n > 0 ? pinned_dev(idx) : nullptr;
-  void* pairs_h = pairs_mode && shadow_pairs ? pinned_dev(shadow_pairs) : nullptr;
+  void* idx_h = ctx->vs_pins ? ctx->vs_idx_h : n > 0 ? pinned_dev(idx) : nullptr;
+  void* pairs_h = ctx->vs_pins ? ctx->vs_pairs_h
+                  : pairs_mode && shadow_pairs ? pinned_dev(shadow_pairs) : nullptr;
+  ctx->vs_pins = false;
   const bool direct = n > 0 && W > 0 && idx_h && (!pairs_mode || !shadow_pairs || pairs_h);
   const bool side_sh = want_shadow && ctx->tail_compacted;
   const bool compacted = side_sh && direct && pairs_mode;
+  const bool emitted = compacted && ctx->tail_emitted;
   if (side_sh && !compacted) KCHK(hipStreamWaitEvent(ctx->stream, ctx->ev_pairs, 0));
   ctx->tail_compacted = false;
+  ctx->tail_emitted = false;
   ScanBatch sb(ctx);
   if (want_shadow && !side_sh)
     KTRY(sb.add(P_<i64>(ctx->tp), ctx->vs_rl, P_<i64>(ctx->poff), SZ_PAIRS));
@@ -3474,7 +3530,7 @@
   }
   if (direct)
     return verify_back_direct(ctx, idx, idx_h, counts, shadow_pairs, pairs_h, shadow_cap,
-                              shadow_count, may_async && ctx->async_rows, compacted);
+                              shadow_count, may_async && ctx->async_rows, compacted, emitted);
   constexpr int NS = SZ_ERR - SZ_NL + 1;
   using clk = std::chrono::steady_clock;
   auto tmark = clk::now();
@@ -3582,11 +3638,19 @@
   const auto t0 = clk::now();
   ctx->ht_wait = 0;
   ctx->ht_wait_cur = 0.0;
-  KTRY(verify_front(ctx, path, gid, ngroups, sys_row, shadow_count != nullptr, nullptr,
-                    shadow_cap < 0));
+  const bool pairs_mode = shadow_count != nullptr && shadow_cap >= 0;
+  ctx->vs_idx_h = ctx->n > 0 ? pinned_dev(idx) : nullptr;
+  ctx->vs_pairs_h = pairs_mode && shadow_pairs ? pinned_dev(shadow_pairs) : nullptr;
+  const bool emit_side = pairs_mode && ctx->n > 0 && ctx->W > 0 && ctx->vs_idx_h &&
+                         (!shadow_pairs || ctx->vs_pairs_h);
+  const int frc = verify_front(ctx, path, gid, ngroups, sys_row, shadow_count != nullptr, nullptr,
+                               shadow_cap < 0, emit_side);
+  ctx->vs_pins = frc == 0;
+  KTRY(frc);
   const auto t1 = clk::now();
   const int rc =
       verify_back(ctx, nullptr, 0, idx, counts, shadow_pairs, shadow_cap, shadow_count, true);
+  ctx->vs_pins = false;
   host_time_record(ctx, t0, t1, clk::now());
   return rc;
 }
diff --git a/kubernetes-verification_amd/csrc/kano_kernels.hpp b/kubernetes-verification_amd/csrc/kano_kernels.hpp
--- a/kubernetes-verification_amd/csrc/kano_kernels.hpp
+++ b/kubernetes-verification_amd/csrc/kano_kernels.hpp
@@ -21,6 +21,7 @@
   const int32_t* moff;
   int32_t* mem;
   int32_t* cval;
+  i64 cvs;
   i64 m0, m1, U;
 };
 struct ClsPair {
@@ -227,7 +228,6 @@
     const int32_t c = a.cid[rp - a.m0];
     cs[k] = c;
     a.cls[i] = c;
-    if (rp == (int32_t)i) a.rep[c] = (int32_t)i;
     uint32_t h = hfin(hmix(0x2545f491u, (uint32_t)c)) & (CLS_LDS - 1);
     int t = -1;
     for (int probe = 0; probe < CLS_LDS; ++probe) {
@@ -286,16 +286,16 @@
 }
 
 __global__ __launch_bounds__(TPB) void k_cls_vals(const int32_t* __restrict__ pv, i64 n,
-                                                  ClsPair pr, FillJobs fj, unsigned nbv) {
+                                                  ClsPair pr, DevFills df, unsigned nbv) {
   if (blockIdx.x >= nbv) {
-    if (blockIdx.y == 0) fill_item(fj, blockIdx.x - nbv, gridDim.x - nbv);
+    if (blockIdx.y == 0) dev_fill_item(df, blockIdx.x - nbv, gridDim.x - nbv);
     return;
   }
   const ClsSide a = blockIdx.y ? pr.s[1] : pr.s[0];
   const i64 c = (i64)blockIdx.x * TPB + threadIdx.x;
-  if (c < a.U) {
+  if (c < (i64)a.cid[a.m1 - a.m0]) {
     const int32_t r = a.rep[c];
-    for (int k = 0; k < a.KS; ++k) a.cval[(i64)k * a.U + c] = pv[(i64)a.keys[k] * n + r];
+    for (int k = 0; k < a.KS; ++k) a.cval[(i64)k * a.cvs + c] = pv[(i64)a.keys[k] * n + r];
   }
 }
 
@@ -325,7 +325,8 @@
   out[e * n + i] = m ? 1 : 0;
 }
 
-__global__ __launch_bounds__(TPB) void k_class_eval(const int32_t* __restrict__ cval, i64 U, i64 P,
+__global__ __launch_bounds__(TPB) void k_class_eval(const int32_t* __restrict__ cval, i64 cvs,
+                                                    i64 U, i64 P,
                                                     const i64* __restrict__ off,
                                                     const int32_t* __restrict__ slot,
                                                     const int32_t* __restrict__ val,
@@ -343,7 +344,7 @@
     const i64 p = p0 + q;
     const i64 t0 = off[p], t1 = off[p + 1];
     bool ok = live;
-    for (i64 t = t0; t < t1 && ok; ++t) ok = cval[(i64)slot[t] * U + c] == val[t];
+    for (i64 t = t0; t < t1 && ok; ++t) ok = cval[(i64)slot[t] * cvs + c] == val[t];
     word |= (u64)ok << q;
     if (outP) {
       const u64 b = __ballot(ok);
@@ -456,15 +457,16 @@
 
 __global__ __launch_bounds__(TPB) void k_pol_pods(PolPodsArgs a) { pol_pods_item(a, blockIdx.x); }
 
-__device__ __forceinline__ uint32_t proj_hash(const int32_t* __restrict__ cval, i64 U, i64 c,
+__device__ __forceinline__ uint32_t proj_hash(const int32_t* __restrict__ cval, i64 cvs, i64 c,
                                               const int32_t* __restrict__ slots, int ns) {
   uint32_t h = 0x2545f491u;
-  for (int k = 0; k < ns; ++k) h = hmix(h, (uint32_t)cval[(i64)slots[k] * U + c]);
+  for (int k = 0; k < ns; ++k) h = hmix(h, (uint32_t)cval[(i64)slots[k] * cvs + c]);
   return hfin(h);
 }
 
 struct JoinSide {
   const int32_t* cval;
+  i64 cvs;
   i64 U;
   const int32_t* moff;
   const int32_t* mslot;
@@ -513,7 +515,7 @@
     const int ns = a.moff[m + 1] - a.moff[m];
     int32_t* tab = a.table + (i64)m * a.T;
     const uint32_t tm = (uint32_t)(a.T - 1);
-    s = proj_hash(a.cval, a.U, c, sl, ns) & tm;
+    s = proj_hash(a.cval, a.cvs, c, sl, ns) & tm;
     for (;;) {
       int32_t cur = tab[s];
       if (cur < 0) {
@@ -523,7 +525,7 @@
       }
       bool eq = true;
       for (int k = 0; k < ns; ++k) {
-        const int32_t* col = a.cval + (i64)sl[k] * a.U;
+        const int32_t* col = a.cval + (i64)sl[k] * a.cvs;
         if (col[cur] != col[c]) { eq = false; break; }
       }
       if (eq) break;
@@ -602,7 +604,7 @@
         if (cur < 0) break;
         bool eq = true;
         for (int k = 0; k < ns; ++k)
-          if (a.cval[(i64)sl[k] * a.U + cur] != a.tval[t0 + k]) { eq = false; break; }
+          if (a.cval[(i64)sl[k] * a.cvs + cur] != a.tval[t0 + k]) { eq = false; break; }
         if (eq) {
           const i64 g = (i64)m * a.T + s;
           st = a.goff[g];
diff --git a/kubernetes-verification_amd/csrc/kano_prims.hpp b/kubernetes-verification_amd/csrc/kano_prims.hpp
--- a/kubernetes-verification_amd/csrc/kano_prims.hpp
+++ b/kubernetes-verification_amd/csrc/kano_prims.hpp
@@ -136,6 +136,7 @@
   const i64* gloff;
   i64 gm0;
   const i64* gcnt;
+  int32_t* gout;
 };
 constexpr int MAX_SCAN_JOBS = 8;
 constexpr int MAX_PUBLISH = 4;
@@ -272,9 +273,11 @@
     }
   } else {
     int32_t* o = static_cast<int32_t*>(jb.out);
+    int32_t* reps = jb.gen == 1 ? jb.gout : nullptr;
 #pragma unroll
     for (int k = 0; k < IT; ++k) {
       if (base + k < jb.n) o[base + k] = (int32_t)pre;
+      if (reps && v[k]) reps[pre] = (int32_t)(jb.gm0 + base + k);
       pre += v[k];
     }
     if (tile == tiles - 1 && threadIdx.x == TPB - 1) {
@@ -361,6 +364,35 @@
 }
 constexpr int FILL_RIDE_BLOCKS = 512;
 
+struct DevFill {
+  uint32_t* ptr;
+  const int32_t* cnt;
+  i64 mul, cap;
+  uint32_t value;
+  int table;
+};
+constexpr int MAX_DEV_FILLS = 8;
+struct DevFills {
+  DevFill j[MAX_DEV_FILLS];
+  int count;
+};
+__device__ __forceinline__ void dev_fill_item(const DevFills& jobs, i64 vb, i64 nvb) {
+  const i64 stride = nvb * TPB;
+  for (int q = 0; q < jobs.count; ++q) {
+    const i64 u = *jobs.j[q].cnt;
+    i64 t = u;
+    if (jobs.j[q].table) {
+      t = 64;
+      while (t < 2 * u) t <<= 1;
+    }
+    const i64 nw = jobs.j[q].mul * t;
+    if (nw > jobs.j[q].cap) continue;
+    uint32_t* p = jobs.j[q].ptr;
+    const uint32_t v = jobs.j[q].value;
+    for (i64 i = vb * TPB + threadIdx.x; i < nw; i += stride) p[i] = v;
+  }
+}
+
 constexpr int GATE_RING = 64;
 static __global__ __attribute__((unused)) __launch_bounds__(64) void k_gate(const u64* bell,
                                                                             u64 want, u64 ticks,
```
